# yu45020/Text_Segmentation_Image_Inpainting

Measured on NVIDIA H100. Metric: PartialConv UNet 512x512 images/sec (fwd+bwd), higher is better.
Workload: dtype bf16

## Files before the change

### include/pconv_b200.h

```cpp
#ifndef PCONV_B200_H_
#define PCONV_B200_H_

#include <stddef.h>
#include <stdint.h>

#ifdef __cplusplus
extern "C" {
#endif

typedef void *pcb_stream_t;

enum { PCB_F32 = 0, PCB_BF16 = 1 };
enum { PCB_ACT_NONE = 0, PCB_ACT_RELU = 1, PCB_ACT_LEAKY = 2, PCB_ACT_RELU6 = 3 };
enum { PCB_MAX_PARTS = 8 };

typedef struct {
    const void    *x;
    const uint8_t *mask;
    int32_t c;
    int32_t x_cstride;
    int32_t x_up;
    int32_t mask_up;
} pcb_part;

typedef struct {
    int32_t n, h, w, cin;
    int32_t cout, kh, kw;
    int32_t stride, pad_h, pad_w, dil;
    int32_t groups;
    int32_t ho, wo;
    int32_t dtype;
    int32_t same_holes;
    int32_t no_guard;
    int32_t plain;
    int32_t force_generic;
    int32_t nparts;
    pcb_part parts[PCB_MAX_PARTS];
} pcb_conv;

const char *pcb_last_error(void);
int pcb_version(void);
unsigned long long pcb_launch_count(void);
int pcb_conv_uses_tensor_cores(const pcb_conv *c);


size_t pcb_pconv_workspace(const pcb_conv *c);

void pcb_conv_weight_layout(const pcb_conv *c, size_t *fwd_elems, size_t *dgrad_elems);
int pcb_conv_weight_prepare(const pcb_conv *c, const float *w_master_krsc, void *w_fwd, void *w_dgrad, pcb_stream_t stream);
int pcb_conv_weight_refresh(const pcb_conv *c, const float *w_master_krsc, void *w_fwd, void *w_dgrad, pcb_stream_t stream);

int pcb_pconv_forward(const pcb_conv *c, const void *w_fwd, const float *bias, void *y, int y_cstride, float *msum,
                      uint8_t *newmask, void *workspace, pcb_stream_t stream);
int pcb_pconv_mask_pass(const pcb_conv *c, float *msum, uint8_t *newmask, void *workspace, pcb_stream_t stream);
int pcb_pconv_forward_premasked(const pcb_conv *c, const void *w_fwd, const float *bias, void *y, int y_cstride, float *msum,
                      uint8_t *newmask, void *workspace, pcb_stream_t stream);
int pcb_conv_fuses_bn_stats(const pcb_conv *c);
int pcb_pconv_forward_bn(const pcb_conv *c, const void *w_fwd, const float *bias, void *y, int y_cstride, float *msum,
                         uint8_t *newmask, void *workspace, int mask_pass_done, double *bn_sums, pcb_stream_t stream);
int pcb_conv_fuses_affine_act(const pcb_conv *c);
int pcb_pconv_forward_affine_act(const pcb_conv *c, const void *w_fwd, const float *bias, void *y, int y_cstride, float *msum,
                                 uint8_t *newmask, void *workspace, int mask_pass_done, const float *scale, const float *shift,
                                 int act, float slope, pcb_stream_t stream);

int pcb_pconv_renorm_backward(const pcb_conv *c, const void *dy, int dy_cstride, const float *msum, void *dc, int dc_cstride,
                              float *dbias, pcb_stream_t stream);

int pcb_pconv_backward_data(const pcb_conv *c, const void *dc, int dc_cstride, const void *w_fwd, const void *w_dgrad,
                            void *const *dx, const int32_t *dx_cstride, pcb_stream_t stream);
int pcb_conv_dgrad_at_source_resolution(const pcb_conv *c);

int pcb_conv_dgrad_fuses_relu(const pcb_conv *c);
int pcb_pconv_backward_data_relu(const pcb_conv *c, const void *dc, int dc_cstride, const void *w_dgrad, void *dx, int dx_cstride,
                                 const void *relu_x, int relu_cstride, pcb_stream_t stream);

int pcb_pconv_backward_weight(const pcb_conv *c, const void *dc, int dc_cstride, float *dw, void *workspace, pcb_stream_t stream);
int pcb_pconv_backward_weight_acc(const pcb_conv *c, const void *dc, int dc_cstride, float *dw, void *workspace, pcb_stream_t stream);

int pcb_debug_pipeline_status(int *code);
enum { PCB_ROUTE_NONE = 0, PCB_ROUTE_GENERIC = 1, PCB_ROUTE_DEPTHWISE = 2, PCB_ROUTE_STEM = 3, PCB_ROUTE_K2R = 4,
       PCB_ROUTE_SMALLCO = 5, PCB_ROUTE_TMA = 6, PCB_ROUTE_TMA_S2 = 7, PCB_ROUTE_GATHER = 8 };
int pcb_debug_conv_routes(const pcb_conv *c, int32_t routes[3]);

int pcb_mask_planes_from_dense(const float *mask_nchw, int n, int c, int h, int w, uint8_t *planes, pcb_stream_t stream);
int pcb_mask_plane_to_dense(const uint8_t *plane, int n, int h, int w, int up, float *dst_nchw, int ctot, int c0, int c,
                            pcb_stream_t stream);

int pcb_bn_stats(const void *x, int dtype, long long count, int c, double *sum, double *sqsum, pcb_stream_t stream);
int pcb_bn_stats_acc(const void *x, int dtype, long long count, int c, double *sums, pcb_stream_t stream);
int pcb_bn_forward_fused(const void *x, int dtype, long long count, int c, const double *sums, const float *gamma,
                         const float *beta, float *running_mean, float *running_var, long long *num_batches_tracked,
                         float momentum, float eps, int act, float slope, const void *residual, void *y, float *coef,
                         pcb_stream_t stream);
int pcb_bn_finalize(const double *sum, const double *sqsum, long long count, int c, const float *gamma,
                    const float *beta, float *running_mean, float *running_var, long long *num_batches_tracked,
                    float momentum, float eps, int training, float *scale, float *shift, float *save_mean,
                    float *save_invstd, pcb_stream_t stream);
int pcb_bn_act_forward(const void *x, int dtype, long long count, int c, const float *scale, const float *shift,
                       int act, float slope, const void *residual, void *y, pcb_stream_t stream);
int pcb_bn_act_backward_reduce(const void *gy, const void *x, int dtype, long long count, int c, const float *scale,
                               const float *shift, const float *mean, const float *invstd, int act, float slope,
                               double *sum_g, double *sum_gx, pcb_stream_t stream);
int pcb_bn_act_backward_reduce_acc(const void *gy, const void *x, int dtype, long long count, int c, const float *scale,
                                   const float *shift, const float *mean, const float *invstd, int act, float slope,
                                   double *sums, pcb_stream_t stream);
int pcb_bn_act_backward_small(const void *gy, const void *x, int dtype, long long count, int c, const float *coef, int act,
                              float slope, const float *msum, void *dx, float *dgamma, float *dbeta, pcb_stream_t stream);
int pcb_bn_act_backward_apply(const void *gy, const void *x, int dtype, long long count, int c, const float *scale,
                              const float *shift, const float *mean, const float *invstd, int act, float slope,
                              const double *sum_g, const double *sum_gx, int training, void *dx, float *dgamma,
                              float *dbeta, pcb_stream_t stream);
int pcb_bn_act_backward_apply_renorm(const void *gy, const void *x, int dtype, long long count, int c, const float *scale,
                                     const float *shift, const float *mean, const float *invstd, int act, float slope,
                                     const double *sum_g, const double *sum_gx, int training, const float *msum, void *dc,
                                     float *dgamma, float *dbeta, pcb_stream_t stream);

int pcb_upsample2x_forward(const void *x, int dtype, int n, int h, int w, int c, void *y, pcb_stream_t stream);
int pcb_upsample2x_backward(const void *gy, int dtype, int n, int h, int w, int c, void *gx, pcb_stream_t stream);
int pcb_concat_forward(const pcb_part *parts, int nparts, int dtype, int n, int h, int w, void *y, pcb_stream_t stream);
int pcb_concat_backward(const void *gy, const int32_t *c, const int32_t *up, int nparts, int dtype, int n, int h,
                        int w, void *const *gx, pcb_stream_t stream);

int pcb_avgpool_forward(const void *x, void *y, int dtype, int n, int h, int w, int c, int k, int stride, int pad, pcb_stream_t stream);
int pcb_avgpool_backward(const void *gy, void *gx, int dtype, int n, int h, int w, int c, int k, int stride, int pad, pcb_stream_t stream);
int pcb_bilinear_forward(const void *x, void *y, int dtype, int n, int h, int w, int c, int scale, pcb_stream_t stream);
int pcb_bilinear_backward(const void *gy, void *gx, int dtype, int n, int h, int w, int c, int scale, pcb_stream_t stream);
int pcb_gap_forward(const void *x, int dtype, int n, long long hw, int c, float *out, pcb_stream_t stream);
int pcb_gap_backward(const float *g, void *dx, int dtype, int n, long long hw, int c, int accumulate, pcb_stream_t stream);
int pcb_scse_forward(const void *x, const float *cse, const float *ws, void *y, float *sse_out, int dtype, int n, long long hw, int c,
                     pcb_stream_t stream);
int pcb_scse_backward(const void *gy, const void *x, const float *cse, const float *ws, const float *sse, void *dx, float *dcse,
                      float *dws, int dtype, int n, long long hw, int c, pcb_stream_t stream);
int pcb_seg_mask_postprocess(const void *logits, int dtype, int n, int h, int w, int cstride, int h_valid, int w_valid, int oh,
                             int ow, uint8_t *out, pcb_stream_t stream);

typedef struct {
    const uint8_t *rgb;
    const uint8_t *mask;
    int32_t h, w, rgb_stride, mask_stride;
} pcb_inpaint_src;
typedef struct {
    int32_t top, left, height, width;
    int32_t gray;
    int32_t nlines, nellipses;
    int32_t lines[5][5];
    int32_t ellipses[5][4];
} pcb_inpaint_params;
int pcb_inpaint_validate(const pcb_inpaint_src *h_srcs, const pcb_inpaint_params *h_params, int n, int cap_n, int cap_h, int cap_w,
                         int out);
int pcb_inpaint_sample(const pcb_inpaint_src *srcs, int n, int out, int strokes, uint64_t *rng, pcb_inpaint_params *params,
                       pcb_stream_t stream);
int pcb_inpaint_prepare(const pcb_inpaint_src *srcs, const pcb_inpaint_params *params, int n, int cap_h, int cap_w, int out,
                        int strokes, uint8_t *tmp, void *corrupted, int dtype, uint8_t *mask_plane, float *clean, pcb_stream_t stream);

typedef struct {
    const uint8_t *page;
    const uint8_t *mask;
    int32_t h, w, page_stride, mask_stride;
} pcb_seg_src;
typedef struct {
    int32_t top, left, height, width;
    int32_t brightness_first;
    float brightness, contrast;
    int32_t reserved;
} pcb_seg_params;
int pcb_seg_validate(const pcb_seg_src *h_srcs, const pcb_seg_params *h_params, int n, int cap_n, int cap_h, int cap_w, int out);
int pcb_seg_sample(const pcb_seg_src *srcs, int n, uint64_t *rng, pcb_seg_params *params, pcb_stream_t stream);
int pcb_seg_prepare(const pcb_seg_src *srcs, const pcb_seg_params *params, int n, int cap_h, int cap_w, int out, uint8_t *tmp,
                    uint8_t *planes, int *hist, const float *h_norm, void *x, int dtype, float *target, pcb_stream_t stream);

int pcb_inpaint_loss_pixel_forward(const float *raw, const float *origin, const void *output, int out_dtype, const long long *out_strides,
                                   const uint8_t *plane, int n, int h, int w, void *vgg_in, int dtype, double *sums, pcb_stream_t stream);
int pcb_inpaint_loss_pixel_backward(const float *raw, const float *origin, const void *output, int out_dtype, const long long *out_strides,
                                    const uint8_t *plane, int n, int h, int w, const void *dvgg_in, int dtype, const float *coef,
                                    const float *gscale, void *grad, const long long *grad_strides, pcb_stream_t stream);
int pcb_maxpool2x2_forward(const void *x, void *y, int dtype, int n, int h, int w, int c, pcb_stream_t stream);
int pcb_maxpool2x2_backward(const void *gy, const void *x, void *gx, int dtype, int n, int h, int w, int c, int relu_mask, pcb_stream_t stream);
int pcb_feature_l1_forward(const void *f, int dtype, int n, long long hw, int c, double *sums, pcb_stream_t stream);
int pcb_feature_loss_backward(const void *f, int dtype, int n, long long hw, int c, const void *g_next, const void *g_gram, float l1_coef,
                              float gram_coef, const float *gscale, void *df, pcb_stream_t stream);
int pcb_gram_l1_forward(const float *gram, int n, int c, float norm, double *sums, pcb_stream_t stream);
int pcb_gram_sign_sym(const float *gram, int n, int c, float norm, float *t, pcb_stream_t stream);
int pcb_k2r_image_weight(const float *w_oihw, int cout, float *wz, pcb_stream_t stream);
int pcb_k2r_image_dgrad(const void *z, int dtype, int n, int h, int w, void *dx, pcb_stream_t stream);
int pcb_inpaint_loss_finalize(const double *sums, const double *h_inv, float *loss, float *terms, pcb_stream_t stream);

enum { PCB_SEG_FOCAL = 0, PCB_SEG_BOOTSTRAP = 1 };
enum { PCB_SEG_NONE = 0, PCB_SEG_MEAN = 1, PCB_SEG_SUM = 2 };
int pcb_seg_loss_partials(long long count);
int pcb_seg_loss_forward(const void *x, int dtype, const long long *x_strides, const float *target, int n, int h, int w, int loss,
                         int reduction, float p0, float one_minus_beta, float background_weight, float words_weight, double *partials,
                         unsigned int *counter, float *out, pcb_stream_t stream);
int pcb_seg_loss_backward(const void *x, int dtype, const long long *x_strides, const float *target, int n, int h, int w, int loss,
                          int reduction, float p0, float one_minus_beta, float background_weight, float words_weight, const float *gout,
                          void *dx, const long long *dx_strides, pcb_stream_t stream);

int pcb_l1_mean_forward(const void *x, int dtype, long long numel, float *loss ,
                        double *scratch , pcb_stream_t stream);
int pcb_l1_mean_backward(const void *x, int dtype, long long numel, float gscale, void *gx, pcb_stream_t stream);
int pcb_sgd_step(float *param, const float *grad, float *momentum_buf, long long numel, float lr, float momentum,
                 float weight_decay, int nesterov, int first_step, pcb_stream_t stream);
int pcb_sgd_step_scaled(float *param, const float *grad, float *momentum_buf, long long numel, float lr, float momentum,
                        float weight_decay, int nesterov, int first_step, float grad_scale, pcb_stream_t stream);
int pcb_sgd_step_dev(float *param, const float *grad, float *momentum_buf, long long numel, const float *lr, float momentum,
                     float weight_decay, int nesterov, float grad_scale, pcb_stream_t stream);
enum { PCB_CLR_TRIANGULAR = 0, PCB_CLR_TRIANGULAR2 = 1, PCB_CLR_EXP_RANGE = 2 };
int pcb_lr_cyclic(long long *iteration, double base_lr, double max_lr, double step_size, int mode, double gamma, float *lr,
                  double *lr64, pcb_stream_t stream);

#ifdef __cplusplus
}
#endif
#endif
```

### text_segmentation_image_inpainting_b200/_lib.py

```python
import ctypes
import os
import threading

from . import build as _build

PCB_F32, PCB_BF16 = 0, 1
ACT_NONE, ACT_RELU, ACT_LEAKY, ACT_RELU6 = 0, 1, 2, 3
MAX_PARTS = 8
SEG_FOCAL, SEG_BOOTSTRAP = 0, 1
SEG_NONE, SEG_MEAN, SEG_SUM = 0, 1, 2
CLR_TRIANGULAR, CLR_TRIANGULAR2, CLR_EXP_RANGE = 0, 1, 2
ROUTES = ("none", "generic", "depthwise", "stem", "k2r", "smallco", "tma", "tma_s2", "gather")

c_int, c_ll, c_float, c_void_p, c_size_t = ctypes.c_int, ctypes.c_longlong, ctypes.c_float, ctypes.c_void_p, ctypes.c_size_t


class Part(ctypes.Structure):
    _fields_ = [("x", c_void_p), ("mask", c_void_p), ("c", ctypes.c_int32), ("x_cstride", ctypes.c_int32),
                ("x_up", ctypes.c_int32), ("mask_up", ctypes.c_int32)]


class Conv(ctypes.Structure):
    _fields_ = [(k, ctypes.c_int32) for k in
                ("n", "h", "w", "cin", "cout", "kh", "kw", "stride", "pad_h", "pad_w", "dil", "groups", "ho", "wo",
                 "dtype", "same_holes", "no_guard", "plain", "force_generic", "nparts")] + [("parts", Part * MAX_PARTS)]


_SIGS = {
    "pcb_last_error": (ctypes.c_char_p, []),
    "pcb_version": (c_int, []),
    "pcb_launch_count": (ctypes.c_ulonglong, []),
    "pcb_conv_uses_tensor_cores": (c_int, [ctypes.POINTER(Conv)]),
    "pcb_conv_dgrad_at_source_resolution": (c_int, [ctypes.POINTER(Conv)]),
    "pcb_pconv_workspace": (c_size_t, [ctypes.POINTER(Conv)]),
    "pcb_conv_weight_layout": (None, [ctypes.POINTER(Conv), ctypes.POINTER(c_size_t), ctypes.POINTER(c_size_t)]),
    "pcb_conv_weight_prepare": (c_int, [ctypes.POINTER(Conv), c_void_p, c_void_p, c_void_p, c_void_p]),
    "pcb_conv_weight_refresh": (c_int, [ctypes.POINTER(Conv), c_void_p, c_void_p, c_void_p, c_void_p]),
    "pcb_pconv_forward": (c_int, [ctypes.POINTER(Conv), c_void_p, c_void_p, c_void_p, c_int, c_void_p, c_void_p, c_void_p, c_void_p]),
    "pcb_pconv_forward_premasked": (c_int, [ctypes.POINTER(Conv), c_void_p, c_void_p, c_void_p, c_int, c_void_p, c_void_p, c_void_p, c_void_p]),
    "pcb_conv_fuses_bn_stats": (c_int, [ctypes.POINTER(Conv)]),
    "pcb_pconv_forward_bn": (c_int, [ctypes.POINTER(Conv), c_void_p, c_void_p, c_void_p, c_int, c_void_p, c_void_p, c_void_p, c_int, c_void_p, c_void_p]),
    "pcb_conv_fuses_affine_act": (c_int, [ctypes.POINTER(Conv)]),
    "pcb_pconv_forward_affine_act": (c_int, [ctypes.POINTER(Conv), c_void_p, c_void_p, c_void_p, c_int, c_void_p, c_void_p, c_void_p, c_int,
                                             c_void_p, c_void_p, c_int, c_float, c_void_p]),
    "pcb_seg_mask_postprocess": (c_int, [c_void_p, c_int, c_int, c_int, c_int, c_int, c_int, c_int, c_int, c_int, c_void_p, c_void_p]),
    "pcb_pconv_mask_pass":(c_int, [ctypes.POINTER(Conv), c_void_p, c_void_p, c_void_p, c_void_p]),
    "pcb_pconv_renorm_backward": (c_int, [ctypes.POINTER(Conv), c_void_p, c_int, c_void_p, c_void_p, c_int, c_void_p, c_void_p]),
    "pcb_pconv_backward_data": (c_int, [ctypes.POINTER(Conv), c_void_p, c_int, c_void_p, c_void_p, ctypes.POINTER(c_void_p),
                                        ctypes.POINTER(ctypes.c_int32), c_void_p]),
    "pcb_pconv_backward_weight": (c_int, [ctypes.POINTER(Conv), c_void_p, c_int, c_void_p, c_void_p, c_void_p]),
    "pcb_pconv_backward_weight_acc": (c_int, [ctypes.POINTER(Conv), c_void_p, c_int, c_void_p, c_void_p, c_void_p]),
    "pcb_debug_pipeline_status": (c_int, [ctypes.POINTER(c_int)]),
    "pcb_debug_conv_routes": (c_int, [ctypes.POINTER(Conv), ctypes.POINTER(ctypes.c_int32)]),
    "pcb_mask_planes_from_dense": (c_int, [c_void_p, c_int, c_int, c_int, c_int, c_void_p, c_void_p]),
    "pcb_mask_plane_to_dense": (c_int, [c_void_p, c_int, c_int, c_int, c_int, c_void_p, c_int, c_int, c_int, c_void_p]),
    "pcb_bn_stats": (c_int, [c_void_p, c_int, c_ll, c_int, c_void_p, c_void_p, c_void_p]),
    "pcb_bn_stats_acc": (c_int, [c_void_p, c_int, c_ll, c_int, c_void_p, c_void_p]),
    "pcb_bn_forward_fused": (c_int, [c_void_p, c_int, c_ll, c_int, c_void_p, c_void_p, c_void_p, c_void_p, c_void_p, c_void_p,
                                     c_float, c_float, c_int, c_float, c_void_p, c_void_p, c_void_p, c_void_p]),
    "pcb_bn_act_backward_reduce_acc": (c_int, [c_void_p, c_void_p, c_int, c_ll, c_int, c_void_p, c_void_p, c_void_p, c_void_p,
                                               c_int, c_float, c_void_p, c_void_p]),
    "pcb_bn_act_backward_small": (c_int, [c_void_p, c_void_p, c_int, c_ll, c_int, c_void_p, c_int, c_float, c_void_p, c_void_p, c_void_p, c_void_p, c_void_p]),
    "pcb_bn_finalize": (c_int, [c_void_p, c_void_p, c_ll, c_int, c_void_p, c_void_p, c_void_p, c_void_p, c_void_p,
                                c_float, c_float, c_int, c_void_p, c_void_p, c_void_p, c_void_p, c_void_p]),
    "pcb_bn_act_forward": (c_int, [c_void_p, c_int, c_ll, c_int, c_void_p, c_void_p, c_int, c_float, c_void_p, c_void_p, c_void_p]),
    "pcb_bn_act_backward_reduce": (c_int, [c_void_p, c_void_p, c_int, c_ll, c_int, c_void_p, c_void_p, c_void_p, c_void_p,
                                           c_int, c_float, c_void_p, c_void_p, c_void_p]),
    "pcb_bn_act_backward_apply": (c_int, [c_void_p, c_void_p, c_int, c_ll, c_int, c_void_p, c_void_p, c_void_p, c_void_p,
                                          c_int, c_float, c_void_p, c_void_p, c_int, c_void_p, c_void_p, c_void_p, c_void_p]),
    "pcb_bn_act_backward_apply_renorm": (c_int, [c_void_p, c_void_p, c_int, c_ll, c_int, c_void_p, c_void_p, c_void_p, c_void_p,
                                                 c_int, c_float, c_void_p, c_void_p, c_int, c_void_p, c_void_p, c_void_p, c_void_p, c_void_p]),
    "pcb_upsample2x_forward": (c_int, [c_void_p, c_int, c_int, c_int, c_int, c_int, c_void_p, c_void_p]),
    "pcb_upsample2x_backward": (c_int, [c_void_p, c_int, c_int, c_int, c_int, c_int, c_void_p, c_void_p]),
    "pcb_concat_forward": (c_int, [ctypes.POINTER(Part), c_int, c_int, c_int, c_int, c_int, c_void_p, c_void_p]),
    "pcb_concat_backward": (c_int, [c_void_p, ctypes.POINTER(ctypes.c_int32), ctypes.POINTER(ctypes.c_int32), c_int, c_int,
                                    c_int, c_int, c_int, ctypes.POINTER(c_void_p), c_void_p]),
    "pcb_avgpool_forward": (c_int, [c_void_p, c_void_p, c_int, c_int, c_int, c_int, c_int, c_int, c_int, c_int, c_void_p]),
    "pcb_avgpool_backward": (c_int, [c_void_p, c_void_p, c_int, c_int, c_int, c_int, c_int, c_int, c_int, c_int, c_void_p]),
    "pcb_bilinear_forward": (c_int, [c_void_p, c_void_p, c_int, c_int, c_int, c_int, c_int, c_int, c_void_p]),
    "pcb_bilinear_backward": (c_int, [c_void_p, c_void_p, c_int, c_int, c_int, c_int, c_int, c_int, c_void_p]),
    "pcb_gap_forward": (c_int, [c_void_p, c_int, c_int, c_ll, c_int, c_void_p, c_void_p]),
    "pcb_gap_backward": (c_int, [c_void_p, c_void_p, c_int, c_int, c_ll, c_int, c_int, c_void_p]),
    "pcb_scse_forward": (c_int, [c_void_p, c_void_p, c_void_p, c_void_p, c_void_p, c_int, c_int, c_ll, c_int, c_void_p]),
    "pcb_scse_backward": (c_int, [c_void_p, c_void_p, c_void_p, c_void_p, c_void_p, c_void_p, c_void_p, c_void_p, c_int, c_int, c_ll,
                                  c_int, c_void_p]),
    "pcb_inpaint_validate": (c_int, [c_void_p, c_void_p, c_int, c_int, c_int, c_int, c_int]),
    "pcb_inpaint_sample": (c_int, [c_void_p, c_int, c_int, c_int, c_void_p, c_void_p, c_void_p]),
    "pcb_inpaint_prepare": (c_int, [c_void_p, c_void_p, c_int, c_int, c_int, c_int, c_int, c_void_p, c_void_p, c_int, c_void_p, c_void_p,
                                    c_void_p]),
    "pcb_seg_validate": (c_int, [c_void_p, c_void_p, c_int, c_int, c_int, c_int, c_int]),
    "pcb_seg_sample": (c_int, [c_void_p, c_int, c_void_p, c_void_p, c_void_p]),
    "pcb_seg_prepare": (c_int, [c_void_p, c_void_p, c_int, c_int, c_int, c_int, c_void_p, c_void_p, c_void_p, c_void_p, c_void_p, c_int,
                                c_void_p, c_void_p]),
    "pcb_seg_loss_partials": (c_int, [c_ll]),
    "pcb_seg_loss_forward": (c_int, [c_void_p, c_int, c_void_p, c_void_p, c_int, c_int, c_int, c_int, c_int, c_float, c_float, c_float,
                                     c_float, c_void_p, c_void_p, c_void_p, c_void_p]),
    "pcb_seg_loss_backward": (c_int, [c_void_p, c_int, c_void_p, c_void_p, c_int, c_int, c_int, c_int, c_int, c_float, c_float, c_float,
                                      c_float, c_void_p, c_void_p, c_void_p, c_void_p]),
    "pcb_inpaint_loss_pixel_forward": (c_int, [c_void_p, c_void_p, c_void_p, c_int, c_void_p, c_void_p, c_int, c_int, c_int, c_void_p,
                                               c_int, c_void_p, c_void_p]),
    "pcb_inpaint_loss_pixel_backward": (c_int, [c_void_p, c_void_p, c_void_p, c_int, c_void_p, c_void_p, c_int, c_int, c_int, c_void_p,
                                                c_int, c_void_p, c_void_p, c_void_p, c_void_p, c_void_p]),
    "pcb_maxpool2x2_forward": (c_int, [c_void_p, c_void_p, c_int, c_int, c_int, c_int, c_int, c_void_p]),
    "pcb_maxpool2x2_backward": (c_int, [c_void_p, c_void_p, c_void_p, c_int, c_int, c_int, c_int, c_int, c_int, c_void_p]),
    "pcb_feature_l1_forward": (c_int, [c_void_p, c_int, c_int, c_ll, c_int, c_void_p, c_void_p]),
    "pcb_feature_loss_backward": (c_int, [c_void_p, c_int, c_int, c_ll, c_int, c_void_p, c_void_p, c_float, c_float, c_void_p, c_void_p,
                                          c_void_p]),
    "pcb_gram_l1_forward": (c_int, [c_void_p, c_int, c_int, c_float, c_void_p, c_void_p]),
    "pcb_gram_sign_sym": (c_int, [c_void_p, c_int, c_int, c_float, c_void_p, c_void_p]),
    "pcb_inpaint_loss_finalize": (c_int, [c_void_p, c_void_p, c_void_p, c_void_p, c_void_p]),
    "pcb_k2r_image_weight": (c_int, [c_void_p, c_int, c_void_p, c_void_p]),
    "pcb_k2r_image_dgrad": (c_int, [c_void_p, c_int, c_int, c_int, c_int, c_void_p, c_void_p]),
    "pcb_conv_dgrad_fuses_relu": (c_int, [ctypes.POINTER(Conv)]),
    "pcb_pconv_backward_data_relu": (c_int, [ctypes.POINTER(Conv), c_void_p, c_int, c_void_p, c_void_p, c_int, c_void_p, c_int, c_void_p]),
    "pcb_l1_mean_forward": (c_int, [c_void_p, c_int, c_ll, c_void_p, c_void_p, c_void_p]),
    "pcb_l1_mean_backward": (c_int, [c_void_p, c_int, c_ll, c_float, c_void_p, c_void_p]),
    "pcb_sgd_step": (c_int, [c_void_p, c_void_p, c_void_p, c_ll, c_float, c_float, c_float, c_int, c_int, c_void_p]),
    "pcb_sgd_step_scaled": (c_int, [c_void_p, c_void_p, c_void_p, c_ll, c_float, c_float, c_float, c_int, c_int, c_float, c_void_p]),
    "pcb_sgd_step_dev": (c_int, [c_void_p, c_void_p, c_void_p, c_ll, c_void_p, c_float, c_float, c_int, c_float, c_void_p]),
    "pcb_lr_cyclic": (c_int, [c_void_p, ctypes.c_double, ctypes.c_double, ctypes.c_double, c_int, ctypes.c_double, c_void_p, c_void_p,
                              c_void_p]),
}

EXPORTED_SYMBOLS = tuple(_SIGS)

_lib = None
_lock = threading.Lock()


class PcbError(RuntimeError):
    pass


def lib_path():
    return _build.LIB


def load():
    global _lib
    if _lib is not None:
        return _lib
    with _lock:
        if _lib is not None:
            return _lib
        path = _build.LIB
        if os.environ.get("PCB_REBUILD") == "1":
            path = _build.build(force=True)
        elif _build.needs_build():
            path = _build.build()
        lib = ctypes.CDLL(path)
        for name, (res, args) in _SIGS.items():
            fn = getattr(lib, name)
            fn.restype = res
            fn.argtypes = args
        _lib = lib
    return _lib


def check(rc):
    if rc != 0:
        raise PcbError(load().pcb_last_error().decode(errors="replace"))


def launch_count():
    return int(load().pcb_launch_count())
```

### text_segmentation_image_inpainting_b200/csrc/api.cu

```cuda
#include <stdarg.h>
#include <string.h>

#include <atomic>

#include "pcb_common.cuh"

static thread_local char g_err[1024] = "";
static std::atomic<unsigned long long> g_launches{0};

int pcb_set_error(const char *fmt, ...) {
    va_list ap;
    va_start(ap, fmt);
    vsnprintf(g_err, sizeof(g_err), fmt, ap);
    va_end(ap);
    return 1;
}
void pcb_count_launch(int n) { g_launches.fetch_add(static_cast<unsigned long long>(n)); }

extern "C" __attribute__((visibility("default"))) const char *pcb_last_error(void) { return g_err; }
extern "C" __attribute__((visibility("default"))) int pcb_version(void) { return 1; }
extern "C" __attribute__((visibility("default"))) unsigned long long pcb_launch_count(void) { return g_launches.load(); }

static int validate(const pcb_conv *c, bool need_x) {
    PCB_CHECK(c != nullptr, "null pcb_conv");
// ... 53 lines not shown
    if (f == FAMILY_TC) return pcb_tc_weight_prepare(c, w_master_krsc, w_fwd, w_dgrad, zero_padding, st);
    return pcb_cast_weights(w_master_krsc, w_fwd, static_cast<long long>(c->cout) * c->kh * c->kw * (c->cin / c->groups), c->dtype, st);
}

PCB_API int pcb_conv_weight_prepare(const pcb_conv *c, const float *w_master_krsc, void *w_fwd, void *w_dgrad, pcb_stream_t stream) {
    return weight_prepare(c, w_master_krsc, w_fwd, w_dgrad, true, stream);
}

PCB_API int pcb_conv_weight_refresh(const pcb_conv *c, const float *w_master_krsc, void *w_fwd, void *w_dgrad, pcb_stream_t stream) {
    return weight_prepare(c, w_master_krsc, w_fwd, w_dgrad, false, stream);
}

static bool fuses_epilogue(const pcb_conv *c) {
    if (!c) return false;
    const Family f = family_of(c);
    return f == FAMILY_DW || (f == FAMILY_TC && pcb_tc_fuses_epilogue(c));
}

PCB_API int pcb_conv_fuses_bn_stats(const pcb_conv *c) { return fuses_epilogue(c) ? 1 : 0; }

PCB_API int pcb_conv_fuses_affine_act(const pcb_conv *c) { return fuses_epilogue(c) ? 1 : 0; }

static int pconv_forward_impl(const pcb_conv *c, const void *w_fwd, const float *bias, void *y, int y_cstride, float *msum,
                              uint8_t *newmask, void *workspace, bool mask_pass_done, double *bn_sums, const pcb_ep *ep,
                              pcb_stream_t stream) {
    if (int rc = validate(c, true)) return rc;
    PCB_CHECK(w_fwd && y && msum && newmask && y_cstride >= c->cout, "pcb_pconv_forward: bad arguments");
    cudaStream_t st = static_cast<cudaStream_t>(stream);
    if (c->plain) msum = nullptr;
    else if (!mask_pass_done)
        if (int rc = pcb_mask_sums(c, msum, newmask, st)) return rc;
    PCB_CHECK(bn_sums == nullptr || pcb_conv_fuses_bn_stats(c), "pcb_pconv_forward_bn: this problem's kernel does not fuse the BatchNorm statistics (ask pcb_conv_fuses_bn_stats first)");
    PCB_CHECK(ep == nullptr || pcb_conv_fuses_affine_act(c), "pcb_pconv_forward_affine_act: this problem's kernel does not apply a fused BatchNorm + activation (ask pcb_conv_fuses_affine_act first)");
    const Family f = family_of(c);
    if (f == FAMILY_DW) {
        PCB_CHECK(y_cstride % 8 == 0, "depthwise forward: y channel stride must be a multiple of 8");
        return pcb_dw_forward(c, w_fwd, bias, y, y_cstride, msum, bn_sums, ep, st);
    }
    if (f == FAMILY_TC) {
        PCB_CHECK(workspace != nullptr, "pcb_pconv_forward: workspace required for the tensor-core path");
        PCB_CHECK((reinterpret_cast<uintptr_t>(w_fwd) & 15) == 0 && (reinterpret_cast<uintptr_t>(y) & 15) == 0, "w / y must be 16-byte aligned");
        return pcb_tc_forward_ws(c, w_fwd, bias, y, y_cstride, msum, static_cast<uint64_t *>(workspace), mask_pass_done, bn_sums, ep, st);
    }
    return pcb_generic_forward(c, w_fwd, bias, y, y_cstride, msum, st);
}

PCB_API int pcb_pconv_forward(const pcb_conv *c, const void *w_fwd, const float *bias, void *y, int y_cstride, float *msum,
                              uint8_t *newmask, void *workspace, pcb_stream_t stream) {
    return pconv_forward_impl(c, w_fwd, bias, y, y_cstride, msum, newmask, workspace, false, nullptr, nullptr, stream);
}

PCB_API int pcb_pconv_forward_bn(const pcb_conv *c, const void *w_fwd, const float *bias, void *y, int y_cstride, float *msum,
                                 uint8_t *newmask, void *workspace, int mask_pass_done, double *bn_sums, pcb_stream_t stream) {
    return pconv_forward_impl(c, w_fwd, bias, y, y_cstride, msum, newmask, workspace, mask_pass_done != 0, bn_sums, nullptr, stream);
}

PCB_API int pcb_pconv_forward_affine_act(const pcb_conv *c, const void *w_fwd, const float *bias, void *y, int y_cstride, float *msum,
                                         uint8_t *newmask, void *workspace, int mask_pass_done, const float *scale, const float *shift,
                                         int act, float slope, pcb_stream_t stream) {
    PCB_CHECK(act >= PCB_ACT_NONE && act <= PCB_ACT_RELU6, "pcb_pconv_forward_affine_act: bad activation %d", act);
    PCB_CHECK((scale == nullptr) == (shift == nullptr), "pcb_pconv_forward_affine_act: scale and shift must both be given or both be NULL");
    const pcb_ep ep{scale, shift, act, slope};
    return pconv_forward_impl(c, w_fwd, bias, y, y_cstride, msum, newmask, workspace, mask_pass_done != 0, nullptr, &ep, stream);
}

PCB_API int pcb_pconv_mask_pass(const pcb_conv *c, float *msum, uint8_t *newmask, void *workspace, pcb_stream_t stream) {
    if (int rc = validate(c, false)) return rc;
    PCB_CHECK(msum && newmask, "pcb_pconv_mask_pass: bad arguments");
    cudaStream_t st = static_cast<cudaStream_t>(stream);
    if (int rc = pcb_mask_sums(c, msum, newmask, st)) return rc;
    if (family_of(c) == FAMILY_TC) {
        PCB_CHECK(workspace != nullptr, "pcb_pconv_mask_pass: workspace required for the tensor-core path");
        return pcb_tc_forward_mask_pass(c, static_cast<uint64_t *>(workspace), st);
    }
    return 0;
}

PCB_API int pcb_pconv_forward_premasked(const pcb_conv *c, const void *w_fwd, const float *bias, void *y, int y_cstride, float *msum,
                                        uint8_t *newmask, void *workspace, pcb_stream_t stream) {
    return pconv_forward_impl(c, w_fwd, bias, y, y_cstride, msum, newmask, workspace, true, nullptr, nullptr, stream);
}

PCB_API int pcb_pconv_backward_data(const pcb_conv *c, const void *dc, int dc_cstride, const void *w_fwd, const void *w_dgrad,
                                    void *const *dx, const int32_t *dx_cstride, pcb_stream_t stream) {
    if (int rc = validate(c, false)) return rc;
    PCB_CHECK(dc && w_fwd && dx && dx_cstride && dc_cstride >= c->cout, "pcb_pconv_backward_data: bad arguments");
    cudaStream_t st = static_cast<cudaStream_t>(stream);
    const Family f = family_of(c);
    if (f == FAMILY_DW) {
        if (!dx[0]) return 0;
        PCB_CHECK(dc_cstride % 8 == 0 && dx_cstride[0] % 8 == 0, "depthwise dgrad: channel strides must be multiples of 8");
        return pcb_dw_dgrad(c, dc, dc_cstride, w_fwd, dx[0], dx_cstride[0], st);
    }
    if (f == FAMILY_TC) return pcb_tc_dgrad(c, dc, dc_cstride, w_dgrad, dx, dx_cstride, st);
    return pcb_generic_dgrad(c, dc, dc_cstride, w_fwd, dx, dx_cstride, st);
}

PCB_API int pcb_conv_dgrad_fuses_relu(const pcb_conv *c) {
    if (!c || validate(c, false) || family_of(c) != FAMILY_TC) return 0;
    return pcb_tc_dgrad_fuses_relu(c) ? 1 : 0;
}

PCB_API int pcb_pconv_backward_data_relu(const pcb_conv *c, const void *dc, int dc_cstride, const void *w_dgrad, void *dx, int dx_cstride,
                                         const void *relu_x, int relu_cstride, pcb_stream_t stream) {
    PCB_CHECK(dc && w_dgrad && dx && relu_x && dc_cstride >= c->cout, "pcb_pconv_backward_data_relu: bad arguments");
    PCB_CHECK(pcb_conv_dgrad_fuses_relu(c), "pcb_pconv_backward_data_relu: this problem's kernel does not fuse the ReLU backward "
                                            "(ask pcb_conv_dgrad_fuses_relu first)");
    PCB_CHECK((reinterpret_cast<uintptr_t>(dc) & 15) == 0, "pcb_pconv_backward_data_relu: dc misaligned");
    void *dxs[1] = {dx};
    const int cs[1] = {dx_cstride};
    return pcb_tc_dgrad(c, dc, dc_cstride, w_dgrad, dxs, cs, static_cast<cudaStream_t>(stream), relu_x, relu_cstride);
}

static int backward_weight_impl(const pcb_conv *c, const void *dc, int dc_cstride, float *dw, void *workspace, bool zero_dw, pcb_stream_t stream) {
    if (int rc = validate(c, true)) return rc;
    PCB_CHECK(dc && dw && dc_cstride >= c->cout, "pcb_pconv_backward_weight: bad arguments");
    cudaStream_t st = static_cast<cudaStream_t>(stream);
    const Family f = family_of(c);
    if (f == FAMILY_DW) {
        PCB_CHECK(dc_cstride % 8 == 0, "depthwise wgrad: dc channel stride must be a multiple of 8");
        return pcb_dw_wgrad(c, dc, dc_cstride, dw, zero_dw, st);
    }
    if (f == FAMILY_TC) {
        PCB_CHECK(workspace != nullptr && (reinterpret_cast<uintptr_t>(dc) & 15) == 0, "pcb_pconv_backward_weight: workspace required / dc misaligned");
        return pcb_tc_wgrad(c, dc, dc_cstride, dw, workspace, zero_dw, st);
    }
    return pcb_generic_wgrad(c, dc, dc_cstride, dw, zero_dw, st);
}

PCB_API int pcb_pconv_backward_weight(const pcb_conv *c, const void *dc, int dc_cstride, float *dw, void *workspace, pcb_stream_t stream) {
    return backward_weight_impl(c, dc, dc_cstride, dw, workspace, true, stream);
}

PCB_API int pcb_pconv_backward_weight_acc(const pcb_conv *c, const void *dc, int dc_cstride, float *dw, void *workspace, pcb_stream_t stream) {
    return backward_weight_impl(c, dc, dc_cstride, dw, workspace, false, stream);
}

PCB_API int pcb_debug_pipeline_status(int *code) {
    PCB_CHECK(code != nullptr, "null code");
    return pcb_tc_read_abort_flag(code);
}

PCB_API int pcb_debug_conv_routes(const pcb_conv *c, int32_t routes[3]) {
    PCB_CHECK(routes != nullptr, "null routes");
    if (int rc = validate(c, false)) return rc;
    const Family f = family_of(c);
    if (f == FAMILY_TC) {
        pcb_tc_routes(c, routes);
        return 0;
    }
    routes[0] = routes[1] = routes[2] = (f == FAMILY_DW) ? PCB_ROUTE_DEPTHWISE : PCB_ROUTE_GENERIC;
    return 0;
}
```

### text_segmentation_image_inpainting_b200/csrc/conv_generic.cu

```cuda
#include <algorithm>
#include <string.h>

#include "pcb_common.cuh"

namespace {

struct GPart {
    const void *x;
    const uint8_t *mask;
    int c, choff, cstride, xup, mup;
};

struct GParams {
    int n, h, w, cin, cout, kh, kw, stride, pad_h, pad_w, dil, groups, ho, wo;
    int same_holes, no_guard, plain, nparts;
    GPart parts[PCB_MAX_PARTS];
};

void fill(GParams &G, const pcb_conv *c) {
    G.n = c->n; G.h = c->h; G.w = c->w; G.cin = c->cin; G.cout = c->cout; G.kh = c->kh; G.kw = c->kw;
    G.stride = c->stride; G.pad_h = c->pad_h; G.pad_w = c->pad_w; G.dil = c->dil; G.groups = c->groups;
    G.ho = c->ho; G.wo = c->wo; G.same_holes = c->same_holes; G.no_guard = c->no_guard; G.plain = c->plain; G.nparts = c->nparts;
    int off = 0;
    for (int p = 0; p < c->nparts; ++p) {
        G.parts[p].x = c->parts[p].x; G.parts[p].mask = c->parts[p].mask; G.parts[p].c = c->parts[p].c;
        G.parts[p].choff = off; G.parts[p].cstride = c->parts[p].x_cstride; G.parts[p].xup = c->parts[p].x_up;
        G.parts[p].mup = c->parts[p].mask_up;
        off += c->parts[p].c;
    }
}

__device__ __forceinline__ bool mask_at(const GParams &G, int p, int nn, int hi, int wi) {
    const GPart &pt = G.parts[p];
    if (!pt.mask) return true;
    return pt.mask[(static_cast<long long>(nn) * (G.h >> pt.mup) + (hi >> pt.mup)) * (G.w >> pt.mup) + (wi >> pt.mup)] != 0;
}

__global__ void mask_sums_kernel(const GParams G, float *msum, uint8_t *newmask) {
    const long long plane = static_cast<long long>(G.ho) * G.wo;
    const long long total = plane * G.n;
    const long long m = blockIdx.x * static_cast<long long>(blockDim.x) + threadIdx.x;
    if (m >= total) return;
    const int mg = (G.groups > 1 && !G.same_holes) ? G.groups : 1;
    const int nn = static_cast<int>(m / plane);
    const int rem = static_cast<int>(m - nn * plane), oh = rem / G.wo, ow = rem - oh * G.wo;
    const int cig = G.cin / G.groups;
    for (int g = 0; g < mg; ++g) {
        if (G.plain) { msum[g * total + m] = 1.f; newmask[g * total + m] = 1; continue; }
        int s = 0;
        const int np = G.same_holes ? 1 : G.nparts;
        for (int p = 0; p < np; ++p) {
            int weight;
            if (G.same_holes) weight = G.cin;
            else if (mg == 1) weight = G.parts[p].c;
            else {
                const int lo = max(G.parts[p].choff, g * cig), hi = min(G.parts[p].choff + G.parts[p].c, (g + 1) * cig);
                weight = max(0, hi - lo);
            }
            if (weight == 0) continue;
            int cnt = 0;
            for (int tr = 0; tr < G.kh; ++tr)
                for (int tc = 0; tc < G.kw; ++tc) {
                    const int hi = oh * G.stride - G.pad_h + tr * G.dil, wi = ow * G.stride - G.pad_w + tc * G.dil;
                    if (hi < 0 || hi >= G.h || wi < 0 || wi >= G.w) continue;
                    cnt += mask_at(G, p, nn, hi, wi) ? 1 : 0;
                }
            s += cnt * weight;
        }
        msum[g * total + m] = static_cast<float>(s);
        newmask[g * total + m] = (G.no_guard || s != 0) ? 1 : 0;
    }
}

template <typename T, int CO>
__global__ void generic_fwd_kernel(const GParams G, const T *__restrict__ w, const float *__restrict__ bias,
                                   const float *__restrict__ msum, T *__restrict__ y, int y_cstride) {
    const long long plane = static_cast<long long>(G.ho) * G.wo;
    const long long total = plane * G.n;
    const long long m = blockIdx.x * static_cast<long long>(blockDim.x) + threadIdx.x;
    if (m >= total) return;
    const int co0 = blockIdx.y * CO;
    const int nn = static_cast<int>(m / plane);
    const int rem = static_cast<int>(m - nn * plane), oh = rem / G.wo, ow = rem - oh * G.wo;
    const int cig = G.cin / G.groups, cog = G.cout / G.groups;
    const int taps = G.kh * G.kw;
    const int mg = (G.groups > 1 && !G.same_holes) ? G.groups : 1;
    float acc[CO];
#pragma unroll
    for (int j = 0; j < CO; ++j) acc[j] = 0.f;

    for (int tr = 0; tr < G.kh; ++tr)
        for (int tc = 0; tc < G.kw; ++tc) {
            const int hi = oh * G.stride - G.pad_h + tr * G.dil, wi = ow * G.stride - G.pad_w + tc * G.dil;
            if (hi < 0 || hi >= G.h || wi < 0 || wi >= G.w) continue;
            const int tap = tr * G.kw + tc;
            for (int p = 0; p < G.nparts; ++p) {
                if (!mask_at(G, p, nn, hi, wi)) continue;
                const GPart &pt = G.parts[p];
                const T *xp = static_cast<const T *>(pt.x) +
                              (static_cast<long long>(nn * (G.h >> pt.xup) + (hi >> pt.xup)) * (G.w >> pt.xup) + (wi >> pt.xup)) * pt.cstride;
                if (G.groups == 1) {
                    for (int cl = 0; cl < pt.c; ++cl) {
                        const float xv = to_f32(xp[cl]);
                        const int ci = pt.choff + cl;
#pragma unroll
                        for (int j = 0; j < CO; ++j)
                            if (co0 + j < G.cout) acc[j] += xv * to_f32(w[(static_cast<long long>(co0 + j) * taps + tap) * cig + ci]);
                    }
                } else {
#pragma unroll
                    for (int j = 0; j < CO; ++j) {
                        const int co = co0 + j;
                        if (co >= G.cout) continue;
                        const int g = co / cog;
                        const int lo = max(pt.choff, g * cig), hi2 = min(pt.choff + pt.c, (g + 1) * cig);
                        for (int ci = lo; ci < hi2; ++ci)
                            acc[j] += to_f32(xp[ci - pt.choff]) * to_f32(w[(static_cast<long long>(co) * taps + tap) * cig + (ci - g * cig)]);
                    }
                }
            }
        }
#pragma unroll
    for (int j = 0; j < CO; ++j) {
        const int co = co0 + j;
        if (co >= G.cout) {
            if (co < y_cstride) y[m * y_cstride + co] = from_f32<T>(0.f);
            continue;
        }
        const int g = (mg == 1) ? 0 : co / cog;
        const float s = msum ? msum[g * total + m] : 1.f;
        const float b = bias ? bias[co] : 0.f;
        float v;
        if (G.no_guard) v = acc[j] / s + b;
        else v = (s == 0.f) ? 0.f : acc[j] / s + b;
        y[m * y_cstride + co] = from_f32<T>(v);
    }
}

struct DxOut { void *ptr[PCB_MAX_PARTS]; int cstride[PCB_MAX_PARTS]; };

template <typename T, int CI>
__global__ void generic_dgrad_kernel(const GParams G, const T *__restrict__ dc, int dc_cstride, const T *__restrict__ w, const DxOut O) {
    const long long plane = static_cast<long long>(G.h) * G.w;
    const long long total = plane * G.n;
    const long long m = blockIdx.x * static_cast<long long>(blockDim.x) + threadIdx.x;
    if (m >= total) return;
    const int ci0 = blockIdx.y * CI;
    const int nn = static_cast<int>(m / plane);
    const int rem = static_cast<int>(m - nn * plane), ih = rem / G.w, iw = rem - ih * G.w;
    const int cig = G.cin / G.groups, cog = G.cout / G.groups;
    const int taps = G.kh * G.kw;
    float acc[CI];
#pragma unroll
    for (int j = 0; j < CI; ++j) acc[j] = 0.f;
    for (int tr = 0; tr < G.kh; ++tr)
        for (int tc = 0; tc < G.kw; ++tc) {
            const int th = ih + G.pad_h - tr * G.dil, tw = iw + G.pad_w - tc * G.dil;
            if (th < 0 || tw < 0) continue;
            const int oh = th / G.stride, ow = tw / G.stride;
            if (oh * G.stride != th || ow * G.stride != tw || oh >= G.ho || ow >= G.wo) continue;
            const int tap = tr * G.kw + tc;
            const T *dp = dc + (static_cast<long long>(nn * G.ho + oh) * G.wo + ow) * dc_cstride;
            if (G.groups == 1) {
                for (int co = 0; co < G.cout; ++co) {
                    const float dv = to_f32(dp[co]);
                    const T *wp = w + (static_cast<long long>(co) * taps + tap) * cig + ci0;
#pragma unroll
                    for (int j = 0; j < CI; ++j)
                        if (ci0 + j < G.cin) acc[j] += dv * to_f32(wp[j]);
                }
            } else {
#pragma unroll
                for (int j = 0; j < CI; ++j) {
                    const int ci = ci0 + j;
                    if (ci >= G.cin) continue;
                    const int g = ci / cig;
                    for (int co = g * cog; co < (g + 1) * cog; ++co)
                        acc[j] += to_f32(dp[co]) * to_f32(w[(static_cast<long long>(co) * taps + tap) * cig + (ci - g * cig)]);
                }
            }
        }
#pragma unroll
    for (int j = 0; j < CI; ++j) {
        const int ci = ci0 + j;
        if (ci >= G.cin) continue;
        int p = 0;
        while (p + 1 < G.nparts && ci >= G.parts[p].choff + G.parts[p].c) ++p;
        if (O.ptr[p] == nullptr) continue;
        const float mv = mask_at(G, p, nn, ih, iw) ? 1.f : 0.f;
        static_cast<T *>(O.ptr[p])[m * O.cstride[p] + (ci - G.parts[p].choff)] = from_f32<T>(acc[j] * mv);
    }
}

template <typename T, int CO_T, int K_T, int PC>
__global__ void __launch_bounds__(256) generic_wgrad_kernel(const GParams G, const T *__restrict__ dc, int dc_cstride, float *__restrict__ dw,
                                                            int g, int pix_per_block) {
    static_assert((CO_T / 4) * (K_T / 4) == 256, "thread tiling");
    __shared__ float s_dc[PC][CO_T];
    __shared__ float s_px[PC][K_T];
    const int cig = G.cin / G.groups, cog = G.cout / G.groups;
    const int taps = G.kh * G.kw;
    const int kg = taps * cig;
    const int k0 = blockIdx.x * K_T, cob = blockIdx.y * CO_T;
    const long long plane = static_cast<long long>(G.ho) * G.wo;
    const long long total = plane * G.n;
    const long long p_begin = static_cast<long long>(blockIdx.z) * pix_per_block;
    const long long p_end = min(total, p_begin + pix_per_block);
    const int tx = threadIdx.x % (K_T / 4), ty = threadIdx.x / (K_T / 4);
    float acc[4][4];
#pragma unroll
    for (int a = 0; a < 4; ++a)
#pragma unroll
        for (int b = 0; b < 4; ++b) acc[a][b] = 0.f;

    for (long long pc = p_begin; pc < p_end; pc += PC) {
        for (int i = threadIdx.x; i < PC * CO_T; i += 256) {
            const int pp = i / CO_T, cc = i - pp * CO_T;
            const long long m = pc + pp;
            float v = 0.f;
            if (m < p_end && cob + cc < cog) v = to_f32(dc[m * dc_cstride + g * cog + cob + cc]);
            s_dc[pp][cc] = v;
        }
        for (int i = threadIdx.x; i < PC * K_T; i += 256) {
            const int pp = i / K_T, kk = i - pp * K_T;
            const long long m = pc + pp;
            const int k = k0 + kk;
            float v = 0.f;
            if (m < p_end && k < kg) {
                const int tap = k / cig, cl = k - tap * cig, ci = g * cig + cl;
                const int tr = tap / G.kw, tc = tap - tr * G.kw;
                const int nn = static_cast<int>(m / plane);
                const int rem = static_cast<int>(m - nn * plane), oh = rem / G.wo, ow = rem - oh * G.wo;
                const int hi = oh * G.stride - G.pad_h + tr * G.dil, wi = ow * G.stride - G.pad_w + tc * G.dil;
                if (hi >= 0 && hi < G.h && wi >= 0 && wi < G.w) {
                    int p = 0;
                    while (p + 1 < G.nparts && ci >= G.parts[p].choff + G.parts[p].c) ++p;
                    if (mask_at(G, p, nn, hi, wi)) {
                        const GPart &pt = G.parts[p];
                        v = to_f32(static_cast<const T *>(pt.x)[(static_cast<long long>(nn * (G.h >> pt.xup) + (hi >> pt.xup)) * (G.w >> pt.xup) + (wi >> pt.xup)) * pt.cstride + (ci - pt.choff)]);
                    }
                }
            }
            s_px[pp][kk] = v;
        }
        __syncthreads();
#pragma unroll
        for (int pp = 0; pp < PC; ++pp) {
            float a[4], b[4];
#pragma unroll
            for (int i = 0; i < 4; ++i) { a[i] = s_dc[pp][ty * 4 + i]; b[i] = s_px[pp][tx * 4 + i]; }
#pragma unroll
            for (int i = 0; i < 4; ++i)
#pragma unroll
                for (int j = 0; j < 4; ++j) acc[i][j] += a[i] * b[j];
        }
        __syncthreads();
    }
#pragma unroll
    for (int i = 0; i < 4; ++i) {
        const int co = cob + ty * 4 + i;
        if (co >= cog) continue;
#pragma unroll
        for (int j = 0; j < 4; ++j) {
            const int k = k0 + tx * 4 + j;
            if (k < kg) atomicAdd(dw + (static_cast<long long>(g * cog + co)) * kg + k, acc[i][j]);
        }
    }
}

template <typename T>
int launch_fwd(const GParams &G, const void *w, const float *bias, const float *msum, void *y, int ycs, cudaStream_t st) {
    const long long total = static_cast<long long>(G.n) * G.ho * G.wo;
    const unsigned gx = static_cast<unsigned>((total + 127) / 128);
    if (ycs <= 4) {
        generic_fwd_kernel<T, 4><<<dim3(gx, (ycs + 3) / 4), 128, 0, st>>>(G, static_cast<const T *>(w), bias, msum, static_cast<T *>(y), ycs);
    } else {
        generic_fwd_kernel<T, 8><<<dim3(gx, (ycs + 7) / 8), 128, 0, st>>>(G, static_cast<const T *>(w), bias, msum, static_cast<T *>(y), ycs);
    }
    PCB_LAUNCH_CHECK();
    return 0;
}

template <typename T>
int launch_dgrad(const GParams &G, const void *dc, int dcs, const void *w, const DxOut &O, cudaStream_t st) {
    const long long total = static_cast<long long>(G.n) * G.h * G.w;
    const unsigned gx = static_cast<unsigned>((total + 127) / 128);
    generic_dgrad_kernel<T, 8><<<dim3(gx, (G.cin + 7) / 8), 128, 0, st>>>(G, static_cast<const T *>(dc), dcs, static_cast<const T *>(w), O);
    PCB_LAUNCH_CHECK();
    return 0;
}

template <typename T>
int launch_wgrad(const GParams &G, const void *dc, int dcs, float *dw, cudaStream_t st) {
    const int cig = G.cin / G.groups, cog = G.cout / G.groups;
    const int kg = G.kh * G.kw * cig;
    const long long total = static_cast<long long>(G.n) * G.ho * G.wo;
    for (int g = 0; g < G.groups; ++g) {
        if (cog <= 8) {
            constexpr int CO_T = 8, K_T = 512, PC = 8;
            const int kt = (kg + K_T - 1) / K_T, ct = (cog + CO_T - 1) / CO_T;
            long long slabs = std::max<long long>(1, std::min<long long>((8ll * pcb_num_sms()) / std::max(1, kt * ct), (total + 2047) / 2048));
            const int ppb = static_cast<int>(((total + slabs - 1) / slabs + PC - 1) / PC * PC);
            slabs = (total + ppb - 1) / ppb;
            generic_wgrad_kernel<T, CO_T, K_T, PC><<<dim3(kt, ct, (unsigned)slabs), 256, 0, st>>>(G, static_cast<const T *>(dc), dcs, dw, g, ppb);
        } else {
            constexpr int CO_T = 64, K_T = 64, PC = 16;
            const int kt = (kg + K_T - 1) / K_T, ct = (cog + CO_T - 1) / CO_T;
            long long slabs = std::max<long long>(1, std::min<long long>((8ll * pcb_num_sms()) / std::max(1, kt * ct), (total + 1023) / 1024));
            const int ppb = static_cast<int>(((total + slabs - 1) / slabs + PC - 1) / PC * PC);
            slabs = (total + ppb - 1) / ppb;
            generic_wgrad_kernel<T, CO_T, K_T, PC><<<dim3(kt, ct, (unsigned)slabs), 256, 0, st>>>(G, static_cast<const T *>(dc), dcs, dw, g, ppb);
        }
        PCB_LAUNCH_CHECK();
    }
    return 0;
}

}

int pcb_mask_sums(const pcb_conv *c, float *msum, uint8_t *newmask, cudaStream_t st) {
    GParams G;
    fill(G, c);
    const long long total = static_cast<long long>(c->n) * c->ho * c->wo;
    mask_sums_kernel<<<static_cast<unsigned>((total + 255) / 256), 256, 0, st>>>(G, msum, newmask);
    PCB_LAUNCH_CHECK();
    return 0;
}

int pcb_generic_forward(const pcb_conv *c, const void *w, const float *bias, void *y, int y_cstride, const float *msum, cudaStream_t st) {
    GParams G;
    fill(G, c);
    if (c->dtype == PCB_BF16) return launch_fwd<bf16>(G, w, bias, msum, y, y_cstride, st);
    return launch_fwd<float>(G, w, bias, msum, y, y_cstride, st);
}

int pcb_generic_dgrad(const pcb_conv *c, const void *dc, int dc_cstride, const void *w_krsc, void *const *dx, const int *dx_cstride,
                      cudaStream_t st) {
    GParams G;
    fill(G, c);
    DxOut O;
    memset(&O, 0, sizeof(O));
    for (int p = 0; p < c->nparts; ++p) { O.ptr[p] = dx[p]; O.cstride[p] = dx_cstride[p]; }
    if (c->dtype == PCB_BF16) return launch_dgrad<bf16>(G, dc, dc_cstride, w_krsc, O, st);
    return launch_dgrad<float>(G, dc, dc_cstride, w_krsc, O, st);
}

int pcb_generic_wgrad(const pcb_conv *c, const void *dc, int dc_cstride, float *dw, bool zero_dw, cudaStream_t st) {
    GParams G;
    fill(G, c);
    const size_t bytes = sizeof(float) * c->cout * c->kh * c->kw * (c->cin / c->groups);
    if (zero_dw) PCB_CUDA(cudaMemsetAsync(dw, 0, bytes, st));
    if (c->dtype == PCB_BF16) return launch_wgrad<bf16>(G, dc, dc_cstride, dw, st);
    return launch_wgrad<float>(G, dc, dc_cstride, dw, st);
}
```

### text_segmentation_image_inpainting_b200/csrc/conv_tc.cu

```cuda
#include <cuda.h>
#include <stdlib.h>
#include <string.h>

#include <algorithm>

#include "pcb_common.cuh"
#include "pcb_ptx.cuh"
#include "pcb_tc_epi.cuh"

namespace {

__device__ __forceinline__ float warp_transpose_sum(float (&v)[32], int lane) {
#pragma unroll
    for (int off = 16, n = 32; off >= 1; off >>= 1, n >>= 1) {
        const bool upper = (lane & off) != 0;
#pragma unroll
        for (int i = 0; i < 16; ++i) {
            if (i < (n >> 1)) {
                const float send = upper ? v[i] : v[i + (n >> 1)];
                const float keep = upper ? v[i + (n >> 1)] : v[i];
                v[i] = keep + __shfl_xor_sync(0xffffffffu, send, off);
            }
        }
    }
// ... 247 lines not shown
            if (MODE == 0 && P.rowpack) {
                const TcPart &pt = P.parts[0];
                const int cs = pt.cstride, rowpitch = P.w * cs;
                for (int tr = 0; tr < P.kh && !dead; ++tr) {
                    int off[8];
                    bool ok[8];
#pragma unroll
                    for (int i = 0; i < 8; ++i) {
                        const bool v = (chunk < P.kw) && ((tmv[0][i] >> (tr * P.kw + chunk)) & 1ull);
                        off[i] = v ? (ibase[0][i] - chunk * 8) + (ph[i] + tr * P.dil) * rowpitch + (pw[i] + chunk * P.dil) * cs : 0;
                        ok[i] = v;
                    }
                    if (!push(pt.x, off, ok)) dead = true;
                }
            } else {
                for (int tap = 0; tap < taps && !dead; ++tap) {
                    const int tr = tap / P.kw, tc = tap - tr * P.kw;
#pragma unroll
                    for (int p = 0; p < TC_MAX_PARTS; ++p) {
                        if (p >= np || dead) break;
                        const TcPart &pt = P.parts[p];
                        const bf16 *src = (MODE == 0) ? pt.x : P.dc;
                        const int cs = (MODE == 0) ? pt.cstride : P.dc_cstride;
                        const int xup = (MODE == 0) ? pt.xup : 0;
                        const int rowpitch = ((MODE == 0) ? (P.w >> xup) : P.wo) * cs;
                        int base[8];
                        bool rv[8];
#pragma unroll
                        for (int i = 0; i < 8; ++i) {
                            bool v;
                            int hi, wi;
                            if (MODE == 0) {
                                v = (tmv[p][i] >> tap) & 1ull;
                                hi = (ph[i] + tr * P.dil) >> xup; wi = (pw[i] + tc * P.dil) >> xup;
                            } else {
                                const int th = ph[i] - tr * P.dil, tw = pw[i] - tc * P.dil;
                                hi = th >> ls; wi = tw >> ls;
                                v = prow[i] && th >= 0 && tw >= 0 && ((th | tw) & (P.stride - 1)) == 0 && hi < P.ho && wi < P.wo;
                            }
                            base[i] = v ? ibase[p][i] + hi * rowpitch + wi * cs : 0;
                            rv[i] = v;
                        }
                        const int nb = ((MODE == 0) ? pt.kext : P.dc_kext) / BLOCK_K;
                        const int c8 = (MODE == 0) ? pt.c8 : P.dc_c8;
                        for (int cb = 0; cb < nb; ++cb) {
                            const bool cv = cb * BLOCK_K + chunk * 8 < c8;
                            int off[8];
                            bool ok[8];
#pragma unroll
                            for (int i = 0; i < 8; ++i) { ok[i] = rv[i] && cv; off[i] = ok[i] ? base[i] + cb * BLOCK_K : 0; }
                            if (!push(src, off, ok)) { dead = true; break; }
                        }
                    }
                }
            }
        }
        ptx::cp_async_wait<0>();
    } else if (warp == 12) {
        if (lane == 0) {
            int itb = 0;
            bool dead = false;
            auto load = [&](int kidx, int n0) -> bool {
                const int s = itb % SB;
                if (!ptx::mbar_wait(bar_empty_b + 8 * s, ((itb / SB) & 1) ^ 1, P.abort_flag, 103)) return false;
                ptx::mbar_arrive_expect_tx(bar_full_b + 8 * s, B_STAGE_BYTES);
                ptx::tma_load_2d(sB + s * B_STAGE_BYTES, &tmap_w, kidx, n0, bar_full_b + 8 * s);
                ++itb;
                return true;
            };
            for (int tile = blockIdx.x; tile < num_tiles && !dead; tile += gridDim.x) {
                const int n0 = (tile % n_tiles) * BLOCK_N;
                if (!tile_active(n0)) continue;
                const int num_kb = (MODE == 0) ? (P.rowpack ? P.kh : taps * (P.ktap / BLOCK_K)) : taps * (P.dc_kext / BLOCK_K);
                for (int kb = 0; kb < num_kb; ++kb)
                    if (!load(kb * BLOCK_K, n0)) { dead = true; break; }
            }
        }
    } else {
        const int e = warp - 4, g = e >> 2;
        const bool leader = (threadIdx.x & 127) == 0;
        const int num_a = (MODE == 0) ? (P.rowpack ? P.kh : taps * (P.ktap / BLOCK_K)) : taps * (P.dc_kext / BLOCK_K);
        const uint32_t a_rows = 64u * 128u;
        float *s_stat = (MODE == 0 && P.bn_sums != nullptr)
                            ? reinterpret_cast<float *>(smem_raw + (s_stat_addr - ptx::smem_u32(smem_raw))) : nullptr;
        const EpiRole<BLOCK_N> R(e);
        float *my_stat = s_stat ? s_stat + R.slice() * STAT_SLICE : nullptr;
        int stat_n0 = -1;
        if (my_stat) {
            for (int i = lane; i < STAT_SLICE; i += 32) my_stat[i] = 0.f;
            __syncwarp();
        }
        int ita = 0, itb = 0;
        bool dead = false;
        for (int tile = blockIdx.x; tile < num_tiles && !dead; tile += gridDim.x) {
            const int m0 = (tile / n_tiles) * BLOCK_M, n0 = (tile % n_tiles) * BLOCK_N;
            if (!tile_active(n0)) continue;
            if (my_stat && n0 != stat_n0) {
                if (stat_n0 >= 0) tc_stats_flush<BLOCK_N>(P, my_stat, lane, stat_n0, R.cb, R.ce, 128);
                stat_n0 = n0;
            }
            float acc[BLOCK_N / 2];
            zero_acc(acc);
            for (int a = 0; a < num_a && !dead; ++a, ++ita) {
                const int sa = ita % SA;
                if (!__all_sync(0xffffffffu, ptx::mbar_wait(bar_full_a + 8 * sa, (ita / SA) & 1, P.abort_flag, 104))) { dead = true; break; }
                ptx::fence_proxy_async_smem();
                const int sb = itb % SB;
                if (__all_sync(0xffffffffu, ptx::mbar_wait(bar_full_b + 8 * sb, (itb / SB) & 1, P.abort_flag, 105))) {
                    const uint64_t db = ptx::make_smem_desc(sB + sb * B_STAGE_BYTES, 16, 1024);
                    ptx::wgmma_fence();
                    const uint64_t da = ptx::make_smem_desc(sA + sa * A_STAGE_BYTES + g * a_rows, 16, 1024);
#pragma unroll
                    for (int k = 0; k < BLOCK_K / 16; ++k)
                        ptx::wgmma_bf16<BLOCK_N, 0, 0>(acc, da + 2 * k, db + 2 * k);
                    ptx::wgmma_commit();
                    ++itb;
                } else {
                    dead = true;
                }
                ptx::wgmma_wait<0>();
                ptx::wgmma_fence_regs(acc);
                if (leader) {
                    ptx::mbar_arrive(bar_empty_b + 8 * sb);
                    ptx::mbar_arrive(bar_empty_a + 8 * sa);
                }
            }
            if (dead) { stat_n0 = -1; break; }
            mma_epilogue<BLOCK_N, MODE>(P, acc, acc_stage, e, lane, m0, n0, my_stat);
        }
        if (my_stat && stat_n0 >= 0) tc_stats_flush<BLOCK_N>(P, my_stat, lane, stat_n0, R.cb, R.ce, 128);
    }
}


template <int BLOCK_N, int MODE, bool HALO>
__global__ void __maxnreg__(TMA_REGS)
pconv_tc_tma_kernel(const __grid_constant__ TcParams P, const __grid_constant__ CUtensorMap tmap_w,
                    const __grid_constant__ CUtensorMap tmap_a0, const __grid_constant__ CUtensorMap tmap_a1) {
    constexpr uint32_t B_BYTES = BLOCK_N * 128;
    extern __shared__ uint8_t smem_raw[];
    const uint32_t smem_base = align1024(ptx::smem_u32(smem_raw));
    const int S = P.stages;
    const int nB = HALO ? P.kw : 1;
    const int hx = HALO ? (P.kw - 1) * P.dil : 0;
    const uint32_t A_BYTES = static_cast<uint32_t>(BLOCK_M + hx) * 128u;
    const uint32_t A_ROOM = (A_BYTES + 1023u) & ~1023u;
    const uint32_t STAGE = A_ROOM + nB * B_BYTES;
    const uint32_t STAGE_TX = A_BYTES + nB * B_BYTES;
    const uint32_t sBar = smem_base + S * STAGE;
    const uint32_t bar_full = sBar, bar_fixed = sBar + 8 * MAX_RING, bar_empty = sBar + 16 * MAX_RING;
    const uint32_t acc_full = sBar + 24 * MAX_RING, acc_empty = acc_full + 8;
    const uint32_t s_stat_addr = sBar + TMA_BAR_BYTES;
    const uint32_t s_acc = s_stat_addr + EPI_STAT_SMEM_BYTES;
    uint8_t *smem_gen = smem_raw + (smem_base - ptx::smem_u32(smem_raw));

    const int warp = __shfl_sync(0xffffffffu, threadIdx.x >> 5, 0), lane = threadIdx.x & 31;
    const int np = (MODE == 0) ? P.nparts : 1;
    const int n_tiles = P.ncols / BLOCK_N;
    const int m_tiles = (P.m_total + BLOCK_M - 1) / BLOCK_M;
    const int num_tiles = m_tiles * n_tiles;
    const int tile0 = static_cast<int>(blockIdx.x), tstep = static_cast<int>(gridDim.x);
    auto m0_of = [&](int mt) -> int { return mt * BLOCK_M; };
    const bool fix = (MODE == 0) && P.use_fix;
    const int kwi = HALO ? 1 : P.kw;

    auto tile_active = [&](int n0) -> bool {
        if (MODE == 0) return true;
        for (int p = 0; p < P.nparts; ++p)
            if (P.parts[p].dx && n0 < P.parts[p].koff + P.parts[p].kext && n0 + BLOCK_N > P.parts[p].koff) return true;
        return false;
    };

    if (threadIdx.x == 0) {
        for (int s = 0; s < MAX_RING; ++s) {
            ptx::mbar_init(bar_full + 8 * s, 1); ptx::mbar_init(bar_fixed + 8 * s, TMA_FIX_THREADS / 32); ptx::mbar_init(bar_empty + 8 * s, 2);
        }
        ptx::mbar_init(acc_full, MMA_WARPS); ptx::mbar_init(acc_empty, EPI_WARPS);
        ptx::fence_mbar_init();
    }
    if (warp == 8 && lane == 0) { ptx::prefetch_tmap(&tmap_w); ptx::prefetch_tmap(&tmap_a0); if (np > 1) ptx::prefetch_tmap(&tmap_a1); }
    __syncthreads();

    float *s_stat = nullptr;
    int stat_n0 = -1;
    bf16 *acc_stage = reinterpret_cast<bf16 *>(smem_gen + (s_acc - smem_base));
    if (warp < MMA_WARPS) {
        ptx::setmaxnreg_inc<TMA_CONSUMER_REGS>();
        const int e = warp, g = warp >> 2;
        const bool leader = (threadIdx.x & 127) == 0;
        const uint32_t ready = fix ? bar_fixed : bar_full;
        const uint64_t desc_a0 = ptx::make_smem_desc(smem_base + g * 64 * 128, 16, 1024);
        const uint64_t desc_b0 = ptx::make_smem_desc(smem_base + A_ROOM, 16, 1024);
        const uint32_t stage16 = STAGE >> 4;
        const int shift0 = (HALO && MODE == 1) ? hx * 8 : 0;
        const int dshift = HALO ? ((MODE == 1) ? -P.dil * 8 : P.dil * 8) : 0;
        const int rows_a = P.kh * kwi;
        int nb0, nb1 = 0, kl0, kl1 = 4;
        {
            const int kext = (MODE == 0) ? P.parts[0].kext : P.dc_kext, c8 = (MODE == 0) ? P.parts[0].c8 : P.dc_c8;
            nb0 = kext / BLOCK_K; kl0 = min(4, (c8 - (nb0 - 1) * BLOCK_K + 15) >> 4);
            if (MODE == 0 && np > 1) { nb1 = P.parts[1].kext / BLOCK_K; kl1 = min(4, (P.parts[1].c8 - (nb1 - 1) * BLOCK_K + 15) >> 4); }
        }
        int s = 0;
        uint32_t ph = 0, aph = 1;
        bool dead = false;
        for (int tile = tile0; tile < num_tiles && !dead; tile += tstep) {
            const int n0 = (tile % n_tiles) * BLOCK_N;
            if (!tile_active(n0)) continue;
            const ConsRows cr = cons_rows<MODE>(P, m0_of(tile / n_tiles), e, lane);
            float acc[BLOCK_N / 2];
            zero_acc(acc);
            int held = -1;
            for (int r = 0; r < rows_a && !dead; ++r) {
#pragma unroll
                for (int p = 0; p < TC_MAX_PARTS; ++p) {
                    const int nbp = (p == 0) ? nb0 : nb1, klast = (p == 0) ? kl0 : kl1;
                    for (int cb = 0; cb < nbp; ++cb) {
                        if (!__all_sync(0xffffffffu, ptx::mbar_wait(ready + 8 * s, ph, P.abort_flag, 124))) { dead = true; break; }
                        uint64_t da = desc_a0 + static_cast<uint64_t>(s * stage16 + shift0), db = desc_b0 + static_cast<uint64_t>(s * stage16);
                        const int ksteps = (cb + 1 < nbp) ? 4 : klast;
                        ptx::wgmma_fence();
                        for (int tc = 0; tc < nB; ++tc, da += dshift, db += B_BYTES >> 4) {
                            if (ksteps == 4) {
#pragma unroll
                                for (int k = 0; k < 4; ++k) ptx::wgmma_bf16<BLOCK_N, 0, 0>(acc, da + 2 * k, db + 2 * k);
                            } else {
                                for (int k = 0; k < ksteps; ++k) ptx::wgmma_bf16<BLOCK_N, 0, 0>(acc, da + 2 * k, db + 2 * k);
                            }
                        }
                        ptx::wgmma_commit();
                        ptx::wgmma_wait<1>();
                        if (held >= 0 && leader) ptx::mbar_arrive(bar_empty + 8 * held);
                        held = s;
                        if (++s == S) { s = 0; ph ^= 1; }
                    }
                    if (dead) break;
                }
            }
            ptx::wgmma_wait<0>();
            ptx::wgmma_fence_regs(acc);
            if (held >= 0 && leader) ptx::mbar_arrive(bar_empty + 8 * held);
            if (dead) break;
            if (!tma_stage_tile<BLOCK_N, MODE>(P, acc, acc_stage, acc_full, acc_empty, aph, e, lane, n0, cr, 125)) break;
        }
    } else {
        ptx::setmaxnreg_dec<TMA_SUPPORT_REGS>();
        if (warp >= EPI_WARP0) {
            const int w = warp - EPI_WARP0;
            s_stat = (MODE == 0 && P.bn_sums != nullptr)
                         ? reinterpret_cast<float *>(smem_gen + (s_stat_addr - smem_base)) + w * EPI_STAT_SLICE : nullptr;
            auto origin = [&](int tile, int &m0, int &n0) {
                m0 = m0_of(tile / n_tiles); n0 = (tile % n_tiles) * BLOCK_N;
                if (!tile_active(n0)) n0 = -1;
            };
            tma_epilogue_warps<BLOCK_N, MODE>(P, tile0, tstep, num_tiles, origin, acc_stage, acc_full, acc_empty, s_stat, stat_n0, w, lane, 126);
            ptx::named_sync(1, EPI_WARPS * 32);
            if (s_stat != nullptr && stat_n0 >= 0) tc_stats_final<BLOCK_N>(P, s_stat - w * EPI_STAT_SLICE, w, lane, stat_n0);
        } else if (warp == 8) {
            int s = 0;
            uint32_t ph = 1;
            const int plane = (MODE == 0) ? P.ho * P.wo : P.h * P.w;
            const int pwid = (MODE == 0) ? P.wo : P.w;
            const int kext0 = (MODE == 0) ? P.parts[0].kext : P.dc_kext, kext1 = (MODE == 0 && np > 1) ? P.parts[1].kext : 0;
            const int dstep = (MODE == 0) ? P.dil : -P.dil;
            const int row_k = P.wk_row, col_k = P.wk_col;
            bool dead = false;
            for (int tile = tile0; tile < num_tiles && !dead; tile += tstep) {
                const int m0 = m0_of(tile / n_tiles), n0 = (tile % n_tiles) * BLOCK_N;
                if (!tile_active(n0)) continue;
                const int img = m0 / plane, rem = m0 - img * plane;
                const int oy = rem / pwid, ox = rem - oy * pwid;
                const int x_org = (MODE == 0) ? ox * P.stride - P.pad_w : (HALO ? ox + P.pad_w - hx : ox + P.pad_w);
                const int y_org = (MODE == 0) ? oy * P.stride - P.pad_h : oy + P.pad_h;
                int krow = P.wk_base;
                for (int tr = 0, y = y_org; tr < P.kh && !dead; ++tr, y += dstep, krow += row_k)
                    for (int ti = 0, x = x_org, kidx = krow; ti < kwi && !dead; ++ti, x += dstep, kidx = krow + ti * col_k) {
#pragma unroll
                        for (int p = 0; p < TC_MAX_PARTS; ++p) {
                            const int kext = (p == 0) ? kext0 : kext1;
                            const CUtensorMap *ma = (p == 0) ? &tmap_a0 : &tmap_a1;
                            for (int c0 = 0; c0 < kext; c0 += BLOCK_K, kidx += BLOCK_K) {
                                if (!__all_sync(0xffffffffu, ptx::mbar_wait(bar_empty + 8 * s, ph, P.abort_flag, 121))) { dead = true; break; }
                                if (ptx::elect_one()) {
                                    const uint32_t full = bar_full + 8 * s, dst = smem_base + s * STAGE;
                                    ptx::mbar_arrive_expect_tx(full, STAGE_TX);
                                    ptx::tma_load_4d(dst, ma, c0, x, y, img, full);
                                    uint32_t bdst = dst + A_ROOM;
                                    for (int tc = 0, kb = kidx; tc < nB; ++tc, kb += col_k, bdst += B_BYTES)
                                        ptx::tma_load_2d(bdst, &tmap_w, kb, n0, full);
                                }
                                __syncwarp();
                                if (++s == S) { s = 0; ph ^= 1; }
                            }
                            if (dead) break;
                        }
                    }
            }
        } else {
            if (fix) {
                constexpr int FR = HALO ? 3 : 2;
                const int t = (warp - 9) * 32 + lane;
                int s = 0;
                uint32_t ph = 0;
                bool dead = false;
                auto zero_row = [&](int row) {
                    uint4 *r = reinterpret_cast<uint4 *>(smem_gen + s * STAGE + row * 128);
                    const uint4 z = make_uint4(0u, 0u, 0u, 0u);
#pragma unroll
                    for (int k = 0; k < 8; ++k) r[k] = z;
                };
                if (!HALO) {
                    uint64_t wnext[FR][TC_MAX_PARTS];
                    auto load_words = [&](int tl) {
#pragma unroll
                        for (int r = 0; r < FR; ++r)
#pragma unroll
                            for (int p = 0; p < TC_MAX_PARTS; ++p) {
                                wnext[r][p] = 0ull;
                                const int m = m0_of(tl / n_tiles) + t + TMA_FIX_THREADS * r;
                                if (p < P.nparts && tl < num_tiles && t + TMA_FIX_THREADS * r < BLOCK_M && m < P.m_total)
                                    wnext[r][p] = __ldg(P.parts[p].tapmask + m);
                            }
                    };
                    load_words(tile0);
                    for (int tile = tile0; tile < num_tiles && !dead; tile += tstep) {
                        uint64_t wcur[FR][TC_MAX_PARTS];
#pragma unroll
                        for (int r = 0; r < FR; ++r)
#pragma unroll
                            for (int p = 0; p < TC_MAX_PARTS; ++p) wcur[r][p] = wnext[r][p];
                        load_words(tile + tstep);
                        if (MODE == 1 && !tile_active((tile % n_tiles) * BLOCK_N)) continue;
                        const int taps = P.kh * P.kw;
                        for (int tap = 0; tap < taps && !dead; ++tap) {
#pragma unroll
                            for (int p = 0; p < TC_MAX_PARTS; ++p) {
                                if (p >= np) break;
                                bool hole[FR], mine = false;
#pragma unroll
                                for (int r = 0; r < FR; ++r) {
                                    hole[r] = t + TMA_FIX_THREADS * r < BLOCK_M && ((wcur[r][p] >> tap) & 1ull) == 0ull;
                                    mine = mine || hole[r];
                                }
                                const bool any_hole = __any_sync(0xffffffffu, mine);
                                const int nb = ((MODE == 0) ? P.parts[p].kext : P.dc_kext) / BLOCK_K;
                                for (int cb = 0; cb < nb; ++cb) {
                                    if (!ptx::mbar_wait(bar_full + 8 * s, ph, P.abort_flag, 122)) { dead = true; break; }
                                    if (any_hole) {
#pragma unroll
                                        for (int r = 0; r < FR; ++r)
                                            if (hole[r]) zero_row(t + TMA_FIX_THREADS * r);
                                        ptx::fence_proxy_async_smem();
                                    }
                                    __syncwarp();
                                    if (lane == 0) ptx::mbar_arrive(bar_fixed + 8 * s);
                                    if (++s == S) { s = 0; ph ^= 1; }
                                }
                                if (dead) break;
                            }
                        }
                    }
                } else {
                    const int plane = P.ho * P.wo;
                    auto load_bits = [&](int tl, uint32_t (&b)[FR]) {
#pragma unroll
                        for (int r = 0; r < FR; ++r) b[r] = 0;
                        if (tl >= num_tiles) return;
                        const int m0 = m0_of(tl / n_tiles);
                        const int img = m0 / plane, rem = m0 - img * plane;
                        const int oy = rem / P.wo, ox = rem - oy * P.wo;
#pragma unroll
                        for (int p = 0; p < TC_MAX_PARTS; ++p) {
                            if (p >= P.nparts || P.parts[p].mask == nullptr) continue;
                            const int mup = P.parts[p].mup;
                            const uint8_t *mk = P.parts[p].mask + static_cast<long long>(img) * (P.h >> mup) * (P.w >> mup);
                            for (int tr = 0; tr < P.kh; ++tr) {
                                const int y = oy - P.pad_h + tr * P.dil;
                                if (y < 0 || y >= P.h) continue;
#pragma unroll
                                for (int r = 0; r < FR; ++r) {
                                    const int row = t + TMA_FIX_THREADS * r, x = ox - P.pad_w + row;
                                    if (row < BLOCK_M + hx && x >= 0 && x < P.w && __ldg(mk + (y >> mup) * (P.w >> mup) + (x >> mup)) == 0)
                                        b[r] |= 1u << (p * 8 + tr);
                                }
                            }
                        }
                    };
                    uint32_t nb_bits[FR];
                    load_bits(tile0, nb_bits);
                    for (int tile = tile0; tile < num_tiles && !dead; tile += tstep) {
                        uint32_t cb_bits[FR];
#pragma unroll
                        for (int r = 0; r < FR; ++r) cb_bits[r] = nb_bits[r];
                        load_bits(tile + tstep, nb_bits);
                        if (MODE == 1 && !tile_active((tile % n_tiles) * BLOCK_N)) continue;
                        for (int tr = 0; tr < P.kh && !dead; ++tr) {
#pragma unroll
                            for (int p = 0; p < TC_MAX_PARTS; ++p) {
                                if (p >= np) break;
                                bool hole[FR], mine = false;
#pragma unroll
                                for (int r = 0; r < FR; ++r) { hole[r] = (cb_bits[r] >> (p * 8 + tr)) & 1u; mine = mine || hole[r]; }
                                const bool any_hole = __any_sync(0xffffffffu, mine);
                                const int nb = ((MODE == 0) ? P.parts[p].kext : P.dc_kext) / BLOCK_K;
                                for (int cb = 0; cb < nb; ++cb) {
                                    if (!ptx::mbar_wait(bar_full + 8 * s, ph, P.abort_flag, 122)) { dead = true; break; }
                                    if (any_hole) {
#pragma unroll
                                        for (int r = 0; r < FR; ++r)
                                            if (hole[r]) zero_row(t + TMA_FIX_THREADS * r);
                                        ptx::fence_proxy_async_smem();
                                    }
                                    __syncwarp();
                                    if (lane == 0) ptx::mbar_arrive(bar_fixed + 8 * s);
                                    if (++s == S) { s = 0; ph ^= 1; }
                                }
                                if (dead) break;
                            }
                        }
                    }
                }
            }
        }
    }

}


constexpr int SP_MAX_ITEMS = 40;
struct SpItem { int dx, dy, wk; };
struct SpTable {
    int n_items;
    SpItem it[SP_MAX_ITEMS];
};

template <int BLOCK_N>
__global__ void __maxnreg__(TMA_REGS)
pconv_tc_sp_kernel(const __grid_constant__ TcParams P, const __grid_constant__ SpTable TB, const __grid_constant__ CUtensorMap tmap_w,
                   const __grid_constant__ CUtensorMap tmap_a) {
    constexpr uint32_t B_BYTES = BLOCK_N * 128;
    constexpr uint32_t STAGE = A_STAGE_BYTES + B_BYTES;
    extern __shared__ uint8_t smem_raw[];
    const uint32_t smem_base = align1024(ptx::smem_u32(smem_raw));
    const int S = P.stages;
    const uint32_t sBar = smem_base + S * STAGE;
    const uint32_t bar_full = sBar, bar_empty = sBar + 16 * MAX_RING;
    const uint32_t acc_full = sBar + 24 * MAX_RING, acc_empty = acc_full + 8;
    const uint32_t s_acc = sBar + TMA_BAR_BYTES + EPI_STAT_SMEM_BYTES;
    bf16 *acc_stage = reinterpret_cast<bf16 *>(smem_raw + (s_acc - ptx::smem_u32(smem_raw)));

    const int warp = __shfl_sync(0xffffffffu, threadIdx.x >> 5, 0), lane = threadIdx.x & 31;
    const int n_tiles = P.ncols / BLOCK_N;
    const int m_tiles = (P.m_total + BLOCK_M - 1) / BLOCK_M;
    const int num_tiles = m_tiles * n_tiles;
    const int tile0 = static_cast<int>(blockIdx.x), tstep = static_cast<int>(gridDim.x);
    const int plane = P.w * P.h;
    const int nbk = P.dc_kext / BLOCK_K;
    const int klast = min(4, (P.dc_c8 - (nbk - 1) * BLOCK_K + 15) >> 4);

    if (threadIdx.x == 0) {
        for (int s = 0; s < MAX_RING; ++s) { ptx::mbar_init(bar_full + 8 * s, 1); ptx::mbar_init(bar_empty + 8 * s, 2); }
        ptx::mbar_init(acc_full, MMA_WARPS); ptx::mbar_init(acc_empty, EPI_WARPS);
        ptx::fence_mbar_init();
    }
    if (warp == 8 && lane == 0) { ptx::prefetch_tmap(&tmap_w); ptx::prefetch_tmap(&tmap_a); }
    __syncthreads();

    if (warp < MMA_WARPS) {
        ptx::setmaxnreg_inc<TMA_CONSUMER_REGS>();
        const int e = warp, g = warp >> 2;
        const bool leader = (threadIdx.x & 127) == 0;
        const uint64_t desc_a0 = ptx::make_smem_desc(smem_base + g * 64 * 128, 16, 1024);
        const uint64_t desc_b0 = ptx::make_smem_desc(smem_base + A_STAGE_BYTES, 16, 1024);
        const uint32_t stage16 = STAGE >> 4;
        int s = 0;
        uint32_t ph = 0, aph = 1;
        bool dead = false;
        for (int tile = tile0; tile < num_tiles && !dead; tile += tstep) {
            float acc[BLOCK_N / 2];
            zero_acc(acc);
            int held = -1;
            for (int i = 0; i < TB.n_items && !dead; ++i) {
                for (int cb = 0; cb < nbk; ++cb) {
                    if (!__all_sync(0xffffffffu, ptx::mbar_wait(bar_full + 8 * s, ph, P.abort_flag, 324))) { dead = true; break; }
                    const uint64_t da = desc_a0 + static_cast<uint64_t>(s * stage16), db = desc_b0 + static_cast<uint64_t>(s * stage16);
                    const int ksteps = (cb + 1 < nbk) ? 4 : klast;
                    ptx::wgmma_fence();
                    for (int k = 0; k < ksteps; ++k) ptx::wgmma_bf16<BLOCK_N, 0, 0>(acc, da + 2 * k, db + 2 * k);
                    ptx::wgmma_commit();
                    ptx::wgmma_wait<1>();
                    if (held >= 0 && leader) ptx::mbar_arrive(bar_empty + 8 * held);
                    held = s;
                    if (++s == S) { s = 0; ph ^= 1; }
                }
            }
            ptx::wgmma_wait<0>();
            ptx::wgmma_fence_regs(acc);
            if (held >= 0 && leader) ptx::mbar_arrive(bar_empty + 8 * held);
            if (dead) break;
            if (!tma_stage_tile<BLOCK_N, 1>(P, acc, acc_stage, acc_full, acc_empty, aph, e, lane, (tile % n_tiles) * BLOCK_N, ConsRows{}, 325)) break;
        }
    } else {
        ptx::setmaxnreg_dec<TMA_SUPPORT_REGS>();
        if (warp >= EPI_WARP0) {
            int stat_n0 = -1;
            auto origin = [&](int tile, int &m0, int &n0) { m0 = (tile / n_tiles) * BLOCK_M; n0 = (tile % n_tiles) * BLOCK_N; };
            tma_epilogue_warps<BLOCK_N, 1>(P, tile0, tstep, num_tiles, origin, acc_stage, acc_full, acc_empty, nullptr, stat_n0,
                                           warp - EPI_WARP0, lane, 326);
        } else if (warp == 8) {
            int s = 0;
            uint32_t ph = 1;
            bool dead = false;
            for (int tile = tile0; tile < num_tiles && !dead; tile += tstep) {
                const int m0 = (tile / n_tiles) * BLOCK_M, n0 = (tile % n_tiles) * BLOCK_N;
                const int img = m0 / plane, rem = m0 - img * plane;
                const int oy = rem / P.w, ox = rem - oy * P.w;
                for (int i = 0; i < TB.n_items && !dead; ++i) {
                    const SpItem it = TB.it[i];
                    const int x = 2 * ox + it.dx, y = 2 * oy + it.dy;
                    for (int cb = 0; cb < nbk; ++cb) {
                        if (!__all_sync(0xffffffffu, ptx::mbar_wait(bar_empty + 8 * s, ph, P.abort_flag, 321))) { dead = true; break; }
                        if (ptx::elect_one()) {
                            const uint32_t full = bar_full + 8 * s, dst = smem_base + s * STAGE;
                            ptx::mbar_arrive_expect_tx(full, STAGE);
                            ptx::tma_load_4d(dst, &tmap_a, cb * BLOCK_K, x, y, img, full);
                            ptx::tma_load_2d(dst + A_STAGE_BYTES, &tmap_w, it.wk + cb * BLOCK_K, n0, full);
                        }
                        __syncwarp();
                        if (++s == S) { s = 0; ph ^= 1; }
                    }
                }
            }
        }
    }
}

__global__ void upsample_part_kernel(const bf16 *__restrict__ src, int cstride, int c8, long long pixels_src, int hs, int ws, bf16 *__restrict__ dst) {
    const int chunks = c8 >> 3;
    const long long total = pixels_src * chunks;
    for (long long i = blockIdx.x * static_cast<long long>(blockDim.x) + threadIdx.x; i < total; i += static_cast<long long>(gridDim.x) * blockDim.x) {
        const int ch = static_cast<int>(i % chunks);
        const long long pix = i / chunks;
        const int x = static_cast<int>(pix % ws);
        const long long t = pix / ws;
        const int y = static_cast<int>(t % hs);
        const long long n = t / hs;
        const uint4 v = __ldg(reinterpret_cast<const uint4 *>(src + pix * cstride + ch * 8));
        bf16 *d = dst + ((n * (2 * hs) + 2 * y) * (2ll * ws) + 2 * x) * c8 + ch * 8;
        uint4 *d0 = reinterpret_cast<uint4 *>(d), *d1 = reinterpret_cast<uint4 *>(d + 2ll * ws * c8);
        d0[0] = v; *reinterpret_cast<uint4 *>(d + c8) = v;
        d1[0] = v; *reinterpret_cast<uint4 *>(d + 2ll * ws * c8 + c8) = v;
    }
}

struct WgParams {
    int n, h, w, cin, cout, kh, kw, stride, pad_h, pad_w, dil, ho, wo;
    int m_total;
    int nparts, rowpack;
// ... 624 lines not shown
    return c->cin >= 32 || c->cout >= 32;
}

struct Layout {
    int rowpack, ktap, cout64, rows_f, bn_f;
    long long kf, kd;
    int koff[TC_MAX_PARTS], kext[TC_MAX_PARTS];
};

Layout layout_of(const pcb_conv *c) {
    Layout L;
    memset(&L, 0, sizeof(L));
    L.rowpack = is_rowpack(c);
    const int taps = c->kh * c->kw;
    if (L.rowpack) {
        L.ktap = 64; L.koff[0] = 0; L.kext[0] = 64;
        L.kf = static_cast<long long>(c->kh) * 64;
    } else {
        int off = 0;
        for (int p = 0; p < c->nparts; ++p) { L.koff[p] = off; L.kext[p] = rup(c->parts[p].c, 64); off += L.kext[p]; }
        L.ktap = off;
        L.kf = static_cast<long long>(taps) * L.ktap;
    }
    L.cout64 = rup(c->cout, 64);
    L.bn_f = (c->cout % 128 == 0) ? 128 : 64;
    L.rows_f = rup(c->cout, L.bn_f);
    L.kd = static_cast<long long>(taps) * L.cout64;
    return L;
}

void fill_parts(const pcb_conv *c, const Layout &L, TcPart *out, const uint64_t *tapmask, long long m_total) {
    int off = 0;
    for (int p = 0; p < c->nparts; ++p) {
        out[p].x = static_cast<const bf16 *>(c->parts[p].x);
        out[p].tapmask = tapmask ? tapmask + static_cast<long long>(p) * m_total : nullptr;
        out[p].mask = c->parts[p].mask;
        out[p].dx = nullptr; out[p].dx_cstride = 0;
        out[p].c = c->parts[p].c;
        out[p].c8 = rup(c->parts[p].c, 8);
        out[p].kext = L.kext[p];
        out[p].koff = L.koff[p];
        out[p].choff = off;
        out[p].cstride = c->parts[p].x_cstride;
        out[p].xup = c->parts[p].x_up;
        out[p].mup = c->parts[p].mask_up;
        off += c->parts[p].c;
    }
}

int launch_tapmask(const pcb_conv *c, uint64_t *out, cudaStream_t st) {
    TapMaskParams T;
    memset(&T, 0, sizeof(T));
    T.n = c->n; T.h = c->h; T.w = c->w; T.kh = c->kh; T.kw = c->kw; T.stride = c->stride; T.pad_h = c->pad_h;
    T.pad_w = c->pad_w; T.dil = c->dil; T.ho = c->ho; T.wo = c->wo; T.m_total = c->n * c->ho * c->wo; T.nparts = c->nparts;
    for (int p = 0; p < c->nparts; ++p) { T.mask[p] = c->parts[p].mask; T.mup[p] = c->parts[p].mask_up; }
    T.out = out;
    tapmask_kernel<<<(T.m_total + 255) / 256, 256, 0, st>>>(T);
    PCB_LAUNCH_CHECK();
    return 0;
}

void set_ep(TcParams &P, const pcb_ep *ep) {
    if (ep == nullptr) return;
    P.ep_on = 1; P.ep_scale = ep->scale; P.ep_shift = ep->shift; P.ep_act = ep->act; P.ep_slope = ep->slope;
}

void base_params(TcParams &P, const pcb_conv *c, const Layout &L) {
    memset(&P, 0, sizeof(P));
    P.n = c->n; P.h = c->h; P.w = c->w; P.cin = c->cin; P.cout = c->cout; P.kh = c->kh; P.kw = c->kw; P.stride = c->stride;
    P.pad_h = c->pad_h; P.pad_w = c->pad_w; P.dil = c->dil; P.ho = c->ho; P.wo = c->wo;
    P.nparts = c->nparts; P.no_guard = c->no_guard; P.rowpack = L.rowpack; P.ktap = L.ktap;
    P.sub = 1; P.py = 0; P.px = 0; P.fh = c->h; P.fw = c->w;
}

constexpr size_t MAX_SMEM = 227 * 1024;
constexpr size_t RING_BUDGET = 208 * 1024;

template <int BLOCK_N, int MODE>
int launch_persistent(TcParams &P, const CUtensorMap &tm, cudaStream_t st) {
    const size_t a_stage = A_STAGE_BYTES;
    const size_t b_stage = BLOCK_N * 128;
    const size_t budget = RING_BUDGET - acc_stage_bytes(BLOCK_N);
    P.ring_b = 6;
    P.ring_a = 6;
    while (P.ring_a * a_stage + P.ring_b * b_stage > budget && P.ring_b > 3) --P.ring_b;
    while (P.ring_a * a_stage + P.ring_b * b_stage > budget && P.ring_a > 2) --P.ring_a;
    const size_t smem = 1024 + P.ring_a * a_stage + P.ring_b * b_stage + 32 * MAX_RING + 16 + STAT_SMEM_BYTES + acc_stage_bytes(BLOCK_N);
    PCB_CHECK(smem <= MAX_SMEM, "tensor-core conv: %zu bytes of shared memory do not fit", smem);
    auto kern = pconv_tc_persistent_kernel<BLOCK_N, MODE>;
    PCB_SMEM_OPT_IN(kern, MAX_SMEM);
    const int num_tiles = ((P.m_total + BLOCK_M - 1) / BLOCK_M) * (P.ncols / BLOCK_N);
    const int grid = std::min(num_tiles, pcb_num_sms());
    kern<<<grid, PERSIST_THREADS, smem, st>>>(P, tm);
    PCB_LAUNCH_CHECK();
    return 0;
}


bool tile_box(int wt, int ht, int *bw, int *bh, int *bn) {
    if (wt < 4) return false;
    if (wt % 128 == 0) { *bw = 128; *bh = 1; *bn = 1; return true; }
    if (128 % wt) return false;
    const int rows = 128 / wt;
    *bw = wt;
    if (ht % rows == 0) { *bh = rows; *bn = 1; return true; }
    if (rows % ht) return false;
    *bh = ht; *bn = rows / ht;
    return true;
}

bool kblock_box(int wt, int ht, int *bw, int *bh, int *bn) {
    if (wt < 4) return false;
    if (wt % 64 == 0) { *bw = 64; *bh = 1; *bn = 1; return true; }
    if (64 % wt) return false;
    const int rows = 64 / wt;
    *bw = wt;
    if (ht % rows == 0) { *bh = rows; *bn = 1; return true; }
    if (rows % ht) return false;
    *bh = ht; *bn = rows / ht;
    return true;
}

bool even_upsampled_parts(const pcb_conv *c) {
    for (int p = 0; p < c->nparts; ++p)
        if (c->parts[p].x_up && ((c->h | c->w) & 1)) return false;
    return true;
}

bool tma_fwd_ok(const pcb_conv *c, int *bw, int *bh, int *bn) {
    if (is_rowpack(c) || !tile_box(c->wo, c->ho, bw, bh, bn)) return false;
    if (c->stride > 2 || *bw * c->stride > 256 || *bh * c->stride > 256) return false;
    return even_upsampled_parts(c);
}

bool tma_dgrad_s2_ok(const pcb_conv *c, int *bw, int *bh, int *bn) {
    if (c->stride != 2 || c->dil != 1 || c->kh < 2 || c->kw < 2 || ((c->h | c->w) & 1) || c->ho != c->h / 2 || c->wo != c->w / 2) return false;
    return tile_box(c->w / 2, c->h / 2, bw, bh, bn);
}

int class_kw(const pcb_conv *c, int px) { return (c->kw - ((px + c->pad_w) & 1) + 1) / 2; }

bool tma_wgrad_ok(const pcb_conv *c, int *bw, int *bh, int *bn) {
    return !is_rowpack(c) && c->stride <= 2 && kblock_box(c->wo, c->ho, bw, bh, bn) && even_upsampled_parts(c);
}

size_t up_bytes(const pcb_conv *c, int p) {
    return (static_cast<size_t>(c->n) * c->h * c->w * rup(c->parts[p].c, 8) * 2 + 255) / 256 * 256;
}
size_t tapmask_bytes(const pcb_conv *c) {
    return (static_cast<size_t>(c->nparts) * c->n * c->ho * c->wo * sizeof(uint64_t) + 255) / 256 * 256;
}

size_t tma_fixed_smem(int block_n) {
    return 1024 + TMA_BAR_BYTES + EPI_STAT_SMEM_BYTES + bf16_stage_bytes(block_n);
}

template <int BLOCK_N, int MODE, bool HALO>
int launch_tma_n(TcParams &P, const CUtensorMap &tw, const CUtensorMap &ta0, const CUtensorMap &ta1, cudaStream_t st) {
    const int nb = HALO ? P.kw : 1;
    const size_t a_room = (static_cast<size_t>(BLOCK_M + (HALO ? (P.kw - 1) * P.dil : 0)) * 128 + 1023) / 1024 * 1024;
    const size_t stage = a_room + static_cast<size_t>(nb) * BLOCK_N * 128;
    const size_t fixed = tma_fixed_smem(BLOCK_N);
    P.stages = static_cast<int>(std::min<size_t>(MAX_RING, (MAX_SMEM - fixed) / stage));
    PCB_CHECK(P.stages >= 2, "TMA-fed conv: stage of %zu bytes does not fit twice", stage);
    const size_t smem = fixed + P.stages * stage;
    auto kern = pconv_tc_tma_kernel<BLOCK_N, MODE, HALO>;
    PCB_SMEM_OPT_IN(kern, MAX_SMEM);
    const int m_tiles = (P.m_total + BLOCK_M - 1) / BLOCK_M;
    const int num_tiles = m_tiles * (P.ncols / BLOCK_N);
    const int grid = std::min(num_tiles, pcb_num_sms());
    kern<<<grid, TMA_THREADS, smem, st>>>(P, tw, ta0, ta1);
    PCB_LAUNCH_CHECK();
    return 0;
}

template <int MODE>
int launch_tma(TcParams &P, const CUtensorMap &tw, const CUtensorMap &ta0, const CUtensorMap &ta1, int bn, bool halo, cudaStream_t st) {
    PCB_CHECK(!(halo && bn == 256), "TMA-fed conv: no 256-wide row-halo tiles");
    if (halo) {
        if (bn == 128) return launch_tma_n<128, MODE, true>(P, tw, ta0, ta1, st);
        if (bn == 64) return launch_tma_n<64, MODE, true>(P, tw, ta0, ta1, st);
        return launch_tma_n<32, MODE, true>(P, tw, ta0, ta1, st);
    }
    if (bn == 256) return launch_tma_n<256, MODE, false>(P, tw, ta0, ta1, st);
    if (bn == 128) return launch_tma_n<128, MODE, false>(P, tw, ta0, ta1, st);
    if (bn == 64) return launch_tma_n<64, MODE, false>(P, tw, ta0, ta1, st);
    return launch_tma_n<32, MODE, false>(P, tw, ta0, ta1, st);
}

bool halo_stages_fit(int kw, int dil, int block_n) {
    const size_t stage = (static_cast<size_t>(128 + (kw - 1) * dil) * 128 + 1023) / 1024 * 1024 + static_cast<size_t>(kw) * block_n * 128;
    return 3 * stage + acc_stage_bytes(block_n) <= RING_BUDGET;
}

bool halo_ok(int kw, int dil, int bw, int bh, int bn, int block_n) {
    return bw == 128 && bh == 1 && bn == 1 && kw >= 2 && 128 + (kw - 1) * dil <= 256 && halo_stages_fit(kw, dil, block_n);
}

int pick_bn(int cols, long long m_total, bool fwd, int sms) {
    const long long m_tiles = (m_total + BLOCK_M - 1) / BLOCK_M;
    if (cols <= 32) return 32;
    auto waves = [&](int b) { return (m_tiles * (cols / b) + sms - 1) / sms; };
    if (cols % 256 == 0 && 2 * waves(256) <= waves(128) && (!fwd || waves(256) == 1)) return 256;
    int bn = (cols % 128 == 0) ? 128 : 64;
    while (bn > 32 && cols % (bn / 2) == 0 && m_tiles * (cols / bn) < sms / 2) bn /= 2;
    return bn;
}

template <int MODE>
int launch_tc(TcParams &P, const CUtensorMap &tm, int bn, cudaStream_t st) {
    return (bn == 128) ? launch_persistent<128, MODE>(P, tm, st) : launch_persistent<64, MODE>(P, tm, st);
}

struct ClassStreams { cudaStream_t aux[3]; cudaEvent_t ev_fork, ev_join[3]; bool ready; };
int class_streams(ClassStreams **out) {
    static thread_local ClassStreams cs_all[PCB_MAX_DEVICES] = {};
    ClassStreams &CS = cs_all[pcb_cur_device()];
    if (!CS.ready) {
        for (int i = 0; i < 3; ++i) {
            PCB_CUDA(cudaStreamCreateWithFlags(&CS.aux[i], cudaStreamNonBlocking));
            PCB_CUDA(cudaEventCreateWithFlags(&CS.ev_join[i], cudaEventDisableTiming));
        }
        PCB_CUDA(cudaEventCreateWithFlags(&CS.ev_fork, cudaEventDisableTiming));
        CS.ready = true;
    }
    *out = &CS;
    return 0;
}

struct SpAxis { int e0[2], ne[2], tapbits[2][4]; bool ok; };

int floordiv2(int v) { return v >= 0 ? v / 2 : -((-v + 1) / 2); }

SpAxis sp_axis(int k, int d, int p) {
    SpAxis A;
    memset(&A, 0, sizeof(A));
    A.ok = k <= 4;
    for (int q = 0; q < 2 && A.ok; ++q) {
        A.e0[q] = floordiv2(q - p);
        const int last = floordiv2(q + (k - 1) * d - p);
        A.ne[q] = last - A.e0[q] + 1;
        if (A.ne[q] < 1 || A.ne[q] > 4) { A.ok = false; break; }
        for (int t = 0; t < k; ++t) A.tapbits[q][floordiv2(q + t * d - p) - A.e0[q]] |= 1 << t;
        for (int e = 0; e < A.ne[q]; ++e)
            if (!A.tapbits[q][e]) A.ok = false;
    }
    return A;
}

struct SpPlan {
    bool ok;
    int pu, ps;
    SpAxis ay, ax;
    int net[4], eoff[4], net_total;
    int kext_u, c8_u;
    long long sp_dg_elems, kd_sp;
    int bw, bh, bn;
    int block_n;
};

SpPlan sp_plan(const pcb_conv *c, const Layout &L, int sms) {
    SpPlan S;
    memset(&S, 0, sizeof(S));
    S.pu = S.ps = -1;
    if (c->stride != 1 || c->ho != c->h || c->wo != c->w || ((c->h | c->w) & 1) || c->nparts > 2) return S;
    for (int p = 0; p < c->nparts; ++p) {
        if (c->parts[p].x_up) { if (S.pu >= 0) return S; S.pu = p; }
        else { if (S.ps >= 0) return S; S.ps = p; }
    }
    if (S.pu < 0) return S;
    if (c->parts[S.pu].mask && c->parts[S.pu].mask_up != 1) return S;
    if (S.ps >= 0 && c->parts[S.ps].mask && c->parts[S.ps].mask_up != 0) return S;
    S.ay = sp_axis(c->kh, c->dil, c->pad_h);
    S.ax = sp_axis(c->kw, c->dil, c->pad_w);
    if (!S.ay.ok || !S.ax.ok) return S;
    if (!tile_box(c->w / 2, c->h / 2, &S.bw, &S.bh, &S.bn)) return S;
    S.kext_u = L.kext[S.pu]; S.c8_u = rup(c->parts[S.pu].c, 8);
    int eo = 0;
    for (int cls = 0; cls < 4; ++cls) {
        S.net[cls] = S.ay.ne[cls >> 1] * S.ax.ne[cls & 1];
        S.eoff[cls] = eo; eo += S.net[cls];
    }
    S.net_total = eo;
    if (S.net_total > SP_MAX_ITEMS) return S;
    S.kd_sp = static_cast<long long>(S.net_total) * L.cout64;
    const long long m_src = static_cast<long long>(c->n) * (c->h / 2) * (c->w / 2);
    S.ok = (m_src + BLOCK_M - 1) / BLOCK_M >= sms / 3;
    S.sp_dg_elems = static_cast<long long>(rup(S.kext_u, 128)) * S.kd_sp;
    S.block_n = std::min(pick_bn(S.kext_u, m_src, true, sms), 64);
    return S;
}

struct SpWParams {
    int cout, taps, cin, kw, cout64, choff_u;
    int eoff[4], nex[4];
    int ybits[2][4], xbits[2][4];
    long long kd_sp;
};

__global__ void sp_weight_dg_kernel(const float *__restrict__ wm, const SpWParams W, bf16 *__restrict__ w_d) {
    const int ci = blockIdx.x;
    int slot = blockIdx.y, cls = 0;
    while (cls < 3 && slot >= W.eoff[cls + 1]) ++cls;
    slot -= W.eoff[cls];
    const int ey = slot / W.nex[cls], ex = slot - ey * W.nex[cls];
    const int yb = W.ybits[cls >> 1][ey], xb = W.xbits[cls & 1][ex];
    for (int co = threadIdx.x; co < W.cout; co += blockDim.x) {
        const float *wrow = wm + static_cast<long long>(co) * W.taps * W.cin + W.choff_u + ci;
        float v = 0.f;
        for (int tr = 0; tr < 4; ++tr)
            if ((yb >> tr) & 1)
                for (int tc = 0; tc < 4; ++tc)
                    if ((xb >> tc) & 1) v += wrow[static_cast<long long>(tr * W.kw + tc) * W.cin];
        w_d[static_cast<long long>(ci) * W.kd_sp + static_cast<long long>(W.eoff[cls] + slot) * W.cout64 + co] = __float2bfloat16_rn(v);
    }
}

int sp_weight_prepare(const pcb_conv *c, const SpPlan &S, const Layout &L, const float *w_master, bf16 *w_d, cudaStream_t st) {
    SpWParams W;
    memset(&W, 0, sizeof(W));
    W.cout = c->cout; W.taps = c->kh * c->kw; W.cin = c->cin; W.kw = c->kw; W.cout64 = L.cout64; W.kd_sp = S.kd_sp;
    for (int p = 0; p < S.pu; ++p) W.choff_u += c->parts[p].c;
    for (int cls = 0; cls < 4; ++cls) { W.eoff[cls] = S.eoff[cls]; W.nex[cls] = S.ax.ne[cls & 1]; }
    for (int q = 0; q < 2; ++q)
        for (int e = 0; e < 4; ++e) { W.ybits[q][e] = S.ay.tapbits[q][e]; W.xbits[q][e] = S.ax.tapbits[q][e]; }
    sp_weight_dg_kernel<<<dim3(c->parts[S.pu].c, S.net_total), 128, 0, st>>>(w_master, W, w_d);
    PCB_LAUNCH_CHECK();
    return 0;
}

template <int BLOCK_N>
int launch_sp_n(TcParams &P, const SpTable &TB, const CUtensorMap &tw, const CUtensorMap &ta, cudaStream_t st) {
    const size_t stage = A_STAGE_BYTES + static_cast<size_t>(BLOCK_N) * 128;
    const size_t fixed = tma_fixed_smem(BLOCK_N);
    P.stages = static_cast<int>(std::min<size_t>(MAX_RING, (MAX_SMEM - fixed) / stage));
    PCB_CHECK(P.stages >= 2, "sub-pixel conv: stage of %zu bytes does not fit twice", stage);
    const size_t smem = fixed + P.stages * stage;
    auto kern = pconv_tc_sp_kernel<BLOCK_N>;
    PCB_SMEM_OPT_IN(kern, MAX_SMEM);
    const int num_tiles = ((P.m_total + BLOCK_M - 1) / BLOCK_M) * (P.ncols / BLOCK_N);
    const int grid = std::min(num_tiles, pcb_num_sms());
    kern<<<grid, TMA_THREADS, smem, st>>>(P, TB, tw, ta);
    PCB_LAUNCH_CHECK();
    return 0;
}

int sp_dgrad_up(const pcb_conv *c, const SpPlan &S, const Layout &L, const void *dc, int dc_cstride, const bf16 *w_sp_dg, void *dx_u, int dx_cstride,
                int *flag, cudaStream_t st) {
    const int hs = c->h / 2, ws = c->w / 2;
    const long long m_src = static_cast<long long>(c->n) * hs * ws;
    TcParams P;
    base_params(P, c, L);
    P.h = hs; P.w = ws; P.m_total = static_cast<int>(m_src);
    P.sub = 1; P.py = 0; P.px = 0; P.fh = hs; P.fw = ws;
    P.nparts = 1;
    memset(P.parts, 0, sizeof(P.parts));
    TcPart &pt = P.parts[0];
    pt.c = c->parts[S.pu].c; pt.c8 = S.c8_u; pt.kext = S.kext_u; pt.koff = 0; pt.mask = c->parts[S.pu].mask; pt.mup = 0;
    pt.dx = static_cast<bf16 *>(dx_u); pt.dx_cstride = dx_cstride;
    PCB_CHECK(dx_cstride % 8 == 0 && dx_cstride >= S.c8_u && (reinterpret_cast<uintptr_t>(dx_u) & 15) == 0, "sub-pixel dgrad: dx must be 16-byte aligned with a channel stride that is a multiple of 8");
    P.dc = static_cast<const bf16 *>(dc); P.dc_cstride = dc_cstride; P.dc_c8 = rup(c->cout, 8); P.dc_kext = L.cout64;
    P.abort_flag = flag;
    P.ncols = S.kext_u;
    P.box_w = S.bw; P.box_h = S.bh; P.box_n = S.bn;
    const int bn = S.block_n;
    SpTable TB;
    memset(&TB, 0, sizeof(TB));
    int ni = 0;
    for (int cls = 0; cls < 4; ++cls) {
        const int py = cls >> 1, px = cls & 1;
        const int ney = S.ay.ne[py], nex = S.ax.ne[px];
        for (int e = 0; e < ney; ++e)
            for (int f = 0; f < nex; ++f) {
                SpItem &it = TB.it[ni++];
                it.dx = px - 2 * (S.ax.e0[px] + f); it.dy = py - 2 * (S.ay.e0[py] + e);
                it.wk = (S.eoff[cls] + e * nex + f) * L.cout64;
            }
    }
    TB.n_items = ni;
    CUtensorMap ta, tw;
    if (int rc = make_tmap_nhwc(&ta, dc, P.dc_c8, c->wo, c->ho, c->n, dc_cstride, S.bw, S.bh, S.bn, 2)) return rc;
    if (int rc = make_tmap_2d(&tw, w_sp_dg, rup(S.kext_u, 128), S.kd_sp, S.kd_sp, bn)) return rc;
    return (bn == 64) ? launch_sp_n<64>(P, TB, tw, ta, st) : launch_sp_n<32>(P, TB, tw, ta, st);
}

enum TcRoute { ROUTE_NONE, ROUTE_STEM, ROUTE_K2R, ROUTE_SMALLCO, ROUTE_TMA, ROUTE_TMA_S2, ROUTE_GATHER };

struct DirPlan {
    TcRoute route;
    int box_w, box_h, box_n;
    int bn;
    bool halo;
};

struct TcPlan {
    bool ok;
    Layout L;
    long long m_out, m_in;
    size_t fwd_elems, dg_elems;
    size_t extra_fwd_off, extra_dg_off;
    size_t sp_off;
    size_t workspace;
    size_t up_off[TC_MAX_PARTS];
    DirPlan fwd, dg, wg;
    bool fwd_tapmask, wg_tapmask;
    StemPlan stem;
    K2rPlan k2r;
    SpPlan sp;
    bool cls_halo[4];
    bool cls_fork;
    bool fuses_epilogue;
    bool dg_fuses_relu;
    bool dg_at_source;
};

TcPlan tc_plan(const pcb_conv *c) {
    TcPlan T;
    memset(&T, 0, sizeof(T));
    T.sp.pu = T.sp.ps = -1;
    if (!common_ok(c)) return T;
    T.ok = true;
    const int sms = pcb_num_sms();
    T.L = layout_of(c);
    const Layout &L = T.L;
    T.m_out = static_cast<long long>(c->n) * c->ho * c->wo;
    T.m_in = static_cast<long long>(c->n) * c->h * c->w;
    bool any_mask = false;
    for (int p = 0; p < c->nparts; ++p) any_mask = any_mask || (c->parts[p].mask != nullptr);
    const bool smallco = !L.rowpack && pcb_smallco_eligible(c);
    if (L.rowpack) T.stem = pcb_stem_plan(c);
    if (smallco) T.k2r = pcb_k2r_plan(c);
    const bool stem = T.stem.ok, k2r = T.k2r.ok;
    if (!L.rowpack && !smallco) T.sp = sp_plan(c, L, sms);

    T.fwd_elems = static_cast<size_t>(L.rows_f) * L.kf;
    T.sp_off = static_cast<size_t>(rup(L.ktap, 128)) * L.kd;
    T.dg_elems = L.rowpack ? 0 : T.sp_off;
    if (T.sp.ok) T.dg_elems += static_cast<size_t>(T.sp.sp_dg_elems);
    T.extra_fwd_off = (T.fwd_elems + 63) / 64 * 64;
    T.extra_dg_off = (T.sp_off + 63) / 64 * 64;
    if (k2r) {
        T.fwd_elems = T.extra_fwd_off + T.k2r.fwd_extra;
        T.dg_elems = T.extra_dg_off + T.k2r.dg_extra;
    }
    if (stem) T.fwd_elems = T.extra_fwd_off + T.stem.fwd_extra;

    int bw, bh, bn;
    const bool fwd_tma = tma_fwd_ok(c, &bw, &bh, &bn);
    DirPlan &F = T.fwd;
    if (stem) F.route = ROUTE_STEM;
    else if (k2r) F.route = ROUTE_K2R;
    else if (smallco) F.route = ROUTE_SMALLCO;
    else if (fwd_tma) {
        F.route = ROUTE_TMA;
        F.box_w = bw; F.box_h = bh; F.box_n = bn;
        F.bn = pick_bn(c->cout <= 32 ? 32 : L.rows_f, T.m_out, true, sms);
        F.halo = c->stride == 1 && c->kh <= 8 && halo_ok(c->kw, c->dil, bw, bh, bn, F.bn);
        T.fwd_tapmask = any_mask && !F.halo;
    } else {
        F.route = ROUTE_GATHER;
        F.bn = L.bn_f;
        T.fwd_tapmask = true;
    }

    DirPlan &D = T.dg;
    if (k2r) D.route = ROUTE_K2R;
    else if (smallco) D.route = ROUTE_SMALLCO;
    else if (L.rowpack) D.route = ROUTE_NONE;
    else if (c->stride == 1 && tile_box(c->w, c->h, &bw, &bh, &bn)) {
        D.route = ROUTE_TMA;
        D.box_w = bw; D.box_h = bh; D.box_n = bn;
        D.bn = pick_bn(L.ktap, T.m_in, false, sms);
        D.halo = c->kh <= 8 && halo_ok(c->kw, c->dil, bw, bh, bn, D.bn);
    } else if (tma_dgrad_s2_ok(c, &bw, &bh, &bn)) {
        D.route = ROUTE_TMA_S2;
        D.box_w = bw; D.box_h = bh; D.box_n = bn;
        const long long m_class = static_cast<long long>(c->n) * (c->h / 2) * (c->w / 2);
        D.bn = pick_bn(L.ktap, m_class, false, sms);
        for (int cls = 0; cls < 4; ++cls) T.cls_halo[cls] = halo_ok(class_kw(c, cls & 1), 1, bw, bh, bn, D.bn);
        T.cls_fork = ((m_class + BLOCK_M - 1) / BLOCK_M) * (L.ktap / D.bn) < sms;
    } else {
        D.route = ROUTE_GATHER;
        D.bn = (L.ktap % 128 == 0) ? 128 : 64;
    }

    const bool wg_tma = tma_wgrad_ok(c, &bw, &bh, &bn);
    DirPlan &W = T.wg;
    if (stem) W.route = ROUTE_STEM;
    else if (k2r) W.route = ROUTE_K2R;
    else if (smallco) W.route = ROUTE_SMALLCO;
    else if (wg_tma) {
        W.route = ROUTE_TMA;
        W.box_w = bw; W.box_h = bh; W.box_n = bn;
        W.halo = c->stride == 1 && c->kw == 3 && bw == 64 && bh == 1 && bn == 1 && 64 + (c->kw - 1) * c->dil <= 256;
        W.bn = (c->cout > 64 && T.m_out >= 128 * 64) ? 128 : 64;
        T.wg_tapmask = any_mask;
    } else {
        W.route = ROUTE_GATHER;
        T.wg_tapmask = true;
    }

    if (k2r) T.workspace = T.k2r.workspace;
    else if (stem) T.workspace = std::max(T.stem.workspace, tapmask_bytes(c));
    else {
        T.workspace = tapmask_bytes(c);
        if (fwd_tma || wg_tma)
            for (int p = 0; p < c->nparts; ++p)
                if (c->parts[p].x_up) { T.up_off[p] = T.workspace; T.workspace += up_bytes(c, p); }
    }

    T.fuses_epilogue = !smallco;
    T.dg_fuses_relu = c->nparts == 1 && !T.sp.ok && D.route == ROUTE_TMA;
    T.dg_at_source = smallco ? k2r : T.sp.ok;
    return T;
}

int a_operand_maps(const pcb_conv *c, const TcPlan &T, void *workspace, int bx, int by, int bn, CUtensorMap (&ta)[TC_MAX_PARTS],
                   int *use_fix, cudaStream_t st) {
    memset(ta, 0, sizeof(ta));
    for (int p = 0; p < c->nparts; ++p) {
        const pcb_part &pt = c->parts[p];
        const void *src = pt.x;
        long long cs = pt.x_cstride;
        const int c8 = rup(pt.c, 8);
        if (pt.x_up) {
            bf16 *up = reinterpret_cast<bf16 *>(static_cast<uint8_t *>(workspace) + T.up_off[p]);
            const long long pix = static_cast<long long>(c->n) * (c->h >> 1) * (c->w >> 1);
            const long long work = pix * (c8 >> 3);
            const int grid = static_cast<int>(std::min<long long>((work + 255) / 256, 16ll * pcb_num_sms()));
            upsample_part_kernel<<<grid, 256, 0, st>>>(static_cast<const bf16 *>(pt.x), pt.x_cstride, c8, pix, c->h >> 1, c->w >> 1, up);
            PCB_LAUNCH_CHECK();
            src = up; cs = c8;
        }
        if (pt.mask) *use_fix = 1;
        if (int rc = make_tmap_nhwc(&ta[p], src, c8, c->w, c->h, c->n, cs, bx, by, bn, c->stride)) return rc;
    }
    if (c->nparts < 2) ta[1] = ta[0];
    return 0;
}

pcb_smallco_layout smallco_layout(const Layout &L) {
    pcb_smallco_layout S;
    S.ktap = L.ktap; S.koff[0] = L.koff[0]; S.koff[1] = L.koff[1]; S.cout64 = L.cout64; S.kf = L.kf; S.kd = L.kd;
    return S;
}

}

bool pcb_tc_eligible(const pcb_conv *c) { return common_ok(c); }

size_t pcb_tc_workspace(const pcb_conv *c) { return tc_plan(c).workspace; }

void pcb_tc_weight_layout(const pcb_conv *c, size_t *fwd_elems, size_t *dgrad_elems) {
    const TcPlan T = tc_plan(c);
    *fwd_elems = T.fwd_elems;
    *dgrad_elems = T.dg_elems;
}

bool pcb_tc_subpixel(const pcb_conv *c) { return tc_plan(c).dg_at_source; }

void pcb_tc_routes(const pcb_conv *c, int32_t routes[3]) {
    static const int32_t code[] = {PCB_ROUTE_NONE, PCB_ROUTE_STEM, PCB_ROUTE_K2R, PCB_ROUTE_SMALLCO, PCB_ROUTE_TMA, PCB_ROUTE_TMA_S2,
                                   PCB_ROUTE_GATHER};
    const TcPlan T = tc_plan(c);
    routes[0] = code[T.fwd.route]; routes[1] = code[T.dg.route]; routes[2] = code[T.wg.route];
}

int pcb_tc_weight_prepare(const pcb_conv *c, const float *w_master, void *w_fwd, void *w_dgrad, bool zero_padding, cudaStream_t st) {
    const TcPlan T = tc_plan(c);
    const Layout &L = T.L;
    const size_t fe = T.fwd_elems, de = T.dg_elems;
    if (zero_padding) {
        PCB_CUDA(cudaMemsetAsync(w_fwd, 0, fe * 2, st));
        if (w_dgrad && de) PCB_CUDA(cudaMemsetAsync(w_dgrad, 0, de * 2, st));
    }
    WPrepParams W;
    memset(&W, 0, sizeof(W));
    W.cout = c->cout; W.taps = c->kh * c->kw; W.cin = c->cin; W.kw = c->kw; W.rowpack = L.rowpack; W.nparts = c->nparts;
    W.ktap = L.ktap; W.cout64 = L.cout64; W.kf = L.kf; W.kd = L.kd;
    int off = 0;
    for (int p = 0; p < c->nparts; ++p) { W.choff[p] = off; W.c[p] = c->parts[p].c; W.koff[p] = L.koff[p]; off += c->parts[p].c; }
    bf16 *wf = static_cast<bf16 *>(w_fwd), *wd = static_cast<bf16 *>(w_dgrad);
    if (!L.rowpack && W.taps <= 65535 && c->cout >= 32 && c->cin >= 32) {
        dim3 tg((c->cin + 31) / 32, (c->cout + 31) / 32, W.taps);
        tc_weight_prepare_tiled_kernel<<<tg, 256, 0, st>>>(w_master, W, wf, (w_dgrad && de) ? wd : nullptr);
    } else {
        const long long total = static_cast<long long>(c->cout) * W.taps * c->cin;
        const int grid = static_cast<int>(std::min<long long>((total + 1023) / 1024, 8ll * pcb_num_sms()));
        tc_weight_prepare_kernel<<<grid < 1 ? 1 : grid, 256, 0, st>>>(w_master, W, wf, (w_dgrad && de) ? wd : nullptr);
    }
    PCB_LAUNCH_CHECK();
    if (T.fwd.route == ROUTE_STEM) return pcb_stem_weight_prepare(c, T.stem, w_master, wf + T.extra_fwd_off, zero_padding, st);
    if (T.fwd.route == ROUTE_K2R) {
        PCB_CHECK(w_dgrad != nullptr, "kernel-to-row weights need the dgrad operand buffer");
        return pcb_k2r_weight_prepare(c, T.k2r, w_master, wf + T.extra_fwd_off, wd + T.extra_dg_off, zero_padding, st);
    }
    if (T.sp.ok) {
        PCB_CHECK(w_dgrad != nullptr, "sub-pixel weights need the dgrad operand buffer");
        return sp_weight_prepare(c, T.sp, L, w_master, wd + T.sp_off, st);
    }
    return 0;
}

int pcb_tc_forward_mask_pass(const pcb_conv *c, uint64_t *tapmask, cudaStream_t st) {
    const TcPlan T = tc_plan(c);
    PCB_CHECK(T.m_out < (1ll << 31), "problem too large");
    return T.fwd_tapmask ? launch_tapmask(c, tapmask, st) : 0;
}

bool pcb_tc_fuses_epilogue(const pcb_conv *c) { return tc_plan(c).fuses_epilogue; }

int pcb_tc_forward_ws(const pcb_conv *c, const void *w_fwd, const float *bias, void *y, int y_cstride, const float *msum,
                      uint64_t *tapmask, bool mask_pass_done, double *bn_sums, const pcb_ep *ep, cudaStream_t st) {
    int *flag = abort_flag_ptr();
    PCB_CHECK(flag != nullptr, "cudaMalloc(abort flag) failed");
    const TcPlan T = tc_plan(c);
    const Layout &L = T.L;
    const DirPlan &F = T.fwd;
    PCB_CHECK(T.m_out < (1ll << 31), "problem too large");
    PCB_CHECK(y_cstride % 8 == 0 && y_cstride >= c->cout, "tensor-core forward: y channel stride must be a multiple of 8 and >= cout");
    PCB_CHECK(bn_sums == nullptr || T.fuses_epilogue, "fused BatchNorm statistics requested from a kernel that does not produce them");
    PCB_CHECK(ep == nullptr || T.fuses_epilogue, "fused BatchNorm + activation requested from a kernel that does not apply it");
    if (!mask_pass_done && T.fwd_tapmask)
        if (int rc = launch_tapmask(c, tapmask, st)) return rc;
    const bf16 *wf = static_cast<const bf16 *>(w_fwd);
    if (F.route == ROUTE_STEM) return pcb_stem_forward(c, T.stem, wf + T.extra_fwd_off, bias, y, y_cstride, msum, tapmask, bn_sums, ep, st);
    if (F.route == ROUTE_K2R) return pcb_k2r_forward(c, T.k2r, smallco_layout(L), w_fwd, wf + T.extra_fwd_off, bias, y, y_cstride, msum, tapmask, st);
    if (F.route == ROUTE_SMALLCO) return pcb_smallco_forward(c, smallco_layout(L), w_fwd, bias, y, y_cstride, msum, st);
    TcParams P;
    base_params(P, c, L);
    P.m_total = static_cast<int>(T.m_out);
    fill_parts(c, L, P.parts, tapmask, T.m_out);
    P.bias = bias; P.msum = msum; P.y = static_cast<bf16 *>(y); P.y_cstride = y_cstride; P.abort_flag = flag;
    P.bn_sums = bn_sums; P.bn_c = c->cout;
    set_ep(P, ep);
    P.ncols = L.rows_f;
    CUtensorMap tm;
    if (int rc = make_tmap_2d(&tm, w_fwd, L.rows_f, L.kf, L.kf, F.bn)) return rc;
    if (F.route == ROUTE_TMA) {
        P.box_w = F.box_w; P.box_h = F.box_h; P.box_n = F.box_n;
        CUtensorMap ta[TC_MAX_PARTS];
        if (int rc = a_operand_maps(c, T, tapmask, F.box_w + (F.halo ? (c->kw - 1) * c->dil : 0), F.box_h, F.box_n, ta, &P.use_fix, st)) return rc;
        P.ncols = (c->cout <= 32) ? 32 : L.rows_f;
        P.wk_base = 0; P.wk_col = L.ktap; P.wk_row = c->kw * L.ktap;
        return launch_tma<0>(P, tm, ta[0], ta[1], F.bn, F.halo, st);
    }
    return launch_tc<0>(P, tm, F.bn, st);
}

bool pcb_tc_dgrad_fuses_relu(const pcb_conv *c) { return tc_plan(c).dg_fuses_relu; }

int pcb_tc_dgrad(const pcb_conv *c, const void *dc, int dc_cstride, const void *w_dgrad, void *const *dx, const int *dx_cstride,
                 cudaStream_t st, const void *relu_x, int relu_cstride) {
    const TcPlan T = tc_plan(c);
    const Layout &L = T.L;
    const DirPlan &D = T.dg;
    PCB_CHECK(D.route != ROUTE_NONE, "data gradient of a row-packed (cin <= 8) tensor-core layer: set force_generic and pass KRSC weights");
    PCB_CHECK(w_dgrad != nullptr && (reinterpret_cast<uintptr_t>(dc) & 15) == 0, "pcb_pconv_backward_data: w_dgrad required / dc misaligned");
    PCB_CHECK(relu_x == nullptr || (T.dg_fuses_relu && relu_cstride % 8 == 0 && relu_cstride >= rup(c->cin, 8) &&
                                    (reinterpret_cast<uintptr_t>(relu_x) & 15) == 0),
              "tensor-core dgrad: the ReLU backward is fused only on the TMA-fed stride-1 kernel (16-byte aligned input, channel stride %% 8 == 0)");
    int *flag = abort_flag_ptr();
    PCB_CHECK(flag != nullptr, "cudaMalloc(abort flag) failed");
    PCB_CHECK(T.m_in < (1ll << 31), "problem too large");
    PCB_CHECK(dc_cstride % 8 == 0 && dc_cstride >= rup(c->cout, 8), "tensor-core dgrad: dc channel stride must be a multiple of 8");
    const bf16 *wd = static_cast<const bf16 *>(w_dgrad);
    if (D.route == ROUTE_K2R) return pcb_k2r_dgrad(c, T.k2r, smallco_layout(L), dc, dc_cstride, w_dgrad, wd + T.extra_dg_off, dx, dx_cstride, st);
    if (D.route == ROUTE_SMALLCO) return pcb_smallco_dgrad(c, smallco_layout(L), dc, dc_cstride, w_dgrad, dx, dx_cstride, st);
    const SpPlan &SPL = T.sp;
    void *dx_local[TC_MAX_PARTS] = {nullptr, nullptr};
    for (int p = 0; p < c->nparts && p < TC_MAX_PARTS; ++p) dx_local[p] = dx[p];
    if (SPL.ok) {
        if (dx[SPL.pu] != nullptr)
            if (int rc = sp_dgrad_up(c, SPL, L, dc, dc_cstride, wd + T.sp_off, dx[SPL.pu], dx_cstride[SPL.pu], flag, st)) return rc;
        dx_local[SPL.pu] = nullptr;
        if (SPL.ps < 0 || dx[SPL.ps] == nullptr) return 0;
    }
    dx = dx_local;
    TcParams P;
    base_params(P, c, L);
    P.m_total = static_cast<int>(T.m_in);
    fill_parts(c, L, P.parts, nullptr, 0);
    for (int p = 0; p < c->nparts; ++p) {
        P.parts[p].dx = static_cast<bf16 *>(dx[p]);
        P.parts[p].dx_cstride = dx_cstride[p];
        PCB_CHECK(!dx[p] || (dx_cstride[p] % 8 == 0 && dx_cstride[p] >= P.parts[p].c8 && (reinterpret_cast<uintptr_t>(dx[p]) & 15) == 0),
                  "tensor-core dgrad: dx[%d] must be 16-byte aligned with a channel stride that is a multiple of 8", p);
    }
    P.dc = static_cast<const bf16 *>(dc); P.dc_cstride = dc_cstride; P.dc_c8 = rup(c->cout, 8); P.dc_kext = L.cout64;
    P.relu_x = static_cast<const bf16 *>(relu_x); P.relu_cstride = relu_cstride;
    P.abort_flag = flag;
    P.ncols = L.ktap;
    CUtensorMap tm;
    if (int rc = make_tmap_2d(&tm, w_dgrad, rup(L.ktap, 128), L.kd, L.kd, D.bn)) return rc;
    if (D.route == ROUTE_TMA) {
        P.box_w = D.box_w; P.box_h = D.box_h; P.box_n = D.box_n;
        P.wk_base = 0; P.wk_col = L.cout64; P.wk_row = c->kw * L.cout64;
        CUtensorMap ta;
        if (int rc = make_tmap_nhwc(&ta, dc, P.dc_c8, c->wo, c->ho, c->n, dc_cstride, D.box_w + (D.halo ? (c->kw - 1) * c->dil : 0), D.box_h, D.box_n, 1)) return rc;
        return launch_tma<1>(P, tm, ta, ta, D.bn, D.halo, st);
    }
    if (D.route == ROUTE_TMA_S2) {
        const int hh = c->h / 2, hw = c->w / 2;
        P.box_w = D.box_w; P.box_h = D.box_h; P.box_n = D.box_n;
        const bool fork = T.cls_fork;
        ClassStreams *CS = nullptr;
        if (fork) {
            if (int rc = class_streams(&CS)) return rc;
            PCB_CUDA(cudaEventRecord(CS->ev_fork, st));
        }
        for (int cls = 0; cls < 4; ++cls) {
            TcParams Q = P;
            const int py = cls >> 1, px = cls & 1;
            const int tr0 = (py + c->pad_h) & 1, tc0 = (px + c->pad_w) & 1;
            Q.kh = (c->kh - tr0 + 1) / 2; Q.kw = class_kw(c, px);
            Q.pad_h = (py + c->pad_h - tr0) / 2; Q.pad_w = (px + c->pad_w - tc0) / 2;
            Q.h = hh; Q.w = hw; Q.stride = 1; Q.dil = 1;
            Q.m_total = static_cast<int>(static_cast<long long>(c->n) * hh * hw);
            Q.sub = 2; Q.py = py; Q.px = px; Q.fh = c->h; Q.fw = c->w;
            Q.wk_base = (tr0 * c->kw + tc0) * L.cout64; Q.wk_row = 2 * c->kw * L.cout64; Q.wk_col = 2 * L.cout64;
            const bool halo = T.cls_halo[cls];
            CUtensorMap ta;
            if (int rc = make_tmap_nhwc(&ta, dc, P.dc_c8, c->wo, c->ho, c->n, dc_cstride, Q.box_w + (halo ? Q.kw - 1 : 0), Q.box_h, Q.box_n, 1)) return rc;
            cudaStream_t cs = (fork && cls > 0) ? CS->aux[cls - 1] : st;
            if (fork && cls > 0) PCB_CUDA(cudaStreamWaitEvent(cs, CS->ev_fork, 0));
            if (int rc = launch_tma<1>(Q, tm, ta, ta, D.bn, halo, cs)) return rc;
            if (fork && cls > 0) {
                PCB_CUDA(cudaEventRecord(CS->ev_join[cls - 1], cs));
                PCB_CUDA(cudaStreamWaitEvent(st, CS->ev_join[cls - 1], 0));
            }
        }
        return 0;
    }
    return launch_tc<1>(P, tm, D.bn, st);
}


template <int BLOCK_N, int T, bool HALO>
int launch_wgrad_tma(WgParams &P, const CUtensorMap &tdc, const CUtensorMap &ta0, const CUtensorMap &ta1, cudaStream_t st) {
    const int rows_a = 64 + (HALO ? (P.kw - 1) * P.dil : 0);
    PCB_CHECK(rows_a <= (HALO ? 3 : 1) * WGRAD_FIX_THREADS, "TMA-fed wgrad: %d-row A blocks exceed the fixer warps", rows_a);
    const size_t a_blk = (static_cast<size_t>(rows_a) * 128 + 1023) / 1024 * 1024;
    const size_t stage = (HALO ? 1 : T) * 2 * a_blk + static_cast<size_t>(BLOCK_N) * 128;
    P.stages = static_cast<int>(std::min<size_t>(MAX_RING, RING_BUDGET / stage));
    PCB_CHECK(P.stages >= 2, "TMA-fed wgrad: stage of %zu bytes does not fit twice", stage);
    const size_t smem = 1024 + P.stages * stage + 24 * MAX_RING;
    auto kern = pconv_tc_wgrad_tma_kernel<BLOCK_N, T, HALO>;
    PCB_SMEM_OPT_IN(kern, MAX_SMEM);
    P.tap_groups = HALO ? P.kh : (P.kh * P.kw + T - 1) / T;
    P.ci_tiles = (P.ktap + 127) / 128;
    const int co_tiles = (P.cout + BLOCK_N - 1) / BLOCK_N;
    const int base_ctas = co_tiles * P.tap_groups * P.ci_tiles;
    const int total_kb = (P.m_total + 63) / 64;
    int splits = (2 * pcb_num_sms() + base_ctas - 1) / base_ctas;
    splits = std::max(1, std::min(splits, total_kb));
    splits = std::min(splits, 65535);
    P.kb_per_split = (total_kb + splits - 1) / splits;
    splits = (total_kb + P.kb_per_split - 1) / P.kb_per_split;
    dim3 grid(base_ctas, splits);
    kern<<<grid, WGRAD_TMA_THREADS, smem, st>>>(P, tdc, ta0, ta1);
    PCB_LAUNCH_CHECK();
    return 0;
}

template <int BLOCK_N, int T, int STAGES>
static int launch_wgrad(WgParams &P, const CUtensorMap &tm, int cout, cudaStream_t st) {
    constexpr size_t smem = 1024 + STAGES * (T * 16384 + BLOCK_N * 128) + 24 * STAGES;
    auto kern = pconv_tc_wgrad_kernel<BLOCK_N, T, STAGES>;
    PCB_SMEM_OPT_IN(kern, (int)smem);
    P.tap_groups = (P.ntaps + T - 1) / T;
    P.ci_tiles = (P.ktap + 127) / 128;
    const int co_tiles = (cout + BLOCK_N - 1) / BLOCK_N;
    const int base_ctas = co_tiles * P.tap_groups * P.ci_tiles;
    const int total_kb = (P.m_total + 63) / 64;
    int splits = (4 * pcb_num_sms() + base_ctas - 1) / base_ctas;
    splits = std::max(1, std::min(splits, total_kb));
    splits = std::min(splits, 65535);
    P.kb_per_split = (total_kb + splits - 1) / splits;
    splits = (total_kb + P.kb_per_split - 1) / P.kb_per_split;
    dim3 grid(base_ctas, splits);
    kern<<<grid, WGRAD_THREADS, smem, st>>>(P, tm);
    PCB_LAUNCH_CHECK();
    return 0;
}

int pcb_tc_wgrad(const pcb_conv *c, const void *dc, int dc_cstride, float *dw, void *workspace, bool zero_dw, cudaStream_t st) {
    int *flag = abort_flag_ptr();
    PCB_CHECK(flag != nullptr, "cudaMalloc(abort flag) failed");
    PCB_CHECK(workspace != nullptr, "pcb_tc_wgrad: workspace required");
    const TcPlan T = tc_plan(c);
    const Layout &L = T.L;
    const DirPlan &W = T.wg;
    PCB_CHECK(T.m_out < (1ll << 31), "problem too large");
    PCB_CHECK(dc_cstride % 8 == 0 && dc_cstride >= c->cout, "tensor-core wgrad: dc channel stride must be a multiple of 8");
    if (W.route == ROUTE_STEM) return pcb_stem_wgrad(c, T.stem, dc, dc_cstride, dw, workspace, zero_dw, st);
    if (W.route == ROUTE_K2R) return pcb_k2r_wgrad(c, T.k2r, dc, dc_cstride, dw, workspace, zero_dw, st);
    if (W.route == ROUTE_SMALLCO) return pcb_smallco_wgrad(c, smallco_layout(L), dc, dc_cstride, dw, zero_dw, st);
    uint64_t *tapmask = static_cast<uint64_t *>(workspace);
    if (T.wg_tapmask)
        if (int rc = launch_tapmask(c, tapmask, st)) return rc;
    const size_t dw_bytes = sizeof(float) * c->cout * c->kh * c->kw * c->cin;
    if (zero_dw) PCB_CUDA(cudaMemsetAsync(dw, 0, dw_bytes, st));
    WgParams P;
    memset(&P, 0, sizeof(P));
    P.n = c->n; P.h = c->h; P.w = c->w; P.cin = c->cin; P.cout = c->cout; P.kh = c->kh; P.kw = c->kw; P.stride = c->stride;
    P.pad_h = c->pad_h; P.pad_w = c->pad_w; P.dil = c->dil; P.ho = c->ho; P.wo = c->wo; P.m_total = static_cast<int>(T.m_out);
    P.nparts = c->nparts; P.rowpack = L.rowpack; P.ktap = L.ktap; P.ntaps = L.rowpack ? c->kh : c->kh * c->kw;
    fill_parts(c, L, P.parts, tapmask, T.m_out);
    P.dw = dw; P.abort_flag = flag;
    CUtensorMap tm;
    if (int rc = make_tmap_2d(&tm, dc, T.m_out, c->cout, dc_cstride, 64)) return rc;
    if (W.route == ROUTE_TMA) {
        P.box_w = W.box_w; P.box_h = W.box_h; P.box_n = W.box_n;
        CUtensorMap ta[TC_MAX_PARTS];
        if (int rc = a_operand_maps(c, T, workspace, W.box_w + (W.halo ? (c->kw - 1) * c->dil : 0), W.box_h, W.box_n, ta, &P.use_fix, st)) return rc;
        if (W.bn == 128) return W.halo ? launch_wgrad_tma<128, 3, true>(P, tm, ta[0], ta[1], st) : launch_wgrad_tma<128, 3, false>(P, tm, ta[0], ta[1], st);
        return W.halo ? launch_wgrad_tma<64, 3, true>(P, tm, ta[0], ta[1], st) : launch_wgrad_tma<64, 3, false>(P, tm, ta[0], ta[1], st);
    }
    return launch_wgrad<64, 3, 3>(P, tm, c->cout, st);
}

int *pcb_tc_abort_flag() { return abort_flag_ptr(); }

int pcb_tc_read_abort_flag(int *value) {
    int *flag = abort_flag_ptr();
    PCB_CHECK(flag != nullptr, "no abort flag");
    PCB_CUDA(cudaMemcpy(value, flag, sizeof(int), cudaMemcpyDeviceToHost));
    if (*value != 0) cudaMemset(flag, 0, sizeof(int));
    return 0;
}
```

### text_segmentation_image_inpainting_b200/csrc/pcb_common.cuh

```cuda
#pragma once
#include <cuda_bf16.h>
#include <cuda_runtime.h>
#include <stdint.h>
#include <stdio.h>

#include "../../include/pconv_b200.h"

int pcb_set_error(const char *fmt, ...);
void pcb_count_launch(int n = 1);

#define PCB_CHECK(cond, ...)                       \
    do {                                           \
        if (!(cond)) return pcb_set_error(__VA_ARGS__); \
    } while (0)

#define PCB_CUDA(expr)                                                                           \
    do {                                                                                         \
        cudaError_t _e = (expr);                                                                 \
        if (_e != cudaSuccess)                                                                   \
            return pcb_set_error("%s:%d: %s -> %s", __FILE__, __LINE__, #expr, cudaGetErrorString(_e)); \
    } while (0)

#define PCB_LAUNCH_CHECK()                                                                        \
    do {                                                                                         \
        cudaError_t _e = cudaGetLastError();                                                     \
        if (_e != cudaSuccess)                                                                   \
            return pcb_set_error("%s:%d: kernel launch -> %s", __FILE__, __LINE__, cudaGetErrorString(_e)); \
        pcb_count_launch();                                                                      \
    } while (0)

constexpr int PCB_MAX_DEVICES = 64;

static inline int pcb_cur_device() {
    int dev = 0;
    cudaGetDevice(&dev);
    return (dev >= 0 && dev < PCB_MAX_DEVICES) ? dev : 0;
}

static inline int pcb_num_sms() {
    static int sms[PCB_MAX_DEVICES] = {0};
    const int dev = pcb_cur_device();
    if (!sms[dev]) {
        int v = 0;
        cudaDeviceGetAttribute(&v, cudaDevAttrMultiProcessorCount, dev);
        sms[dev] = v > 0 ? v : 132;
    }
    return sms[dev];
}

#define PCB_SMEM_OPT_IN(kern, bytes)                                                                          \
    do {                                                                                                      \
        static bool pcb_done_[PCB_MAX_DEVICES] = {};                                                          \
        const int pcb_dev_ = pcb_cur_device();                                                                \
        if (!pcb_done_[pcb_dev_]) {                                                                           \
            PCB_CUDA(cudaFuncSetAttribute(kern, cudaFuncAttributeMaxDynamicSharedMemorySize, (int)(bytes))); \
            pcb_done_[pcb_dev_] = true;                                                                       \
        }                                                                                                     \
    } while (0)

static inline size_t pcb_dtype_size(int dtype) { return dtype == PCB_BF16 ? 2 : 4; }

typedef __nv_bfloat16 bf16;

template <typename T> __device__ __forceinline__ float to_f32(T v);
template <> __device__ __forceinline__ float to_f32<float>(float v) { return v; }
template <> __device__ __forceinline__ float to_f32<bf16>(bf16 v) { return __bfloat162float(v); }

template <typename T> __device__ __forceinline__ T from_f32(float v);
template <> __device__ __forceinline__ float from_f32<float>(float v) { return v; }
template <> __device__ __forceinline__ bf16 from_f32<bf16>(float v) { return __float2bfloat16_rn(v); }

constexpr float PCB_SIGMOID_HALF_THRESHOLD = 8.940696716308594e-08f;
__device__ __forceinline__ bool sigmoid_above_half(float x) { return x > PCB_SIGMOID_HALF_THRESHOLD; }

__device__ __forceinline__ float apply_act(float z, int act, float slope) {
    if (act == PCB_ACT_RELU) return z > 0.f ? z : 0.f;
    if (act == PCB_ACT_LEAKY) return z > 0.f ? z : z * slope;
    if (act == PCB_ACT_RELU6) return fminf(fmaxf(z, 0.f), 6.f);
    return z;
}
__device__ __forceinline__ float act_grad(float z, int act, float slope) {
    if (act == PCB_ACT_RELU) return z > 0.f ? 1.f : 0.f;
    if (act == PCB_ACT_LEAKY) return z > 0.f ? 1.f : slope;
    if (act == PCB_ACT_RELU6) return (z > 0.f && z < 6.f) ? 1.f : 0.f;
    return 1.f;
}

template <typename T> struct Vec8;
template <> struct Vec8<bf16> {
    static __device__ __forceinline__ void load(const bf16 *p, float (&v)[8]) {
        uint4 r = *reinterpret_cast<const uint4 *>(p);
        const __nv_bfloat162 *h = reinterpret_cast<const __nv_bfloat162 *>(&r);
#pragma unroll
        for (int i = 0; i < 4; ++i) {
            float2 f = __bfloat1622float2(h[i]);
            v[2 * i] = f.x;
            v[2 * i + 1] = f.y;
        }
    }
    static __device__ __forceinline__ void store(bf16 *p, const float (&v)[8]) {
        uint4 r;
        __nv_bfloat162 *h = reinterpret_cast<__nv_bfloat162 *>(&r);
#pragma unroll
        for (int i = 0; i < 4; ++i) h[i] = __floats2bfloat162_rn(v[2 * i], v[2 * i + 1]);
        *reinterpret_cast<uint4 *>(p) = r;
    }
};
template <> struct Vec8<float> {
    static __device__ __forceinline__ void load(const float *p, float (&v)[8]) {
        float4 a = reinterpret_cast<const float4 *>(p)[0], b = reinterpret_cast<const float4 *>(p)[1];
        v[0] = a.x; v[1] = a.y; v[2] = a.z; v[3] = a.w; v[4] = b.x; v[5] = b.y; v[6] = b.z; v[7] = b.w;
    }
    static __device__ __forceinline__ void store(float *p, const float (&v)[8]) {
        reinterpret_cast<float4 *>(p)[0] = make_float4(v[0], v[1], v[2], v[3]);
        reinterpret_cast<float4 *>(p)[1] = make_float4(v[4], v[5], v[6], v[7]);
    }
};

__device__ __forceinline__ float warp_sum(float v) {
#pragma unroll
    for (int o = 16; o > 0; o >>= 1) v += __shfl_xor_sync(0xffffffffu, v, o);
    return v;
}

struct pcb_ep { const float *scale, *shift; int act; float slope; };

int pcb_generic_forward(const pcb_conv *c, const void *w, const float *bias, void *y, int y_cstride, const float *msum, cudaStream_t st);
int pcb_generic_dgrad(const pcb_conv *c, const void *dc, int dc_cstride, const void *w_krsc, void *const *dx, const int *dx_cstride,
                      cudaStream_t st);
int pcb_generic_wgrad(const pcb_conv *c, const void *dc, int dc_cstride, float *dw, bool zero_dw, cudaStream_t st);
int pcb_mask_sums(const pcb_conv *c, float *msum, uint8_t *newmask, cudaStream_t st);
bool pcb_tc_eligible(const pcb_conv *c);
size_t pcb_tc_workspace(const pcb_conv *c);
void pcb_tc_weight_layout(const pcb_conv *c, size_t *fwd_elems, size_t *dgrad_elems);
int pcb_tc_weight_prepare(const pcb_conv *c, const float *w_master, void *w_fwd, void *w_dgrad, bool zero_padding, cudaStream_t st);
int pcb_tc_forward_mask_pass(const pcb_conv *c, uint64_t *tapmask, cudaStream_t st);
int pcb_tc_forward_ws(const pcb_conv *c, const void *w_fwd, const float *bias, void *y, int y_cstride, const float *msum,
                      uint64_t *tapmask, bool mask_pass_done, double *bn_sums, const pcb_ep *ep, cudaStream_t st);
bool pcb_tc_fuses_epilogue(const pcb_conv *c);
bool pcb_tc_subpixel(const pcb_conv *c);
int pcb_tc_dgrad(const pcb_conv *c, const void *dc, int dc_cstride, const void *w_dgrad, void *const *dx, const int *dx_cstride,
                 cudaStream_t st, const void *relu_x = nullptr, int relu_cstride = 0);
bool pcb_tc_dgrad_fuses_relu(const pcb_conv *c);
int pcb_tc_wgrad(const pcb_conv *c, const void *dc, int dc_cstride, float *dw, void *workspace, bool zero_dw, cudaStream_t st);
int pcb_tc_read_abort_flag(int *value);
int *pcb_tc_abort_flag();
void pcb_tc_routes(const pcb_conv *c, int32_t routes[3]);
struct pcb_smallco_layout { int ktap, koff[2], cout64; long long kf, kd; };
bool pcb_smallco_eligible(const pcb_conv *c);
int pcb_smallco_forward(const pcb_conv *c, const pcb_smallco_layout &L, const void *w_fwd, const float *bias, void *y, int y_cstride, const float *msum,
                        cudaStream_t st);
int pcb_smallco_dgrad(const pcb_conv *c, const pcb_smallco_layout &L, const void *dc, int dc_cstride, const void *w_dgrad, void *const *dx, const int *dx_cstride,
                      cudaStream_t st);
int pcb_smallco_wgrad(const pcb_conv *c, const pcb_smallco_layout &L, const void *dc, int dc_cstride, float *dw, bool zero_dw, cudaStream_t st);
struct K2rPlan {
    bool ok;
    int pu, ps;
    int cu, cs, choff_u, choff_s;
    pcb_conv sub;
    size_t sub_fe, sub_de;
    size_t fwd_extra, dg_extra;
    size_t workspace;
};
K2rPlan pcb_k2r_plan(const pcb_conv *c);
int pcb_k2r_weight_prepare(const pcb_conv *c, const K2rPlan &K, const float *w_master, void *w_fwd_extra, void *w_dg_extra, bool zero_padding,
                           cudaStream_t st);
int pcb_k2r_forward(const pcb_conv *c, const K2rPlan &K, const pcb_smallco_layout &L, const void *w_fwd, const void *w_fwd_extra, const float *bias,
                    void *y, int y_cstride, const float *msum, void *workspace, cudaStream_t st);
int pcb_k2r_dgrad(const pcb_conv *c, const K2rPlan &K, const pcb_smallco_layout &L, const void *dc, int dc_cstride, const void *w_dgrad,
                  const void *w_dg_extra, void *const *dx, const int *dx_cstride, cudaStream_t st);
int pcb_k2r_wgrad(const pcb_conv *c, const K2rPlan &K, const void *dc, int dc_cstride, float *dw, void *workspace, bool zero_dw, cudaStream_t st);
struct StemPlan {
    bool ok;
    int sc;
    size_t fwd_extra;
    size_t workspace;
};
StemPlan pcb_stem_plan(const pcb_conv *c);
int pcb_stem_weight_prepare(const pcb_conv *c, const StemPlan &K, const float *w_master, void *w_fwd_extra, bool zero_padding, cudaStream_t st);
int pcb_stem_forward(const pcb_conv *c, const StemPlan &K, const void *w_fwd_extra, const float *bias, void *y, int y_cstride,
                     const float *msum, void *workspace, double *bn_sums, const pcb_ep *ep, cudaStream_t st);
int pcb_stem_wgrad(const pcb_conv *c, const StemPlan &K, const void *dc, int dc_cstride, float *dw, void *workspace, bool zero_dw,
                   cudaStream_t st);
bool pcb_dw_eligible(const pcb_conv *c);
int pcb_dw_weight_prepare(const pcb_conv *c, const float *w_master, void *w_t, cudaStream_t st);
int pcb_dw_forward(const pcb_conv *c, const void *w_t, const float *bias, void *y, int y_cstride, const float *msum, double *bn_sums,
                   const pcb_ep *ep, cudaStream_t st);
int pcb_dw_dgrad(const pcb_conv *c, const void *dc, int dc_cstride, const void *w_t, void *dx, int dx_cstride, cudaStream_t st);
int pcb_dw_wgrad(const pcb_conv *c, const void *dc, int dc_cstride, float *dw, bool zero_dw, cudaStream_t st);
```

### text_segmentation_image_inpainting_b200/csrc/pcb_ptx.cuh

```cuda
#pragma once
#include <cuda.h>
#include <cuda_runtime.h>
#include <stdint.h>

namespace ptx {

__device__ __forceinline__ uint32_t smem_u32(const void *p) { return static_cast<uint32_t>(__cvta_generic_to_shared(p)); }

__device__ __forceinline__ bool elect_one() {
    uint32_t pred = 0;
    asm volatile(
        "{\n\t.reg .pred P;\n\telect.sync _|P, 0xffffffff;\n\tselp.b32 %0, 1, 0, P;\n\t}" : "=r"(pred));
    return pred != 0;
}

__device__ __forceinline__ void mbar_init(uint32_t bar, uint32_t count) {
    asm volatile("mbarrier.init.shared::cta.b64 [%0], %1;" ::"r"(bar), "r"(count) : "memory");
}
__device__ __forceinline__ void fence_mbar_init() { asm volatile("fence.mbarrier_init.release.cluster;" ::: "memory"); }
__device__ __forceinline__ void mbar_arrive(uint32_t bar) {
    asm volatile("mbarrier.arrive.shared::cta.b64 _, [%0];" ::"r"(bar) : "memory");
}
__device__ __forceinline__ void mbar_arrive_expect_tx(uint32_t bar, uint32_t bytes) {
    asm volatile("mbarrier.arrive.expect_tx.shared::cta.b64 _, [%0], %1;" ::"r"(bar), "r"(bytes) : "memory");
}
__device__ __forceinline__ bool mbar_try_wait(uint32_t bar, uint32_t parity) {
    uint32_t ok;
    asm volatile(
        "{\n\t.reg .pred P;\n\t"
        "mbarrier.try_wait.parity.shared::cta.b64 P, [%1], %2;\n\t"
        "selp.b32 %0, 1, 0, P;\n\t}"
        : "=r"(ok)
        : "r"(bar), "r"(parity)
        : "memory");
    return ok != 0;
}
__device__ __forceinline__ bool mbar_wait(uint32_t bar, uint32_t parity, int *abort_flag, int code) {
    if (mbar_try_wait(bar, parity)) return true;
    const long long t0 = clock64();
    for (uint32_t it = 1;; ++it) {
        if (mbar_try_wait(bar, parity)) return true;
        if ((it & 63) == 0) {
            if (*reinterpret_cast<volatile int *>(abort_flag) != 0) return false;
            if (clock64() - t0 > 4000000000ll) break;
        }
    }
    atomicCAS(abort_flag, 0, code);
    return false;
}
__device__ __forceinline__ void cp_async_mbar_arrive(uint32_t bar) {
    asm volatile("cp.async.mbarrier.arrive.shared::cta.b64 [%0];" ::"r"(bar) : "memory");
}

__device__ __forceinline__ void cp_async_16(uint32_t dst, const void *src, bool valid) {
    const uint32_t sz = valid ? 16u : 0u;
    asm volatile("cp.async.cg.shared.global [%0], [%1], 16, %2;" ::"r"(dst), "l"(src), "r"(sz) : "memory");
}
__device__ __forceinline__ void cp_async_16_ca(uint32_t dst, const void *src, bool valid) {
    const uint32_t sz = valid ? 16u : 0u;
    asm volatile("cp.async.ca.shared.global [%0], [%1], 16, %2;" ::"r"(dst), "l"(src), "r"(sz) : "memory");
}
__device__ __forceinline__ void cp_async_commit() { asm volatile("cp.async.commit_group;" ::: "memory"); }
template <int N> __device__ __forceinline__ void cp_async_wait() { asm volatile("cp.async.wait_group %0;" ::"n"(N) : "memory"); }

__device__ __forceinline__ void fence_proxy_async_smem() { asm volatile("fence.proxy.async.shared::cta;" ::: "memory"); }

__device__ __forceinline__ void prefetch_tmap(const CUtensorMap *m) {
    asm volatile("prefetch.tensormap [%0];" ::"l"(reinterpret_cast<uint64_t>(m)) : "memory");
}
__device__ __forceinline__ void tma_load_2d(uint32_t dst, const CUtensorMap *m, int c0, int c1, uint32_t bar) {
    asm volatile(
        "cp.async.bulk.tensor.2d.shared::cluster.global.mbarrier::complete_tx::bytes [%0], [%1, {%3, %4}], [%2];"
        ::"r"(dst), "l"(reinterpret_cast<uint64_t>(m)), "r"(bar), "r"(c0), "r"(c1)
        : "memory");
}
__device__ __forceinline__ void tma_load_4d(uint32_t dst, const CUtensorMap *m, int c0, int c1, int c2, int c3, uint32_t bar) {
    asm volatile(
        "cp.async.bulk.tensor.4d.shared::cluster.global.mbarrier::complete_tx::bytes [%0], [%1, {%3, %4, %5, %6}], [%2];"
        ::"r"(dst), "l"(reinterpret_cast<uint64_t>(m)), "r"(bar), "r"(c0), "r"(c1), "r"(c2), "r"(c3)
        : "memory");
}

__device__ __forceinline__ void wgmma_fence() { asm volatile("wgmma.fence.sync.aligned;" ::: "memory"); }
__device__ __forceinline__ void wgmma_commit() { asm volatile("wgmma.commit_group.sync.aligned;" ::: "memory"); }
template <int N> __device__ __forceinline__ void wgmma_wait() { asm volatile("wgmma.wait_group.sync.aligned %0;" ::"n"(N) : "memory"); }
template <int R> __device__ __forceinline__ void wgmma_fence_regs(float (&d)[R]) {
#pragma unroll
    for (int i = 0; i < R; ++i) asm volatile("" : "+f"(d[i])::"memory");
}
template <int TA, int TB> __device__ __forceinline__ void wgmma_m64n32(float (&d)[16], uint64_t a_desc, uint64_t b_desc) {
    asm volatile(
        "{\n\t"
        "wgmma.mma_async.sync.aligned.m64n32k16.f32.bf16.bf16 "
        "{%0, %1, %2, %3, %4, %5, %6, %7, %8, %9, %10, %11, %12, %13, %14, %15}, %16, %17, 1, 1, 1, %18, %19;\n\t"
        "}"
        : "+f"(d[0]), "+f"(d[1]), "+f"(d[2]), "+f"(d[3]), "+f"(d[4]), "+f"(d[5]), "+f"(d[6]), "+f"(d[7]), "+f"(d[8]), "+f"(d[9]), "+f"(d[10]), "+f"(d[11]), "+f"(d[12]), "+f"(d[13]), "+f"(d[14]), "+f"(d[15])
        : "l"(a_desc), "l"(b_desc), "n"(TA), "n"(TB));
}
template <int TA, int TB, int R> __device__ __forceinline__ void wgmma_m64n64(float (&d)[R], uint64_t a_desc, uint64_t b_desc) {
    static_assert(R >= 32, "m64n64 accumulator");
    asm volatile(
        "{\n\t"
        "wgmma.mma_async.sync.aligned.m64n64k16.f32.bf16.bf16 "
        "{%0, %1, %2, %3, %4, %5, %6, %7, %8, %9, %10, %11, %12, %13, %14, %15, %16, %17, %18, %19, %20, %21, %22, %23, %24, %25, %26, %27, %28, %29, %30, %31}, %32, %33, 1, 1, 1, %34, %35;\n\t"
        "}"
        : "+f"(d[0]), "+f"(d[1]), "+f"(d[2]), "+f"(d[3]), "+f"(d[4]), "+f"(d[5]), "+f"(d[6]), "+f"(d[7]), "+f"(d[8]), "+f"(d[9]), "+f"(d[10]), "+f"(d[11]), "+f"(d[12]), "+f"(d[13]), "+f"(d[14]), "+f"(d[15]), "+f"(d[16]), "+f"(d[17]), "+f"(d[18]), "+f"(d[19]), "+f"(d[20]), "+f"(d[21]), "+f"(d[22]), "+f"(d[23]), "+f"(d[24]), "+f"(d[25]), "+f"(d[26]), "+f"(d[27]), "+f"(d[28]), "+f"(d[29]), "+f"(d[30]), "+f"(d[31])
        : "l"(a_desc), "l"(b_desc), "n"(TA), "n"(TB));
}
template <int TA, int TB> __device__ __forceinline__ void wgmma_m64n128(float (&d)[64], uint64_t a_desc, uint64_t b_desc) {
    asm volatile(
        "{\n\t"
        "wgmma.mma_async.sync.aligned.m64n128k16.f32.bf16.bf16 "
        "{%0, %1, %2, %3, %4, %5, %6, %7, %8, %9, %10, %11, %12, %13, %14, %15, %16, %17, %18, %19, %20, %21, %22, %23, %24, %25, %26, %27, %28, %29, %30, %31, %32, %33, %34, %35, %36, %37, %38, %39, %40, %41, %42, %43, %44, %45, %46, %47, %48, %49, %50, %51, %52, %53, %54, %55, %56, %57, %58, %59, %60, %61, %62, %63}, %64, %65, 1, 1, 1, %66, %67;\n\t"
        "}"
        : "+f"(d[0]), "+f"(d[1]), "+f"(d[2]), "+f"(d[3]), "+f"(d[4]), "+f"(d[5]), "+f"(d[6]), "+f"(d[7]), "+f"(d[8]), "+f"(d[9]), "+f"(d[10]), "+f"(d[11]), "+f"(d[12]), "+f"(d[13]), "+f"(d[14]), "+f"(d[15]), "+f"(d[16]), "+f"(d[17]), "+f"(d[18]), "+f"(d[19]), "+f"(d[20]), "+f"(d[21]), "+f"(d[22]), "+f"(d[23]), "+f"(d[24]), "+f"(d[25]), "+f"(d[26]), "+f"(d[27]), "+f"(d[28]), "+f"(d[29]), "+f"(d[30]), "+f"(d[31]), "+f"(d[32]), "+f"(d[33]), "+f"(d[34]), "+f"(d[35]), "+f"(d[36]), "+f"(d[37]), "+f"(d[38]), "+f"(d[39]), "+f"(d[40]), "+f"(d[41]), "+f"(d[42]), "+f"(d[43]), "+f"(d[44]), "+f"(d[45]), "+f"(d[46]), "+f"(d[47]), "+f"(d[48]), "+f"(d[49]), "+f"(d[50]), "+f"(d[51]), "+f"(d[52]), "+f"(d[53]), "+f"(d[54]), "+f"(d[55]), "+f"(d[56]), "+f"(d[57]), "+f"(d[58]), "+f"(d[59]), "+f"(d[60]), "+f"(d[61]), "+f"(d[62]), "+f"(d[63])
        : "l"(a_desc), "l"(b_desc), "n"(TA), "n"(TB));
}
template <int N, int TA, int TB> __device__ __forceinline__ void wgmma_bf16(float (&d)[N / 2], uint64_t a_desc, uint64_t b_desc) {
    if constexpr (N == 32) wgmma_m64n32<TA, TB>(d, a_desc, b_desc);
    else if constexpr (N == 64) wgmma_m64n64<TA, TB>(d, a_desc, b_desc);
    else if constexpr (N == 128) wgmma_m64n128<TA, TB>(d, a_desc, b_desc);
    else {
        static_assert(N == 256 && TB == 0, "wgmma tile width");
        wgmma_m64n128<TA, TB>(*reinterpret_cast<float (*)[64]>(&d[0]), a_desc, b_desc);
        wgmma_m64n128<TA, TB>(*reinterpret_cast<float (*)[64]>(&d[64]), a_desc, b_desc + (16384 >> 4));
    }
}
template <int N> __device__ __forceinline__ void setmaxnreg_inc() { asm volatile("setmaxnreg.inc.sync.aligned.u32 %0;" ::"n"(N)); }
template <int N> __device__ __forceinline__ void setmaxnreg_dec() { asm volatile("setmaxnreg.dec.sync.aligned.u32 %0;" ::"n"(N)); }
__device__ __forceinline__ void named_sync(int id, int threads) { asm volatile("bar.sync %0, %1;" ::"r"(id), "r"(threads) : "memory"); }

__host__ __device__ __forceinline__ uint64_t make_smem_desc(uint32_t smem_addr, uint32_t lbo_bytes, uint32_t sbo_bytes) {
    uint64_t d = 0;
    d |= static_cast<uint64_t>((smem_addr >> 4) & 0x3FFFu);
    d |= static_cast<uint64_t>((lbo_bytes >> 4) & 0x3FFFu) << 16;
    d |= static_cast<uint64_t>((sbo_bytes >> 4) & 0x3FFFu) << 32;
    d |= 1ull << 62;
    return d;
}

}
```

### text_segmentation_image_inpainting_b200/csrc/pcb_tc_epi.cuh

```cuda
#pragma once
#include <cuda.h>

#include "pcb_common.cuh"
#include "pcb_ptx.cuh"

namespace {

constexpr int BLOCK_M = 128;
constexpr int BLOCK_K = 64;
constexpr int A_STAGE_BYTES = BLOCK_M * 128;
constexpr int NUM_PRODUCER_THREADS = 128;
constexpr int TC_MAX_PARTS = 2;
constexpr int MMA_WARPS = 8;
constexpr int MMA_THREADS = MMA_WARPS * 32;
constexpr int acc_pitch(int block_n) { return block_n + 4; }
constexpr int acc_stage_bytes(int block_n) { return BLOCK_M * acc_pitch(block_n) * 4; }

inline int rup(int v, int m) { return (v + m - 1) / m * m; }

struct TcPart {
    const bf16 *x;
    const uint64_t *tapmask;
    const uint8_t *mask;
    bf16 *dx;
    int c, c8, kext, koff, choff, cstride, xup, mup, dx_cstride;
};

struct TcParams {
    int n, h, w, cin, cout, kh, kw, stride, pad_h, pad_w, dil, ho, wo;
    int m_total;
    int nparts, no_guard, rowpack;
    int ncols;
    int ring_a, ring_b;
    int ktap;
    TcPart parts[TC_MAX_PARTS];
    const float *bias; const float *msum; bf16 *y; int y_cstride;
    const bf16 *dc; int dc_cstride, dc_c8, dc_kext;
    const bf16 *relu_x; int relu_cstride;
    int *abort_flag;
    int box_w, box_h, box_n, stages, use_fix;
    int wk_base, wk_row, wk_col;
    int sub, py, px, fh, fw;
    double *bn_sums;
    int bn_c;
    const float *ep_scale, *ep_shift;
    int ep_on, ep_act;
    float ep_slope;
};

constexpr int STAT_SLICE = 256;
constexpr int STAT_SMEM_BYTES = MMA_WARPS * STAT_SLICE * 4 + 16;
constexpr int EPI_WARPS = 4;
constexpr int EPI_STAT_SLICE = 512;
constexpr int EPI_STAT_SQ = EPI_STAT_SLICE / 2;
constexpr int EPI_STAT_SMEM_BYTES = EPI_WARPS * EPI_STAT_SLICE * 4;
constexpr int bf16_pitch(int block_n) { return block_n + 8; }
constexpr int bf16_stage_bytes(int block_n) { return BLOCK_M * bf16_pitch(block_n) * 2; }

__device__ __forceinline__ float warp_transpose_sum16(float (&v)[16], int lane) {
#pragma unroll
    for (int i = 0; i < 16; ++i) v[i] += __shfl_xor_sync(0xffffffffu, v[i], 16);
#pragma unroll
    for (int off = 8, n = 16; off >= 1; off >>= 1, n >>= 1) {
        const bool upper = (lane & off) != 0;
#pragma unroll
        for (int i = 0; i < 8; ++i) {
            if (i < (n >> 1)) {
                const float send = upper ? v[i] : v[i + (n >> 1)];
                const float keep = upper ? v[i + (n >> 1)] : v[i];
                v[i] = keep + __shfl_xor_sync(0xffffffffu, send, off);
            }
        }
    }
    return v[0];
}

__device__ __forceinline__ uint32_t align1024(uint32_t a) { return (a + 1023u) & ~1023u; }

struct EpiRow {
    long long mo;
    int m;
    bool rvalid, hole;
    float inv;
    float dscale[TC_MAX_PARTS];
};

template <int MODE>
__device__ __forceinline__ EpiRow tc_epi_row(const TcParams &P, int m, bool renorm = true) {
    EpiRow er;
    er.m = m;
    er.rvalid = m < P.m_total;
    er.inv = 0.f;
    er.hole = false;
    er.mo = m;
    int en = 0, eh = 0, ew = 0;
    if (MODE == 1 && er.rvalid) {
        en = m / (P.h * P.w); const int rem = m - en * P.h * P.w; eh = rem / P.w; ew = rem - eh * P.w;
        eh = eh * P.sub + P.py; ew = ew * P.sub + P.px;
        er.mo = (static_cast<long long>(en) * P.fh + eh) * P.fw + ew;
    }
    if (MODE == 0 && er.rvalid && renorm) {
        const float s = P.msum ? P.msum[er.mo] : 1.f;
        er.hole = (s == 0.f) && !P.no_guard;
        er.inv = er.hole ? 0.f : 1.0f / s;
    }
#pragma unroll
    for (int p = 0; p < TC_MAX_PARTS; ++p) {
        er.dscale[p] = 1.f;
        if (MODE == 1 && p < P.nparts) {
            const TcPart &pt = P.parts[p];
            if (er.rvalid && pt.dx != nullptr && pt.mask != nullptr)
                er.dscale[p] = pt.mask[(static_cast<long long>(en) * (P.fh >> pt.mup) + (eh >> pt.mup)) * (P.fw >> pt.mup) + (ew >> pt.mup)] ? 1.f : 0.f;
        }
    }
    return er;
}

template <int BLOCK_N>
__device__ __forceinline__ void tc_stats_flush(const TcParams &P, float *s_stat, int lane, int n0, int cb, int ce, int sq_off) {
    __syncwarp();
    for (int c0 = cb; c0 < ce; c0 += 32) {
        const int co = n0 + c0 + lane;
        if (co < P.bn_c) {
            atomicAdd(P.bn_sums + co, static_cast<double>(s_stat[c0 - cb + lane]));
            atomicAdd(P.bn_sums + P.bn_c + co, static_cast<double>(s_stat[sq_off + c0 - cb + lane]));
        }
        s_stat[c0 - cb + lane] = 0.f; s_stat[sq_off + c0 - cb + lane] = 0.f;
    }
    __syncwarp();
}

template <int BLOCK_N>
__device__ __forceinline__ void tc_stats_final(const TcParams &P, const float *stat_base, int w, int lane, int stat_n0) {
    for (int col = w * 32 + lane; col < BLOCK_N; col += EPI_WARPS * 32) {
        const int co = stat_n0 + col;
        if (co < P.bn_c) {
            float a = 0.f, q = 0.f;
#pragma unroll
            for (int w4 = 0; w4 < EPI_WARPS; ++w4) { a += stat_base[w4 * EPI_STAT_SLICE + col]; q += stat_base[w4 * EPI_STAT_SLICE + EPI_STAT_SQ + col]; }
            atomicAdd(P.bn_sums + co, static_cast<double>(a));
            atomicAdd(P.bn_sums + P.bn_c + co, static_cast<double>(q));
        }
    }
}

template <int R> __device__ __forceinline__ void zero_acc(float (&a)[R]) {
#pragma unroll
    for (int i = 0; i < R; ++i) a[i] = 0.f;
}

constexpr int MAX_RING = 8;

constexpr int EPI_WARP0 = MMA_WARPS + 4;
constexpr int TMA_THREADS = (EPI_WARP0 + EPI_WARPS) * 32;
constexpr int TMA_FIX_THREADS = 96;
constexpr int TMA_REGS = 128;
constexpr int TMA_CONSUMER_REGS = 192, TMA_SUPPORT_REGS = 64;
static_assert(TMA_THREADS == 512 && 2 * 128 * TMA_CONSUMER_REGS + 2 * 128 * TMA_SUPPORT_REGS == TMA_THREADS * TMA_REGS &&
              TMA_THREADS * TMA_REGS <= 65536, "TMA-fed fwd / dgrad register budget");

constexpr size_t TMA_BAR_BYTES = 24 * MAX_RING + 16;

template <int BLOCK_N, int MODE>
__device__ __forceinline__ void tc_epilogue_bf16(const TcParams &P, const EpiRow &er, const bf16 *srow, int lane, int n0, float *s_stat) {
    const bool stats = (MODE == 0) && (s_stat != nullptr);
#pragma unroll 1
    for (int c0 = 0; c0 < BLOCK_N; c0 += 32) {
        const int col = n0 + c0;
        bf16 *orow = nullptr;
        int nstore = 0;
        int xlocal = 0;
        float scale = 1.f;
        if (MODE == 0) {
            if (er.rvalid && col < P.y_cstride) { orow = P.y + er.mo * P.y_cstride + col; nstore = min(32, P.y_cstride - col); }
        } else {
#pragma unroll
            for (int p = 0; p < TC_MAX_PARTS; ++p) {
                if (p >= P.nparts) break;
                const TcPart &pt = P.parts[p];
                const int local = col - pt.koff;
                if (local >= 0 && local < pt.kext && pt.dx != nullptr && local < pt.c8 && er.rvalid) {
                    orow = pt.dx + er.mo * pt.dx_cstride + local;
                    nstore = min(32, pt.c8 - local);
                    scale = er.dscale[p];
                    xlocal = local;
                }
            }
        }
        if (nstore == 0 && !stats) continue;
        uint4 o[4];
#pragma unroll
        for (int j = 0; j < 4; ++j) o[j] = reinterpret_cast<const uint4 *>(srow + c0)[j];
        if (MODE == 1 && scale != 1.f) {
            __nv_bfloat162 *ob = reinterpret_cast<__nv_bfloat162 *>(o);
#pragma unroll
            for (int j = 0; j < 16; ++j) {
                const float2 f = __bfloat1622float2(ob[j]);
                ob[j] = __floats2bfloat162_rn(f.x * scale, f.y * scale);
            }
        }
// ... 146 lines not shown
```

Before: 1161.

## Split K across thread-block clusters for under-occupied TMA convolutions with DSMEM reduction

Adds a cluster-based split-K mode to the TMA wgmma convolution kernels. When a layer launches too few tiles to fill the SMs, several CTAs in a cluster each take a slice of the K loop, and rank 0 sums their partial accumulators through distributed shared memory before running the epilogue. The mask-sum kernel is also tightened: it uses 32-bit indexing, trims out-of-bounds taps up front and reads the mask directly. This trades extra cluster synchronisation and DSMEM traffic for better SM utilisation on small deep layers.

```diff
diff --git a/include/pconv_b200.h b/include/pconv_b200.h
--- a/include/pconv_b200.h
+++ b/include/pconv_b200.h
@@ -81,6 +81,7 @@
 enum { PCB_ROUTE_NONE = 0, PCB_ROUTE_GENERIC = 1, PCB_ROUTE_DEPTHWISE = 2, PCB_ROUTE_STEM = 3, PCB_ROUTE_K2R = 4,
        PCB_ROUTE_SMALLCO = 5, PCB_ROUTE_TMA = 6, PCB_ROUTE_TMA_S2 = 7, PCB_ROUTE_GATHER = 8 };
 int pcb_debug_conv_routes(const pcb_conv *c, int32_t routes[3]);
+int pcb_debug_conv_ksplit(const pcb_conv *c, int32_t out[2]);
 
 int pcb_mask_planes_from_dense(const float *mask_nchw, int n, int c, int h, int w, uint8_t *planes, pcb_stream_t stream);
 int pcb_mask_plane_to_dense(const uint8_t *plane, int n, int h, int w, int up, float *dst_nchw, int ctot, int c0, int c,
diff --git a/text_segmentation_image_inpainting_b200/_lib.py b/text_segmentation_image_inpainting_b200/_lib.py
--- a/text_segmentation_image_inpainting_b200/_lib.py
+++ b/text_segmentation_image_inpainting_b200/_lib.py
@@ -52,6 +52,7 @@
     "pcb_pconv_backward_weight_acc": (c_int, [ctypes.POINTER(Conv), c_void_p, c_int, c_void_p, c_void_p, c_void_p]),
     "pcb_debug_pipeline_status": (c_int, [ctypes.POINTER(c_int)]),
     "pcb_debug_conv_routes": (c_int, [ctypes.POINTER(Conv), ctypes.POINTER(ctypes.c_int32)]),
+    "pcb_debug_conv_ksplit": (c_int, [ctypes.POINTER(Conv), ctypes.POINTER(ctypes.c_int32)]),
     "pcb_mask_planes_from_dense": (c_int, [c_void_p, c_int, c_int, c_int, c_int, c_void_p, c_void_p]),
     "pcb_mask_plane_to_dense": (c_int, [c_void_p, c_int, c_int, c_int, c_int, c_void_p, c_int, c_int, c_int, c_void_p]),
     "pcb_bn_stats": (c_int, [c_void_p, c_int, c_ll, c_int, c_void_p, c_void_p, c_void_p]),
diff --git a/text_segmentation_image_inpainting_b200/csrc/api.cu b/text_segmentation_image_inpainting_b200/csrc/api.cu
--- a/text_segmentation_image_inpainting_b200/csrc/api.cu
+++ b/text_segmentation_image_inpainting_b200/csrc/api.cu
@@ -229,3 +229,14 @@
     routes[0] = routes[1] = routes[2] = (f == FAMILY_DW) ? PCB_ROUTE_DEPTHWISE : PCB_ROUTE_GENERIC;
     return 0;
 }
+
+PCB_API int pcb_debug_conv_ksplit(const pcb_conv *c, int32_t out[2]) {
+    PCB_CHECK(out != nullptr, "null out");
+    if (int rc = validate(c, false)) return rc;
+    if (family_of(c) == FAMILY_TC) {
+        pcb_tc_ksplit(c, out);
+        return 0;
+    }
+    out[0] = out[1] = 1;
+    return 0;
+}
diff --git a/text_segmentation_image_inpainting_b200/csrc/conv_generic.cu b/text_segmentation_image_inpainting_b200/csrc/conv_generic.cu
--- a/text_segmentation_image_inpainting_b200/csrc/conv_generic.cu
+++ b/text_segmentation_image_inpainting_b200/csrc/conv_generic.cu
@@ -36,15 +36,21 @@
     return pt.mask[(static_cast<long long>(nn) * (G.h >> pt.mup) + (hi >> pt.mup)) * (G.w >> pt.mup) + (wi >> pt.mup)] != 0;
 }
 
-__global__ void mask_sums_kernel(const GParams G, float *msum, uint8_t *newmask) {
-    const long long plane = static_cast<long long>(G.ho) * G.wo;
-    const long long total = plane * G.n;
-    const long long m = blockIdx.x * static_cast<long long>(blockDim.x) + threadIdx.x;
+__global__ void __launch_bounds__(256) mask_sums_kernel(const GParams G, float *msum, uint8_t *newmask) {
+    const int plane = G.ho * G.wo;
+    const int total = plane * G.n;
+    const int m = static_cast<int>(blockIdx.x) * 256 + static_cast<int>(threadIdx.x);
     if (m >= total) return;
     const int mg = (G.groups > 1 && !G.same_holes) ? G.groups : 1;
-    const int nn = static_cast<int>(m / plane);
-    const int rem = static_cast<int>(m - nn * plane), oh = rem / G.wo, ow = rem - oh * G.wo;
+    const int nn = m / plane;
+    const int rem = m - nn * plane, oh = rem / G.wo, ow = rem - oh * G.wo;
     const int cig = G.cin / G.groups;
+    const int y0 = oh * G.stride - G.pad_h, x0 = ow * G.stride - G.pad_w;
+    int tr0 = 0, tr1 = G.kh, tc0 = 0, tc1 = G.kw;
+    while (tr0 < tr1 && y0 + tr0 * G.dil < 0) ++tr0;
+    while (tr1 > tr0 && y0 + (tr1 - 1) * G.dil >= G.h) --tr1;
+    while (tc0 < tc1 && x0 + tc0 * G.dil < 0) ++tc0;
+    while (tc1 > tc0 && x0 + (tc1 - 1) * G.dil >= G.w) --tc1;
     for (int g = 0; g < mg; ++g) {
         if (G.plain) { msum[g * total + m] = 1.f; newmask[g * total + m] = 1; continue; }
         int s = 0;
@@ -58,13 +64,18 @@
                 weight = max(0, hi - lo);
             }
             if (weight == 0) continue;
-            int cnt = 0;
-            for (int tr = 0; tr < G.kh; ++tr)
-                for (int tc = 0; tc < G.kw; ++tc) {
-                    const int hi = oh * G.stride - G.pad_h + tr * G.dil, wi = ow * G.stride - G.pad_w + tc * G.dil;
-                    if (hi < 0 || hi >= G.h || wi < 0 || wi >= G.w) continue;
-                    cnt += mask_at(G, p, nn, hi, wi) ? 1 : 0;
-                }
+            const uint8_t *mk = G.parts[p].mask;
+            int cnt = (tr1 - tr0) * (tc1 - tc0);
+            if (mk != nullptr) {
+                const int mup = G.parts[p].mup, mw = G.w >> mup;
+                const uint8_t *base = mk + static_cast<long long>(nn) * (G.h >> mup) * mw;
+                cnt = 0;
+                for (int tr = tr0; tr < tr1; ++tr) {
+                    const uint8_t *row = base + ((y0 + tr * G.dil) >> mup) * mw;
+#pragma unroll 4
+                    for (int tc = tc0; tc < tc1; ++tc) cnt += __ldg(row + ((x0 + tc * G.dil) >> mup)) != 0 ? 1 : 0;
+                }
+            }
             s += cnt * weight;
         }
         msum[g * total + m] = static_cast<float>(s);
@@ -322,6 +333,7 @@
     GParams G;
     fill(G, c);
     const long long total = static_cast<long long>(c->n) * c->ho * c->wo;
+    PCB_CHECK(total < (1ll << 31) && static_cast<long long>(c->n) * c->h * c->w < (1ll << 31), "mask sums: problem too large");
     mask_sums_kernel<<<static_cast<unsigned>((total + 255) / 256), 256, 0, st>>>(G, msum, newmask);
     PCB_LAUNCH_CHECK();
     return 0;
diff --git a/text_segmentation_image_inpainting_b200/csrc/conv_tc.cu b/text_segmentation_image_inpainting_b200/csrc/conv_tc.cu
--- a/text_segmentation_image_inpainting_b200/csrc/conv_tc.cu
+++ b/text_segmentation_image_inpainting_b200/csrc/conv_tc.cu
@@ -423,6 +423,7 @@
     const uint32_t acc_full = sBar + 24 * MAX_RING, acc_empty = acc_full + 8;
     const uint32_t s_stat_addr = sBar + TMA_BAR_BYTES;
     const uint32_t s_acc = s_stat_addr + EPI_STAT_SMEM_BYTES;
+    const uint32_t partials_ready = s_acc + bf16_stage_bytes(BLOCK_N), released = partials_ready + 8;
     uint8_t *smem_gen = smem_raw + (smem_base - ptx::smem_u32(smem_raw));
 
     const int warp = __shfl_sync(0xffffffffu, threadIdx.x >> 5, 0), lane = threadIdx.x & 31;
@@ -430,10 +431,16 @@
     const int n_tiles = P.ncols / BLOCK_N;
     const int m_tiles = (P.m_total + BLOCK_M - 1) / BLOCK_M;
     const int num_tiles = m_tiles * n_tiles;
-    const int tile0 = static_cast<int>(blockIdx.x), tstep = static_cast<int>(gridDim.x);
     auto m0_of = [&](int mt) -> int { return mt * BLOCK_M; };
     const bool fix = (MODE == 0) && P.use_fix;
     const int kwi = HALO ? 1 : P.kw;
+    const int ks = (BLOCK_N <= 128 && P.ksplit > 1) ? P.ksplit : 1;
+    const int rank = ks > 1 ? static_cast<int>(ptx::cluster_ctarank()) : 0;
+    const int tile0 = static_cast<int>(blockIdx.x) / ks, tstep = static_cast<int>(gridDim.x) / ks;
+    const int kst = P.kh * kwi *
+                    (((MODE == 0) ? P.parts[0].kext : P.dc_kext) + ((MODE == 0 && np > 1) ? P.parts[1].kext : 0)) / BLOCK_K;
+    const int k_lo = static_cast<int>(static_cast<long long>(rank) * kst / ks);
+    const int k_hi = static_cast<int>(static_cast<long long>(rank + 1) * kst / ks);
 
     auto tile_active = [&](int n0) -> bool {
         if (MODE == 0) return true;
@@ -447,10 +454,12 @@
             ptx::mbar_init(bar_full + 8 * s, 1); ptx::mbar_init(bar_fixed + 8 * s, TMA_FIX_THREADS / 32); ptx::mbar_init(bar_empty + 8 * s, 2);
         }
         ptx::mbar_init(acc_full, MMA_WARPS); ptx::mbar_init(acc_empty, EPI_WARPS);
+        ptx::mbar_init(partials_ready, ks - 1 > 0 ? ks - 1 : 1); ptx::mbar_init(released, 1);
         ptx::fence_mbar_init();
     }
     if (warp == 8 && lane == 0) { ptx::prefetch_tmap(&tmap_w); ptx::prefetch_tmap(&tmap_a0); if (np > 1) ptx::prefetch_tmap(&tmap_a1); }
     __syncthreads();
+    if (ks > 1) ptx::cluster_arrive();
 
     float *s_stat = nullptr;
     int stat_n0 = -1;
@@ -478,15 +487,17 @@
         for (int tile = tile0; tile < num_tiles && !dead; tile += tstep) {
             const int n0 = (tile % n_tiles) * BLOCK_N;
             if (!tile_active(n0)) continue;
-            const ConsRows cr = cons_rows<MODE>(P, m0_of(tile / n_tiles), e, lane);
+            const ConsRows cr = rank == 0 ? cons_rows<MODE>(P, m0_of(tile / n_tiles), e, lane) : ConsRows{};
             float acc[BLOCK_N / 2];
             zero_acc(acc);
             int held = -1;
+            int q = 0;
             for (int r = 0; r < rows_a && !dead; ++r) {
 #pragma unroll
                 for (int p = 0; p < TC_MAX_PARTS; ++p) {
                     const int nbp = (p == 0) ? nb0 : nb1, klast = (p == 0) ? kl0 : kl1;
-                    for (int cb = 0; cb < nbp; ++cb) {
+                    for (int cb = 0; cb < nbp; ++cb, ++q) {
+                        if (q < k_lo || q >= k_hi) continue;
                         if (!__all_sync(0xffffffffu, ptx::mbar_wait(ready + 8 * s, ph, P.abort_flag, 124))) { dead = true; break; }
                         uint64_t da = desc_a0 + static_cast<uint64_t>(s * stage16 + shift0), db = desc_b0 + static_cast<uint64_t>(s * stage16);
                         const int ksteps = (cb + 1 < nbp) ? 4 : klast;
@@ -512,6 +523,34 @@
             ptx::wgmma_fence_regs(acc);
             if (held >= 0 && leader) ptx::mbar_arrive(bar_empty + 8 * held);
             if (dead) break;
+            if (ks > 1) {
+                const uint32_t part = smem_base + 16u * threadIdx.x;
+                if (rank > 0) {
+                    ptx::named_sync(2, MMA_THREADS);
+                    float4 *dst = reinterpret_cast<float4 *>(smem_gen) + threadIdx.x;
+#pragma unroll
+                    for (int j = 0; j < BLOCK_N / 8; ++j)
+                        dst[j * MMA_THREADS] = make_float4(acc[4 * j], acc[4 * j + 1], acc[4 * j + 2], acc[4 * j + 3]);
+                    ptx::named_sync(2, MMA_THREADS);
+                    ptx::cluster_wait();
+                    if (threadIdx.x == 0) ptx::mbar_arrive_remote(ptx::mapa(partials_ready, 0));
+                    __all_sync(0xffffffffu, ptx::mbar_wait_cluster(released, 0, P.abort_flag, 128));
+                    break;
+                }
+                if (!__all_sync(0xffffffffu, ptx::mbar_wait_cluster(partials_ready, 0, P.abort_flag, 127))) break;
+#pragma unroll 1
+                for (int pr = 1; pr < ks; ++pr) {
+                    const uint32_t src = ptx::mapa(part, static_cast<uint32_t>(pr));
+#pragma unroll
+                    for (int j = 0; j < BLOCK_N / 8; ++j) {
+                        const float4 v = ptx::ld_dsmem_f4(src + 16u * MMA_THREADS * j);
+                        acc[4 * j] += v.x; acc[4 * j + 1] += v.y; acc[4 * j + 2] += v.z; acc[4 * j + 3] += v.w;
+                    }
+                }
+                ptx::named_sync(2, MMA_THREADS);
+                if (threadIdx.x == 0)
+                    for (int pr = 1; pr < ks; ++pr) ptx::mbar_arrive_remote(ptx::mapa(released, static_cast<uint32_t>(pr)));
+            }
             if (!tma_stage_tile<BLOCK_N, MODE>(P, acc, acc_stage, acc_full, acc_empty, aph, e, lane, n0, cr, 125)) break;
         }
     } else {
@@ -524,7 +563,8 @@
                 m0 = m0_of(tile / n_tiles); n0 = (tile % n_tiles) * BLOCK_N;
                 if (!tile_active(n0)) n0 = -1;
             };
-            tma_epilogue_warps<BLOCK_N, MODE>(P, tile0, tstep, num_tiles, origin, acc_stage, acc_full, acc_empty, s_stat, stat_n0, w, lane, 126);
+            tma_epilogue_warps<BLOCK_N, MODE>(P, tile0, tstep, rank == 0 ? num_tiles : 0, origin, acc_stage, acc_full, acc_empty, s_stat,
+                                              stat_n0, w, lane, 126);
             ptx::named_sync(1, EPI_WARPS * 32);
             if (s_stat != nullptr && stat_n0 >= 0) tc_stats_final<BLOCK_N>(P, s_stat - w * EPI_STAT_SLICE, w, lane, stat_n0);
         } else if (warp == 8) {
@@ -544,13 +584,15 @@
                 const int x_org = (MODE == 0) ? ox * P.stride - P.pad_w : (HALO ? ox + P.pad_w - hx : ox + P.pad_w);
                 const int y_org = (MODE == 0) ? oy * P.stride - P.pad_h : oy + P.pad_h;
                 int krow = P.wk_base;
+                int q = 0;
                 for (int tr = 0, y = y_org; tr < P.kh && !dead; ++tr, y += dstep, krow += row_k)
                     for (int ti = 0, x = x_org, kidx = krow; ti < kwi && !dead; ++ti, x += dstep, kidx = krow + ti * col_k) {
 #pragma unroll
                         for (int p = 0; p < TC_MAX_PARTS; ++p) {
                             const int kext = (p == 0) ? kext0 : kext1;
                             const CUtensorMap *ma = (p == 0) ? &tmap_a0 : &tmap_a1;
-                            for (int c0 = 0; c0 < kext; c0 += BLOCK_K, kidx += BLOCK_K) {
+                            for (int c0 = 0; c0 < kext; c0 += BLOCK_K, kidx += BLOCK_K, ++q) {
+                                if (q < k_lo || q >= k_hi) continue;
                                 if (!__all_sync(0xffffffffu, ptx::mbar_wait(bar_empty + 8 * s, ph, P.abort_flag, 121))) { dead = true; break; }
                                 if (ptx::elect_one()) {
                                     const uint32_t full = bar_full + 8 * s, dst = smem_base + s * STAGE;
@@ -603,6 +645,7 @@
                         load_words(tile + tstep);
                         if (MODE == 1 && !tile_active((tile % n_tiles) * BLOCK_N)) continue;
                         const int taps = P.kh * P.kw;
+                        int q = 0;
                         for (int tap = 0; tap < taps && !dead; ++tap) {
 #pragma unroll
                             for (int p = 0; p < TC_MAX_PARTS; ++p) {
@@ -615,7 +658,8 @@
                                 }
                                 const bool any_hole = __any_sync(0xffffffffu, mine);
                                 const int nb = ((MODE == 0) ? P.parts[p].kext : P.dc_kext) / BLOCK_K;
-                                for (int cb = 0; cb < nb; ++cb) {
+                                for (int cb = 0; cb < nb; ++cb, ++q) {
+                                    if (q < k_lo || q >= k_hi) continue;
                                     if (!ptx::mbar_wait(bar_full + 8 * s, ph, P.abort_flag, 122)) { dead = true; break; }
                                     if (any_hole) {
 #pragma unroll
@@ -665,6 +709,7 @@
                         for (int r = 0; r < FR; ++r) cb_bits[r] = nb_bits[r];
                         load_bits(tile + tstep, nb_bits);
                         if (MODE == 1 && !tile_active((tile % n_tiles) * BLOCK_N)) continue;
+                        int q = 0;
                         for (int tr = 0; tr < P.kh && !dead; ++tr) {
 #pragma unroll
                             for (int p = 0; p < TC_MAX_PARTS; ++p) {
@@ -674,7 +719,8 @@
                                 for (int r = 0; r < FR; ++r) { hole[r] = (cb_bits[r] >> (p * 8 + tr)) & 1u; mine = mine || hole[r]; }
                                 const bool any_hole = __any_sync(0xffffffffu, mine);
                                 const int nb = ((MODE == 0) ? P.parts[p].kext : P.dc_kext) / BLOCK_K;
-                                for (int cb = 0; cb < nb; ++cb) {
+                                for (int cb = 0; cb < nb; ++cb, ++q) {
+                                    if (q < k_lo || q >= k_hi) continue;
                                     if (!ptx::mbar_wait(bar_full + 8 * s, ph, P.abort_flag, 122)) { dead = true; break; }
                                     if (any_hole) {
 #pragma unroll
@@ -1605,24 +1651,72 @@
 }
 
 size_t tma_fixed_smem(int block_n) {
-    return 1024 + TMA_BAR_BYTES + EPI_STAT_SMEM_BYTES + bf16_stage_bytes(block_n);
+    return 1024 + TMA_BAR_BYTES + EPI_STAT_SMEM_BYTES + bf16_stage_bytes(block_n) + 16;
+}
+
+size_t tma_stage_bytes(int block_n, bool halo, int kw, int dil) {
+    const size_t a_room = (static_cast<size_t>(BLOCK_M + (halo ? (kw - 1) * dil : 0)) * 128 + 1023) / 1024 * 1024;
+    return a_room + static_cast<size_t>(halo ? kw : 1) * block_n * 128;
+}
+int tma_stages(int block_n, bool halo, int kw, int dil) {
+    return static_cast<int>(std::min<size_t>(MAX_RING, (MAX_SMEM - tma_fixed_smem(block_n)) / tma_stage_bytes(block_n, halo, kw, dil)));
+}
+
+int tma_ksplit(long long ctas, int par, int kstages, int sms, int block_n, bool halo, int kw, int dil) {
+    const long long busy = ctas * par;
+    if (2 * busy >= sms || block_n > 128) return 1;
+    if (static_cast<size_t>(tma_stages(block_n, halo, kw, dil)) * tma_stage_bytes(block_n, halo, kw, dil) < static_cast<size_t>(block_n) * 512)
+        return 1;
+    int s = 1;
+    while (s < 8 && busy * (s + 1) <= sms && kstages / (s + 1) >= 8) ++s;
+    return s;
 }
 
 template <int BLOCK_N, int MODE, bool HALO>
 int launch_tma_n(TcParams &P, const CUtensorMap &tw, const CUtensorMap &ta0, const CUtensorMap &ta1, cudaStream_t st) {
-    const int nb = HALO ? P.kw : 1;
-    const size_t a_room = (static_cast<size_t>(BLOCK_M + (HALO ? (P.kw - 1) * P.dil : 0)) * 128 + 1023) / 1024 * 1024;
-    const size_t stage = a_room + static_cast<size_t>(nb) * BLOCK_N * 128;
+    const size_t stage = tma_stage_bytes(BLOCK_N, HALO, P.kw, P.dil);
     const size_t fixed = tma_fixed_smem(BLOCK_N);
-    P.stages = static_cast<int>(std::min<size_t>(MAX_RING, (MAX_SMEM - fixed) / stage));
+    P.stages = tma_stages(BLOCK_N, HALO, P.kw, P.dil);
     PCB_CHECK(P.stages >= 2, "TMA-fed conv: stage of %zu bytes does not fit twice", stage);
     const size_t smem = fixed + P.stages * stage;
     auto kern = pconv_tc_tma_kernel<BLOCK_N, MODE, HALO>;
     PCB_SMEM_OPT_IN(kern, MAX_SMEM);
     const int m_tiles = (P.m_total + BLOCK_M - 1) / BLOCK_M;
     const int num_tiles = m_tiles * (P.ncols / BLOCK_N);
-    const int grid = std::min(num_tiles, pcb_num_sms());
-    kern<<<grid, TMA_THREADS, smem, st>>>(P, tw, ta0, ta1);
+    if (P.ksplit > 1) {
+        static int fits[PCB_MAX_DEVICES][9] = {};
+        static size_t fits_smem[PCB_MAX_DEVICES][9] = {};
+        const int dev = pcb_cur_device();
+        while (P.ksplit > 1) {
+            const int s = P.ksplit;
+            if (fits_smem[dev][s] != smem) {
+                cudaLaunchConfig_t q = {};
+                cudaLaunchAttribute qa[1];
+                q.gridDim = dim3(static_cast<unsigned>(num_tiles * s)); q.blockDim = dim3(TMA_THREADS); q.dynamicSmemBytes = smem;
+                qa[0].id = cudaLaunchAttributeClusterDimension; qa[0].val.clusterDim.x = s; qa[0].val.clusterDim.y = 1; qa[0].val.clusterDim.z = 1;
+                q.attrs = qa; q.numAttrs = 1;
+                int n = 0;
+                PCB_CUDA(cudaOccupancyMaxActiveClusters(&n, kern, &q));
+                fits[dev][s] = n; fits_smem[dev][s] = smem;
+            }
+            if (fits[dev][s] >= num_tiles) break;
+            --P.ksplit;
+        }
+    }
+    if (P.ksplit > 1) {
+        cudaLaunchConfig_t cfg = {};
+        cudaLaunchAttribute at[1];
+        cfg.gridDim = dim3(static_cast<unsigned>(num_tiles * P.ksplit)); cfg.blockDim = dim3(TMA_THREADS);
+        cfg.dynamicSmemBytes = smem; cfg.stream = st;
+        at[0].id = cudaLaunchAttributeClusterDimension;
+        at[0].val.clusterDim.x = P.ksplit; at[0].val.clusterDim.y = 1; at[0].val.clusterDim.z = 1;
+        cfg.attrs = at; cfg.numAttrs = 1;
+        PCB_CUDA(cudaLaunchKernelEx(&cfg, kern, P, tw, ta0, ta1));
+    } else {
+        P.ksplit = 1;
+        const int grid = std::min(num_tiles, pcb_num_sms());
+        kern<<<grid, TMA_THREADS, smem, st>>>(P, tw, ta0, ta1);
+    }
     PCB_LAUNCH_CHECK();
     return 0;
 }
@@ -1844,6 +1938,7 @@
     int box_w, box_h, box_n;
     int bn;
     bool halo;
+    int ksplit;
 };
 
 struct TcPlan {
@@ -1862,6 +1957,7 @@
     SpPlan sp;
     bool cls_halo[4];
     bool cls_fork;
+    int cls_ksplit[4];
     bool fuses_epilogue;
     bool dg_fuses_relu;
     bool dg_at_source;
@@ -1909,6 +2005,9 @@
         F.box_w = bw; F.box_h = bh; F.box_n = bn;
         F.bn = pick_bn(c->cout <= 32 ? 32 : L.rows_f, T.m_out, true, sms);
         F.halo = c->stride == 1 && c->kh <= 8 && halo_ok(c->kw, c->dil, bw, bh, bn, F.bn);
+        const int fcols = c->cout <= 32 ? 32 : L.rows_f;
+        F.ksplit = tma_ksplit(((T.m_out + BLOCK_M - 1) / BLOCK_M) * (fcols / F.bn), 1, c->kh * (F.halo ? 1 : c->kw) * (L.ktap / BLOCK_K),
+                              sms, F.bn, F.halo, c->kw, c->dil);
         T.fwd_tapmask = any_mask && !F.halo;
     } else {
         F.route = ROUTE_GATHER;
@@ -1925,13 +2024,23 @@
         D.box_w = bw; D.box_h = bh; D.box_n = bn;
         D.bn = pick_bn(L.ktap, T.m_in, false, sms);
         D.halo = c->kh <= 8 && halo_ok(c->kw, c->dil, bw, bh, bn, D.bn);
+        D.ksplit = tma_ksplit(((T.m_in + BLOCK_M - 1) / BLOCK_M) * (L.ktap / D.bn), 1, c->kh * (D.halo ? 1 : c->kw) * (L.cout64 / BLOCK_K),
+                              sms, D.bn, D.halo, c->kw, c->dil);
     } else if (tma_dgrad_s2_ok(c, &bw, &bh, &bn)) {
         D.route = ROUTE_TMA_S2;
         D.box_w = bw; D.box_h = bh; D.box_n = bn;
         const long long m_class = static_cast<long long>(c->n) * (c->h / 2) * (c->w / 2);
         D.bn = pick_bn(L.ktap, m_class, false, sms);
         for (int cls = 0; cls < 4; ++cls) T.cls_halo[cls] = halo_ok(class_kw(c, cls & 1), 1, bw, bh, bn, D.bn);
-        T.cls_fork = ((m_class + BLOCK_M - 1) / BLOCK_M) * (L.ktap / D.bn) < sms;
+        const long long cls_ctas = ((m_class + BLOCK_M - 1) / BLOCK_M) * (L.ktap / D.bn);
+        T.cls_fork = cls_ctas < sms;
+        D.ksplit = 1;
+        for (int cls = 0; cls < 4; ++cls) {
+            const int kh_c = (c->kh - (((cls >> 1) + c->pad_h) & 1) + 1) / 2, kw_c = class_kw(c, cls & 1);
+            T.cls_ksplit[cls] = tma_ksplit(cls_ctas, T.cls_fork ? 4 : 1, kh_c * (T.cls_halo[cls] ? 1 : kw_c) * (L.cout64 / BLOCK_K), sms,
+                                           D.bn, T.cls_halo[cls], kw_c, 1);
+            D.ksplit = std::max(D.ksplit, T.cls_ksplit[cls]);
+        }
     } else {
         D.route = ROUTE_GATHER;
         D.bn = (L.ktap % 128 == 0) ? 128 : 64;
@@ -2011,6 +2120,12 @@
 }
 
 bool pcb_tc_subpixel(const pcb_conv *c) { return tc_plan(c).dg_at_source; }
+
+void pcb_tc_ksplit(const pcb_conv *c, int32_t out[2]) {
+    const TcPlan T = tc_plan(c);
+    out[0] = std::max(1, T.fwd.ksplit);
+    out[1] = std::max(1, T.dg.ksplit);
+}
 
 void pcb_tc_routes(const pcb_conv *c, int32_t routes[3]) {
     static const int32_t code[] = {PCB_ROUTE_NONE, PCB_ROUTE_STEM, PCB_ROUTE_K2R, PCB_ROUTE_SMALLCO, PCB_ROUTE_TMA, PCB_ROUTE_TMA_S2,
@@ -2096,6 +2211,7 @@
         if (int rc = a_operand_maps(c, T, tapmask, F.box_w + (F.halo ? (c->kw - 1) * c->dil : 0), F.box_h, F.box_n, ta, &P.use_fix, st)) return rc;
         P.ncols = (c->cout <= 32) ? 32 : L.rows_f;
         P.wk_base = 0; P.wk_col = L.ktap; P.wk_row = c->kw * L.ktap;
+        P.ksplit = F.ksplit;
         return launch_tma<0>(P, tm, ta[0], ta[1], F.bn, F.halo, st);
     }
     return launch_tc<0>(P, tm, F.bn, st);
@@ -2151,6 +2267,7 @@
         P.wk_base = 0; P.wk_col = L.cout64; P.wk_row = c->kw * L.cout64;
         CUtensorMap ta;
         if (int rc = make_tmap_nhwc(&ta, dc, P.dc_c8, c->wo, c->ho, c->n, dc_cstride, D.box_w + (D.halo ? (c->kw - 1) * c->dil : 0), D.box_h, D.box_n, 1)) return rc;
+        P.ksplit = D.ksplit;
         return launch_tma<1>(P, tm, ta, ta, D.bn, D.halo, st);
     }
     if (D.route == ROUTE_TMA_S2) {
@@ -2173,6 +2290,7 @@
             Q.sub = 2; Q.py = py; Q.px = px; Q.fh = c->h; Q.fw = c->w;
             Q.wk_base = (tr0 * c->kw + tc0) * L.cout64; Q.wk_row = 2 * c->kw * L.cout64; Q.wk_col = 2 * L.cout64;
             const bool halo = T.cls_halo[cls];
+            Q.ksplit = T.cls_ksplit[cls];
             CUtensorMap ta;
             if (int rc = make_tmap_nhwc(&ta, dc, P.dc_c8, c->wo, c->ho, c->n, dc_cstride, Q.box_w + (halo ? Q.kw - 1 : 0), Q.box_h, Q.box_n, 1)) return rc;
             cudaStream_t cs = (fork && cls > 0) ? CS->aux[cls - 1] : st;
diff --git a/text_segmentation_image_inpainting_b200/csrc/pcb_common.cuh b/text_segmentation_image_inpainting_b200/csrc/pcb_common.cuh
--- a/text_segmentation_image_inpainting_b200/csrc/pcb_common.cuh
+++ b/text_segmentation_image_inpainting_b200/csrc/pcb_common.cuh
@@ -146,6 +146,7 @@
 int pcb_tc_read_abort_flag(int *value);
 int *pcb_tc_abort_flag();
 void pcb_tc_routes(const pcb_conv *c, int32_t routes[3]);
+void pcb_tc_ksplit(const pcb_conv *c, int32_t out[2]);
 struct pcb_smallco_layout { int ktap, koff[2], cout64; long long kf, kd; };
 bool pcb_smallco_eligible(const pcb_conv *c);
 int pcb_smallco_forward(const pcb_conv *c, const pcb_smallco_layout &L, const void *w_fwd, const float *bias, void *y, int y_cstride, const float *msum,
diff --git a/text_segmentation_image_inpainting_b200/csrc/pcb_ptx.cuh b/text_segmentation_image_inpainting_b200/csrc/pcb_ptx.cuh
--- a/text_segmentation_image_inpainting_b200/csrc/pcb_ptx.cuh
+++ b/text_segmentation_image_inpainting_b200/csrc/pcb_ptx.cuh
@@ -40,6 +40,50 @@
     const long long t0 = clock64();
     for (uint32_t it = 1;; ++it) {
         if (mbar_try_wait(bar, parity)) return true;
+        if ((it & 63) == 0) {
+            if (*reinterpret_cast<volatile int *>(abort_flag) != 0) return false;
+            if (clock64() - t0 > 4000000000ll) break;
+        }
+    }
+    atomicCAS(abort_flag, 0, code);
+    return false;
+}
+__device__ __forceinline__ uint32_t cluster_ctarank() {
+    uint32_t r;
+    asm volatile("mov.u32 %0, %%cluster_ctarank;" : "=r"(r));
+    return r;
+}
+__device__ __forceinline__ uint32_t mapa(uint32_t addr, uint32_t rank) {
+    uint32_t r;
+    asm volatile("mapa.shared::cluster.u32 %0, %1, %2;" : "=r"(r) : "r"(addr), "r"(rank));
+    return r;
+}
+__device__ __forceinline__ void mbar_arrive_remote(uint32_t remote_bar) {
+    asm volatile("mbarrier.arrive.release.cluster.shared::cluster.b64 _, [%0];" ::"r"(remote_bar) : "memory");
+}
+__device__ __forceinline__ float4 ld_dsmem_f4(uint32_t remote_addr) {
+    float4 v;
+    asm volatile("ld.shared::cluster.v4.f32 {%0, %1, %2, %3}, [%4];" : "=f"(v.x), "=f"(v.y), "=f"(v.z), "=f"(v.w) : "r"(remote_addr) : "memory");
+    return v;
+}
+__device__ __forceinline__ void cluster_arrive() { asm volatile("barrier.cluster.arrive.release;" ::: "memory"); }
+__device__ __forceinline__ void cluster_wait() { asm volatile("barrier.cluster.wait.acquire;" ::: "memory"); }
+__device__ __forceinline__ bool mbar_try_wait_cluster(uint32_t bar, uint32_t parity) {
+    uint32_t ok;
+    asm volatile(
+        "{\n\t.reg .pred P;\n\t"
+        "mbarrier.try_wait.parity.acquire.cluster.shared::cta.b64 P, [%1], %2;\n\t"
+        "selp.b32 %0, 1, 0, P;\n\t}"
+        : "=r"(ok)
+        : "r"(bar), "r"(parity)
+        : "memory");
+    return ok != 0;
+}
+__device__ __forceinline__ bool mbar_wait_cluster(uint32_t bar, uint32_t parity, int *abort_flag, int code) {
+    if (mbar_try_wait_cluster(bar, parity)) return true;
+    const long long t0 = clock64();
+    for (uint32_t it = 1;; ++it) {
+        if (mbar_try_wait_cluster(bar, parity)) return true;
         if ((it & 63) == 0) {
             if (*reinterpret_cast<volatile int *>(abort_flag) != 0) return false;
             if (clock64() - t0 > 4000000000ll) break;
diff --git a/text_segmentation_image_inpainting_b200/csrc/pcb_tc_epi.cuh b/text_segmentation_image_inpainting_b200/csrc/pcb_tc_epi.cuh
--- a/text_segmentation_image_inpainting_b200/csrc/pcb_tc_epi.cuh
+++ b/text_segmentation_image_inpainting_b200/csrc/pcb_tc_epi.cuh
@@ -46,6 +46,7 @@
     const float *ep_scale, *ep_shift;
     int ep_on, ep_act;
     float ep_slope;
+    int ksplit;
 };
 
 constexpr int STAT_SLICE = 256;
```

New measurement: 1181 (median of 6 runs). +1.7%, better.
